# andrewcharlesjones/spatial-alignment

Measured on AMD Instinct MI355X. Metric: training steps/sec (ELBO fwd+bwd), 2-view N=10k M=200, 1/2/4/8 GPU, higher is better.
Workload: dtype f32 (fp64 warp layer, covariance whitening and M x M factorisations)

## Files before the change

include/gpsa_hip.h:

```cpp
#ifndef GPSA_HIP_H
#define GPSA_HIP_H

#ifdef __cplusplus
extern "C" {
#endif

enum {
  GPSA_F32 = 0,
  GPSA_F64 = 1,
  GPSA_F32_X64 = 2,
  GPSA_F32_OUT64 = 3,
  GPSA_F32_ACC64 = 4
};
enum { GPSA_K_RBF = 0, GPSA_K_MATERN12 = 1, GPSA_K_MATERN32 = 2 };
enum { GPSA_EINVAL = -1, GPSA_EWORKSPACE = -2, GPSA_EUNSUPPORTED = -3 };

int gpsa_version(void);
const char* gpsa_build_arch(void);
const char* gpsa_source_hash(void);

int gpsa_kmat(int dtype, int in_dtype, int kind, const void* Z, int M, const void* X, long long C,
              int D, const void* ls_u, const void* var_u, double jitter, void* K, void* stream);

long long gpsa_kmat_bwd_workspace(int dtype, int M, long long C, int D);
int gpsa_kmat_bwd(int dtype, int in_dtype, int kind, const void* Z, int M, const void* X, long long C,
                  int D, const void* ls_u, const void* var_u, const void* Kbar, int same, void* dZ,
                  void* dX, void* dparams, void* workspace, long long workspace_bytes, void* stream);

long long gpsa_gemm_workspace(int dtype, int m, int n, int batch, int splitk);
int gpsa_gemm(int dtype, int transA, int transB, int m, int n, long long k, double alpha,
              const void* A, long long lda, long long strideA, const void* B, long long ldb,
              long long strideB, double beta, void* C, long long ldc, long long strideC, int batch,
              int splitk, void* workspace, long long workspace_bytes, void* stream);

int gpsa_thin_update_f32(const float* A, int M, int L, const float* B, long long C, float* out, void* stream);

int gpsa_omega_fwd(const float* A, int M, int batch, double jitter, double* Omega, void* stream);
int gpsa_omega_bwd(const double* G, const float* A, int M, int batch, int symmetric, float* dA,
                   void* stream);
int gpsa_omega_fwd2(const float* A0, int n0, double* Omega0, const float* A1, int n1, double* Omega1, int M,
                    double jitter, void* stream);
int gpsa_omega_bwd2(const double* G0, const float* A0, float* dA0, int n0, const double* G1, const float* A1,
                    float* dA1, int n1, int M, int symmetric, void* stream);

int gpsa_chol_f64(void* A, int M, int batch, void* logdet, int* info, void* stream);
int gpsa_tri_inv_f64(const void* L, void* Linv, int M, int batch, void* stream);
int gpsa_chol_inv_f64(const void* A, void* Linv, int M, int batch, void* logdet, int* info,
                      void* stream);
int gpsa_chol_inv_sel_f64(const void* A, void* Linv, int M, int batch, int n_always, int keep_lo, int keep_hi,
                          void* logdet, int* info, void* stream);
long long gpsa_chol_inv_blocked_workspace(int M, int batch);
int gpsa_chol_inv_blocked_f64(const void* A, void* Linv, int M, int batch, void* logdet, int* info,
                              void* workspace, long long workspace_bytes, void* stream);

int gpsa_experiment_split_bf16_product(const float* Omega, const float* alpha, int M, long long C, int L, int nprod,
                                       float* W, void* stream);
int gpsa_experiment_split_bf16_rate(int nprod, int outputs, float* out, void* stream);

long long gpsa_quadform_workspace(int dtype, int M, long long C, int L);
int gpsa_quadform_fwd(int dtype, int omega_dtype, const void* alpha, const void* Omega, int M,
                      long long C, int L, void* v, void* workspace, long long workspace_bytes,
                      void* stream);
int gpsa_quadform_bwd_alpha(int dtype, int omega_dtype, const void* alpha, const void* Omega,
                            const void* g, int M, long long C, int L, void* dalpha, void* workspace,
                            long long workspace_bytes, void* stream);
int gpsa_quadform_fwd_keep(int dtype, const void* alpha, const void* Omega, int M, long long C, int L,
                           void* v, void* W, const void* dcT, void* meanT, void* stream);
int gpsa_quadform_bwd_alpha_kept(int dtype, const void* W, const void* g, int M, long long C, int L,
                                 const void* dcT, const void* dmeanT, void* dalpha, void* stream);
long long gpsa_quadform_keep_f32_workspace(int M, int L);
long long gpsa_quadform_keep_f32_bytes(int M, long long C, int L);
int gpsa_quadform_fwd_keep_f32(int omega_dtype, const float* alpha, const void* Omega, int M, long long C, int L,
                               float* v, float* W, void* workspace, long long workspace_bytes, void* stream);
int gpsa_quadform_bwd_alpha_kept_f32(const float* W, const float* g, int M, long long C, int L, const float* dcT,
                                     const float* dmeanT, float* dalpha, void* stream);
int gpsa_quadform_elbo_parts(void);
long long gpsa_quadform_elbo_f32_workspace(int M, long long C, int L);
int gpsa_quadform_elbo_f32(int omega_dtype, const float* alpha, const void* Omega, int M, long long C, int L,
                           const float* meanT, const double* q, const float* var_u, const float* eps, const float* Y,
                           long long N, int S, const float* noise_u, float* g, float* dmeanT, float* abar, double* part,
                           float* FT, void* workspace, long long workspace_bytes, void* stream);
int gpsa_quadform_elbo_takes_delta(int M);
int gpsa_quadform_elbo_delta_f32(int omega_dtype, const float* alpha, const void* Omega, int M, long long C, int L,
                                 const float* delta, const double* q, const float* var_u, const float* eps,
                                 const float* Y, long long N, int S, const float* noise_u, float* g, float* dmeanT,
                                 float* abar, double* part, float* FT, void* workspace, long long workspace_bytes,
                                 void* stream);
long long gpsa_quadform_elbo_x3_f32_workspace(int M, long long C, int L);
int gpsa_quadform_elbo_x3_f32(int omega_dtype, const float* alpha, const void* Omega, int M, long long C, int L,
                              const float* meanT, const double* q, const float* var_u, const float* eps, const float* Y,
                              long long N, int S, const float* noise_u, float* g, float* dmeanT, float* abar, double* part,
                              float* FT, void* workspace, long long workspace_bytes, void* stream);
int gpsa_quadform_elbo_delta_x3_f32(int omega_dtype, const float* alpha, const void* Omega, int M, long long C, int L,
                                    const float* delta, const double* q, const float* var_u, const float* eps,
                                    const float* Y, long long N, int S, const float* noise_u, float* g, float* dmeanT,
                                    float* abar, double* part, float* FT, void* workspace, long long workspace_bytes,
                                    void* stream);
int gpsa_quadform_elbo_skip_f32(int omega_dtype, const float* alpha, const void* Omega, int M, long long C, int L,
                                const float* meanT, const double* q, const float* var_u, const float* eps, const float* Y,
                                long long N, int S, const float* noise_u, float* g, float* dmeanT, float* abar,
                                double* part, float* FT, void* workspace, long long workspace_bytes, void* stream);
int gpsa_quadform_elbo_delta_skip_f32(int omega_dtype, const float* alpha, const void* Omega, int M, long long C, int L,
                                      const float* delta, const double* q, const float* var_u, const float* eps,
                                      const float* Y, long long N, int S, const float* noise_u, float* g, float* dmeanT,
                                      float* abar, double* part, float* FT, void* workspace, long long workspace_bytes,
                                      void* stream);
int gpsa_quadform_bwd_omega(int dtype, int out_dtype, const void* alpha, const void* g, int M, long long C,
                            int L, void* dOmega, void* workspace, long long workspace_bytes, void* stream);
int gpsa_quadform_bwd_omega_takes_delta(int M, long long C);
int gpsa_quadform_bwd_omega_delta_f32(int out_dtype, const float* alpha, const float* g, const float* dmeanT, int M,
                                      long long C, int L, void* dOmega, float* ddelta, double dbeta, void* workspace,
                                      long long workspace_bytes, void* stream);
long long gpsa_quadform_bwd_omega_x3_workspace(int M, long long C, int L);
int gpsa_quadform_bwd_omega_x3(int dtype, int out_dtype, const void* alpha, const void* g, int M, long long C, int L,
                               void* dOmega, void* workspace, long long workspace_bytes, void* stream);
int gpsa_quadform_bwd_omega_delta_x3(int out_dtype, const float* alpha, const float* g, const float* dmeanT, int M,
                                     long long C, int L, void* dOmega, float* ddelta, double dbeta, void* workspace,
                                     long long workspace_bytes, void* stream);

long long gpsa_whiten_workspace(int M);
int gpsa_whiten_f64(const double* Kinv, int in_dtype, const void* Kuf, int M, long long C,
                    int alpha_dtype, void* alpha, double* q, void* workspace, long long workspace_bytes,
                    void* stream);

int gpsa_panel_mm(int dtype, int p_dtype, int transP, const void* P, const void* X, int M, long long C,
                  void* Y, void* colsq, void* workspace, long long workspace_bytes, void* stream);

int gpsa_col_axpy(int dtype, const void* Y, const void* X, const void* d, double s, int M,
                  long long C, void* out, void* stream);

int gpsa_data_sample_fwd(const float* meanT, const float* v, const double* q, const float* var_u,
                         const float* eps, long long C, int L, float* F, float* Sigma, void* stream);
int gpsa_data_sample_bwd(const float* dF, const float* eps, const float* Sigma, const float* var_u,
                         long long C, int L, float* g, float* dmeanT, float* qbar, int dvar_dtype, void* dvar_u,
                         void* workspace, long long workspace_bytes, void* stream);
int gpsa_warp_sample_fwd(const double* meanT, const double* v, const double* q, const float* var_u,
                         const float* X, const float* slopes, const float* intercept,
                         const float* eps, long long n, int D, int S, float* Gmean, float* Gs,
                         double* Gs64, int* bad, void* stream);
int gpsa_warp_sample_bwd(const float* dGmean, const float* dGs, const double* dGs64, const float* eps,
                         const float* var_u, const float* X, long long n, int D, int S, double* dmeanT, double* g,
                         double* qbar, float* dvar_u, float* dslopes, float* dintercept,
                         void* workspace, long long workspace_bytes, void* stream);

int gpsa_mean_resid_fwd(const float* Z, const float* slopes, const float* intercept,
                        const float* delta, int M, int D, double scale, float* mu_z, double* resid,
                        void* stream);
int gpsa_mean_resid_bwd(const double* dresid, const float* Z, const float* slopes, int M, int D,
                        double scale, float* ddelta, float* dZ, float* dslopes, float* dintercept,
                        void* stream);

int gpsa_loglik_fwd(const float* F, const float* Y, const float* noise_u, int S, long long N, int P,
                    double* out, void* workspace, long long workspace_bytes, void* stream);
int gpsa_loglik_bwd(const float* F, const float* Y, const float* noise_u, const double* gout, int S,
                    long long N, int P, float* dF, float* dnoise_u, void* workspace,
                    long long workspace_bytes, void* stream);

int gpsa_bdot(int dtype, const void* A, long long strideA, const void* B, long long strideB,
              long long n, int batch, void* out, void* workspace, long long workspace_bytes,
              void* stream);
int gpsa_add_diag(int dtype, void* A, int M, int batch, double s, void* stream);

int gpsa_mvn_kl_fwd(const double* Kinv, const double* logdetK, const double* Omega,
                    long long omega_stride, const double* logdetO, long long logdet_stride,
                    const double* Dm, const double* KD, int M, int L, double* kl, void* stream);
int gpsa_mvn_kl_bwd(const double* Kuu, const double* Kinv, const double* Omega, long long omega_stride,
                    const double* Oinv, long long oinv_stride, const double* Dm, const double* KD,
                    const double* g, int M, int L, double* dOmega, double* dDm, double* Sp,
                    void* stream);

int gpsa_mvn_kl_grouped_fwd(const double* mats, const double* inv, const double* logdet,
                            const int* om_idx, const int* pr_idx, const double* D, int M, int T,
                            double* kl, double* KD, void* stream);
int gpsa_mvn_kl_grouped_bwd(const double* mats, const double* inv, const int* om_idx,
                            const int* pr_list, const int* grp_off, const int* order, const double* D,
                            const double* KD, const double* g, int M, int T, int P, double* dOmega,
                            double* dD, double* S, void* stream);

int gpsa_elbo_fwd(const double* ll, int n_ll, const double* kl, int n_kl, double kl_scale, float* loss,
                  void* stream);
int gpsa_elbo_bwd(const float* gloss, int n_ll, int n_kl, double kl_scale, double* dll, double* dkl,
                  void* stream);

long long gpsa_kmeans_workspace(long long N, int D, int K);
int gpsa_kmeans_assign(const float* X, long long N, int D, const float* centres, int K, int* assign,
                       float* d2, void* stream);
int gpsa_kmeans_update(const float* X, const int* assign, long long N, int D, int K, float* centres,
                       int* counts, void* workspace, long long workspace_bytes, void* stream);


int gpsa_kmat_batched(int kind, const float* Z, long long strideZ, int M, const float* X, long long strideX,
                      long long C, int D, const float* ls_u, const float* var_u, int stride_par,
                      const long long* n_live, int batch, double jitter, double* K, long long strideK,
                      void* stream);
long long gpsa_kmat_bwd_batched_workspace(int M, long long C, int D, int batch);
int gpsa_kmat_bwd_batched(int kind, const float* Z, long long strideZ, int M, const float* X, long long strideX,
                          long long C, int D, const float* ls_u, const float* var_u, int stride_par,
                          const long long* n_live, int batch, const double* Kbar, long long strideK, int same,
                          double* dZ, long long stride_dZ, double* dparams, void* workspace,
                          long long workspace_bytes, void* stream);
int gpsa_kmat_bwd_x64(int kind, const float* Z, int M, const double* X, long long C, int D, const float* ls_u,
                      const float* var_u, const float* Kbar, double* dZ, double* dX, double* dparams,
                      void* workspace, long long workspace_bytes, void* stream);
int gpsa_kmat_bwd_x64_f64(int kind, const float* Z, int M, const double* X, long long C, int D, const float* ls_u,
                          const float* var_u, const double* Kbar, double* dZ, double* dX, double* dparams,
                          void* workspace, long long workspace_bytes, void* stream);
int gpsa_kmat_bwd_x64_f64_axpy(int kind, const float* Z, int M, const double* X, long long C, int D, const float* ls_u,
                               const float* var_u, const double* Kbar, const double* X2, const float* d, double s,
                               double* dZ, double* dX, double* dparams, void* workspace, long long workspace_bytes,
                               void* stream);
long long gpsa_exact_dkuu_workspace(int M, long long C);
int gpsa_exact_dkuu_f64(const double* G, const double* A, const float* d, int M, long long C, double* dK,
                        void* workspace, long long workspace_bytes, void* stream);
long long gpsa_longk_f64_workspace(int M, long long K, int nprob);
int gpsa_longk_f64(int nprob, const double* const* G, const double* const* B, const void* const* d, int d_dtype,
                   int M, long long K, long long ld, int sym, const double* alpha, const double* beta,
                   double* const* out, void* workspace, long long workspace_bytes, void* stream);
int gpsa_kmat_bwd_x64_axpy(int kind, const float* Z, int M, const double* X, long long C, int D, const float* ls_u,
                           const float* var_u, const float* Kbar, const float* X2, const float* d, double s,
                           double* dZ, double* dX, double* dparams, void* workspace, long long workspace_bytes,
                           void* stream);
int gpsa_whiten_f64_dual(const double* Kinv, const double* Kuf, int M, long long C, double* alpha64, float* alpha32,
                         double* q, void* workspace, long long workspace_bytes, void* stream);

int gpsa_whiten_gen_f64_dual(const double* Kinv, int kind, const float* Z, const double* X64, int D, const float* ls_u,
                             const float* var_u, int M, long long C, double* alpha64, float* alpha32, double* q,
                             void* workspace, long long workspace_bytes, void* stream);
int gpsa_whiten_axpy_f32(const double* Kinv, const float* X, int M, long long C, const float* X2, const float* d,
                         double s, float* out, void* workspace, long long workspace_bytes, void* stream);
int gpsa_whiten_batched_f64(const double* Kinv, long long strideKinv, const double* Kuf, int M, long long C,
                            long long strideX, double* alpha, double* q, int batch, void* workspace,
                            long long workspace_bytes, void* stream);
int gpsa_quadform_fwd_keep_batched_f64(const double* alpha, const double* Omega, int M, long long C, int L,
                                       double* v, double* W, const double* dcT, double* meanT, int batch,
                                       void* stream);
int gpsa_quadform_bwd_alpha_kept_batched_f64(const double* W, const double* g, int M, long long C, int L,
                                             const double* dcT, const double* dmeanT, double* dalpha,
                                             int batch, void* stream);
int gpsa_col_axpy_batched_f64(const double* Y, const double* X, const double* d, double s, int M, long long C,
                              double* out, int batch, void* stream);
long long gpsa_gram_batched_workspace(int M, long long C, int L, int batch);
int gpsa_gram_batched_f64(const double* alpha, const double* g, int M, long long C, int L, double* dOmega,
                          int batch, void* workspace, long long workspace_bytes, void* stream);
int gpsa_mvn_kl_grouped_bwd_acc(const double* mats, const double* inv, const int* om_idx,
                                const int* pr_list, const int* grp_off, const int* order, const double* D,
                                const double* KD, const double* g, int M, int T, int P, double* dOmega,
                                double* dD, double* S, int accumulate, void* stream);
int gpsa_mvn_kl_grouped_fwd_slices(int M);
int gpsa_mvn_kl_grouped_fwd_sliced(const double* mats, const double* inv, const double* logdet, const int* om_idx,
                                   const int* pr_idx, const double* D, int M, int T, double* kl, double* KD,
                                   double* kl_copy, double* part, int* cnt, void* stream);

#define GPSA_MAX_MODS 4

typedef struct gpsa_step_desc {
  int n_views, n_dims, n_mods, n_samples;
  int m_x, m_g;
  int kind_warp, kind_data;
  int n_latent[GPSA_MAX_MODS];
  int n_out[GPSA_MAX_MODS];
  int has_lmc[GPSA_MAX_MODS];
  long long n_rows[GPSA_MAX_MODS];
  int s_test;
  long long n_test[GPSA_MAX_MODS];
  int want_kl;
  const int* view_fixed;
  const long long* view_rows;
  long long keep_budget_bytes;
  int exact_inducing_grad;
  int kl_own_lo, kl_own_hi;
  int contraction;
} gpsa_step_desc;

typedef struct gpsa_step_params {
  const float* Xtilde;
  const float* delta_G;
  const float* Omega_sqt_G;
  const float* warp_ls;
  const float* warp_var;
  const float* slopes;
  const float* intercepts;
  const float* Gtilde;
  const float* data_ls;
  const float* data_var;
  const float* Omega_sqt_F[GPSA_MAX_MODS];
  const float* delta_F[GPSA_MAX_MODS];
  const float* W[GPSA_MAX_MODS];
} gpsa_step_params;

typedef struct gpsa_step_param_grads {
  float *Xtilde, *delta_G, *Omega_sqt_G, *warp_ls, *warp_var, *Gtilde, *data_ls, *data_var;
  float* Omega_sqt_F[GPSA_MAX_MODS];
  float* delta_F[GPSA_MAX_MODS];
  float* W[GPSA_MAX_MODS];
} gpsa_step_param_grads;

typedef struct gpsa_step_io {
  const float* X[GPSA_MAX_MODS];
  const float* eps_G;
  const float* eps_F[GPSA_MAX_MODS];
  const float* G_test[GPSA_MAX_MODS];
  const float* eps_F_test[GPSA_MAX_MODS];
  float* G_means[GPSA_MAX_MODS];
  float* G_samples[GPSA_MAX_MODS];
  float* F_latent[GPSA_MAX_MODS];
  float* F_obs[GPSA_MAX_MODS];
  float* F_latent_test[GPSA_MAX_MODS];
  float* F_obs_test[GPSA_MAX_MODS];
  float* mu_z;
  double* kl;
  int* flag;
  int keep_products;
  int reuse_mm;
  int fuse_elbo;
  const float* Y[GPSA_MAX_MODS];
  const float* noise_u[GPSA_MAX_MODS];
  double* ll_part[GPSA_MAX_MODS];
  float* F_fused_T[GPSA_MAX_MODS];
  double* bwd_acc;
  int bwd_acc_mode;
  void* f_event;
  const float* loss_src;
  float* loss_dst;
  int skip_missing;
} gpsa_step_io;

typedef struct gpsa_step_out_grads {
  const float* dG_means[GPSA_MAX_MODS];
  const float* dG_samples[GPSA_MAX_MODS];
  const float* dF_latent[GPSA_MAX_MODS];
  const float* dF_obs[GPSA_MAX_MODS];
  const float* dF_latent_test[GPSA_MAX_MODS];
  const float* dF_obs_test[GPSA_MAX_MODS];
  const double* dkl;
  const float* gloss;
} gpsa_step_out_grads;

void* gpsa_step_create(const gpsa_step_desc* desc);
int gpsa_step_describe(const gpsa_step_desc* desc, long long* out);
void gpsa_step_destroy(void* plan);
long long gpsa_step_saved_bytes(const void* plan);
long long gpsa_step_saved_bytes_nokeep(const void* plan);
int gpsa_step_fused(const void* plan, int m);
int gpsa_step_contraction(const void* plan, int m);
long long gpsa_step_scratch_bytes(const void* plan);
long long gpsa_step_bwd_acc_bytes(const void* plan);
int gpsa_step_n_kl(const void* plan);
int gpsa_step_n_factorised(const void* plan);
long long gpsa_step_eps_g_numel(const void* plan);
int gpsa_step_graph(void* plan, int enable, long long* out);
long long gpsa_step_early_backwards(const void* plan);
int gpsa_step_batch_layout(const void* plan, long long* out);
int gpsa_step_forward(void* plan, const gpsa_step_params* params, const gpsa_step_io* io, void* saved,
                      void* scratch, int stages, void* stream);
unsigned long long gpsa_stream_capture_id(void* stream);
int gpsa_step_timing(void* plan, int slots);
int gpsa_step_timing_read(void* plan, float* ms, int max_steps);
int gpsa_step_backward(void* plan, const gpsa_step_params* params, const gpsa_step_io* io,
                       const gpsa_step_out_grads* og, void* saved, void* scratch,
                       const gpsa_step_param_grads* grads, void* stream);

int gpsa_elbo_loss_fwd(int n_ll, const float* const* F, const float* const* Y, const float* const* noise_u,
                       const int* S, const long long* N, const int* P, const double* kl, int n_kl,
                       double kl_scale, float* loss, double* ll_out, void* workspace,
                       long long workspace_bytes, void* stream);
int gpsa_elbo_loss_bwd(int n_ll, const float* const* F, const float* const* Y, const float* const* noise_u,
                       const int* S, const long long* N, const int* P, const float* gloss, int n_kl,
                       double kl_scale, float* const* dF, float* const* dnoise, float* dnoise_all, int n_noise,
                       double* dkl, void* workspace, long long workspace_bytes, void* stream);

int gpsa_elbo_loss_fused_fwd(int n_ll, const float* const* F, const float* const* Y, const float* const* noise_u,
                             const int* S, const long long* N, const int* P, const double* const* zpart, int nparts,
                             const double* kl, int n_kl, double kl_scale, float* loss, double* ll_out, void* workspace,
                             long long workspace_bytes, void* stream);
int gpsa_elbo_loss_fused_bwd(int n_ll, const float* const* F, const float* const* Y, const float* const* noise_u,
                             const int* S, const long long* N, const int* P, const double* const* zpart, int nparts,
                             const float* gloss, int n_kl, double kl_scale, float* const* dF, float* const* dnoise,
                             float* dnoise_all, int n_noise, double* dkl, void* workspace, long long workspace_bytes,
                             void* stream);
long long gpsa_lmc_loglik_workspace(long long C, int L, int P, int nparts);
int gpsa_lmc_loglik_fused_f32(const float* F, const float* W, const float* Y, const float* noise_u, int S, long long N,
                              int L, int P, double* zpart, int nparts, float* dF, float* dW, void* workspace,
                              long long workspace_bytes, void* stream);
int gpsa_elbo_fused_post(float* g_ext, float* dmeanT, float* abar, int M, long long C, int L, const float* gloss,
                         const float* var_u, int dvar_dtype, void* dvar_u, void* workspace, long long workspace_bytes,
                         void* stream);

int gpsa_adam_step(int n, float* const* params, const float* const* grads, float* const* exp_avg,
                   float* const* exp_avg_sq, const long long* numel, double lr, double beta1, double beta2,
                   double eps, float* step, void* stream);

int gpsa_row_sample_gather(int n_mods, const int* n_views, const long long* n_rows, const long long* batch,
                           unsigned long long seed, long long* counter, const float* const* X, const int* D,
                           const float* const* Y, const int* P, long long* const* rows, float* const* Xb,
                           float* const* Yb, void* stream);
int gpsa_elbo_loss_weighted_fwd(int n_ll, const float* const* F, const float* const* Y, const float* const* noise_u,
                                const int* S, const long long* N, const int* P, const int* n_views,
                                const long long* const* view_off, const double* const* w, const double* kl, int n_kl,
                                double kl_scale, float* loss, double* ll_out, void* workspace,
                                long long workspace_bytes, void* stream);
int gpsa_elbo_loss_weighted_bwd(int n_ll, const float* const* F, const float* const* Y, const float* const* noise_u,
                                const int* S, const long long* N, const int* P, const int* n_views,
                                const long long* const* view_off, const double* const* w, const float* gloss, int n_kl,
                                double kl_scale, float* const* dF, float* const* dnoise, float* dnoise_all,
                                int n_noise, double* dkl, void* workspace, long long workspace_bytes, void* stream);

long long gpsa_count_observed_workspace(void);
int gpsa_count_observed(int n_ll, const float* const* Y, const long long* N, const int* P, const int* n_views,
                        const long long* const* view_off, double* const* nobs, void* workspace,
                        long long workspace_bytes, void* stream);
int gpsa_elbo_loss_skip_fwd(int n_ll, const float* const* F, const float* const* Y, const float* const* noise_u,
                            const int* S, const long long* N, const int* P, const double* const* zpart, int nparts,
                            const int* n_views, const long long* const* view_off, const double* const* w,
                            const double* const* nobs, const double* kl, int n_kl, double kl_scale, float* loss,
                            double* ll_out, void* workspace, long long workspace_bytes, void* stream);
int gpsa_elbo_loss_skip_bwd(int n_ll, const float* const* F, const float* const* Y, const float* const* noise_u,
                            const int* S, const long long* N, const int* P, const double* const* zpart, int nparts,
                            const int* n_views, const long long* const* view_off, const double* const* w,
                            const double* const* nobs, const float* gloss, int n_kl, double kl_scale, float* const* dF,
                            float* const* dnoise, float* dnoise_all, int n_noise, double* dkl, void* workspace,
                            long long workspace_bytes, void* stream);
int gpsa_lmc_loglik_fused_skip_f32(const float* F, const float* W, const float* Y, const float* noise_u, int S, long long N,
                                   int L, int P, double* zpart, int nparts, float* dF, float* dW, void* workspace,
                                   long long workspace_bytes, void* stream);

#define GPSA_LIK_GAUSSIAN 0
#define GPSA_LIK_POISSON 1
long long gpsa_lgamma_sum_workspace(void);
int gpsa_lgamma_sum(int n_ll, const float* const* Y, const long long* N, const int* P, const int* n_views,
                    const long long* const* view_off, int skip, double* const* out, void* workspace,
                    long long workspace_bytes, void* stream);
int gpsa_elbo_loss_pois_fwd(int n_ll, const float* const* F, const float* const* Y, const float* const* noise_u,
                            const int* S, const long long* N, const int* P, const double* const* zpart, int nparts,
                            const int* n_views, const long long* const* view_off, const double* const* w,
                            const double* const* nobs, const int* kind, const double* const* lgam,
                            const float* const* log_offset, int skip, const double* kl, int n_kl, double kl_scale,
                            float* loss, double* ll_out, void* workspace, long long workspace_bytes, void* stream);
int gpsa_elbo_loss_pois_bwd(int n_ll, const float* const* F, const float* const* Y, const float* const* noise_u,
                            const int* S, const long long* N, const int* P, const double* const* zpart, int nparts,
                            const int* n_views, const long long* const* view_off, const double* const* w,
                            const double* const* nobs, const int* kind, const double* const* lgam,
                            const float* const* log_offset, int skip, const float* gloss, int n_kl, double kl_scale,
                            float* const* dF, float* const* dnoise, float* dnoise_all, int n_noise, double* dkl,
                            void* workspace, long long workspace_bytes, void* stream);
int gpsa_quadform_elbo_pois_f32(int omega_dtype, const float* alpha, const void* Omega, int M, long long C, int L,
                                const float* meanT, const double* q, const float* var_u, const float* eps, const float* Y,
                                long long N, int S, const float* noise_u, float* g, float* dmeanT, float* abar,
                                double* part, float* FT, const float* log_offset, int skip, void* workspace,
                                long long workspace_bytes, void* stream);
int gpsa_quadform_elbo_delta_pois_f32(int omega_dtype, const float* alpha, const void* Omega, int M, long long C, int L,
                                      const float* delta, const double* q, const float* var_u, const float* eps,
                                      const float* Y, long long N, int S, const float* noise_u, float* g, float* dmeanT,
                                      float* abar, double* part, float* FT, const float* log_offset, int skip,
                                      void* workspace, long long workspace_bytes, void* stream);
int gpsa_lmc_loglik_fused_pois_f32(const float* F, const float* W, const float* Y, const float* log_offset, int skip, int S,
                                   long long N, int L, int P, double* zpart, int nparts, float* dF, float* dW,
                                   void* workspace, long long workspace_bytes, void* stream);
int gpsa_step_likelihood(void* plan, int m, int kind, const float* log_offset);

#define GPSA_LIK_NEGBIN 2
long long gpsa_nb_const_workspace(long long N, int P, int n_views);
int gpsa_nb_const(int n_ll, const float* const* Y, const long long* N, const int* P, const float* const* log_disp,
                  const int* n_views, const long long* const* view_off, const double* const* w, int skip,
                  double* const* csum, double* const* dconst, void* workspace, long long workspace_bytes, void* stream);
int gpsa_quadform_elbo_nb_f32(int omega_dtype, const float* alpha, const void* Omega, int M, long long C, int L,
                              const float* meanT, const double* q, const float* var_u, const float* eps, const float* Y,
                              long long N, int S, const float* noise_u, float* g, float* dmeanT, float* abar, double* part,
                              float* FT, const float* log_offset, const float* log_disp, float* u_elems, double* usum,
                              int skip, void* workspace, long long workspace_bytes, void* stream);
int gpsa_quadform_elbo_delta_nb_f32(int omega_dtype, const float* alpha, const void* Omega, int M, long long C, int L,
                                    const float* delta, const double* q, const float* var_u, const float* eps,
                                    const float* Y, long long N, int S, const float* noise_u, float* g, float* dmeanT,
                                    float* abar, double* part, float* FT, const float* log_offset, const float* log_disp,
                                    float* u_elems, double* usum, int skip, void* workspace, long long workspace_bytes,
                                    void* stream);
int gpsa_step_dispersion(void* plan, int m, const float* log_disp, float* u_elems, double* usum, const float* log_offset);
long long gpsa_lmc_loglik_nb_workspace(long long C, int L, int P, int nparts);
int gpsa_lmc_loglik_fused_nb_f32(const float* F, const float* W, const float* Y, const float* log_offset,
                                 const float* log_disp, int skip, int S, long long N, int L, int P, double* zpart,
                                 int nparts, float* dF, float* dW, double* usum, void* workspace,
                                 long long workspace_bytes, void* stream);
long long gpsa_elbo_loss_nb_workspace(int n_ll, const int* S, const long long* N, const int* P, const int* n_views,
                                      const int* kind);
int gpsa_elbo_loss_nb_fwd(int n_ll, const float* const* F, const float* const* Y, const float* const* noise_u,
                          const int* S, const long long* N, const int* P, const double* const* zpart, int nparts,
                          const int* n_views, const long long* const* view_off, const double* const* w,
                          const double* const* nobs, const int* kind, const double* const* lgam,
                          const float* const* log_offset, const float* const* log_disp, const double* const* csum,
                          int skip, const double* kl, int n_kl, double kl_scale, float* loss, double* ll_out,
                          void* workspace, long long workspace_bytes, void* stream);
int gpsa_elbo_loss_nb_bwd(int n_ll, const float* const* F, const float* const* Y, const float* const* noise_u,
                          const int* S, const long long* N, const int* P, const double* const* zpart, int nparts,
                          const int* n_views, const long long* const* view_off, const double* const* w,
                          const double* const* nobs, const int* kind, const double* const* lgam,
                          const float* const* log_offset, const float* const* log_disp, const double* const* dconst,
                          const double* const* usum, int skip, const float* gloss, int n_kl, double kl_scale,
                          float* const* dF, float* const* dnoise, float* dnoise_all, int n_noise, double* dkl,
                          float* const* ddisp, void* workspace, long long workspace_bytes, void* stream);

int gpsa_predict_moments_f32(const float* meanT, const float* v, const double* q, const float* var_u, long long c,
                             int S, int L, int P, const float* W, const float* noise_u, int include_noise,
                             const float* Y, float* F_mean, float* F_var, float* Fl_mean, float* Fl_var, double* lpd,
                             void* stream);

int gpsa_predict_counts_f32(const float* meanT, const float* v, const double* q, const float* var_u, long long c, int S,
                            int L, int P, const float* W, const float* log_offset, const float* Y, float* Y_mean,
                            float* Y_var, double* lpd, void* stream);

int gpsa_warp_field_f64(int kind, const double* Z, const double* beta, const double* A, const double* b,
                        const double* ls_u, const double* var_u, const double* X, long long n, int M, int D, double* G,
                        double* J, double* det, void* stream);
int gpsa_warp_invert_f64(int kind, const double* Z, const double* beta, const double* A, const double* b,
                         const double* ls_u, const double* var_u, const double* target, const double* x0, int iters,
                         long long n, int M, int D, double* X, double* residual, void* stream);

long long gpsa_knn_workspace(long long nq, long long nr, int k, int parts);
int gpsa_knn_f64(const double* Q, long long nq, const double* R, long long nr, int D, int k, int exclude_self, int parts,
                 int* idx, double* d2, void* workspace, long long workspace_bytes, void* stream);
int gpsa_knn_average_f32(const int* idx, const double* d2, long long nq, int k, const float* Y, long long nr, int P,
                         int weights, float* out, void* stream);
// ... 107 lines not shown
```

spatial_alignment_amd/_lib.py:

```python
import ctypes as C
import os

_HERE = os.path.dirname(os.path.abspath(__file__))
LIB_PATH = os.path.join(_HERE, "libgpsa_hip.so")

_vp, _i, _ll, _d = C.c_void_p, C.c_int, C.c_longlong, C.c_double

SIGNATURES = {
    "gpsa_version": (_i, []),
    "gpsa_build_arch": (C.c_char_p, []),
    "gpsa_source_hash": (C.c_char_p, []),
    "gpsa_kmat": (_i, [_i, _i, _i, _vp, _i, _vp, _ll, _i, _vp, _vp, _d, _vp, _vp]),
    "gpsa_kmat_bwd_workspace": (_ll, [_i, _i, _ll, _i]),
    "gpsa_kmat_bwd": (_i, [_i, _i, _i, _vp, _i, _vp, _ll, _i, _vp, _vp, _vp, _i, _vp, _vp, _vp, _vp, _ll, _vp]),
    "gpsa_gemm_workspace": (_ll, [_i, _i, _i, _i, _i]),
    "gpsa_gemm": (_i, [_i, _i, _i, _i, _i, _ll, _d, _vp, _ll, _ll, _vp, _ll, _ll, _d, _vp, _ll, _ll,
                       _i, _i, _vp, _ll, _vp]),
    "gpsa_omega_fwd": (_i, [_vp, _i, _i, _d, _vp, _vp]),
    "gpsa_omega_bwd": (_i, [_vp, _vp, _i, _i, _i, _vp, _vp]),
    "gpsa_omega_fwd2": (_i, [_vp, _i, _vp, _vp, _i, _vp, _i, _d, _vp]),
    "gpsa_omega_bwd2": (_i, [_vp, _vp, _vp, _i, _vp, _vp, _vp, _i, _i, _i, _vp]),
    "gpsa_chol_f64": (_i, [_vp, _i, _i, _vp, _vp, _vp]),
    "gpsa_tri_inv_f64": (_i, [_vp, _vp, _i, _i, _vp]),
    "gpsa_chol_inv_f64": (_i, [_vp, _vp, _i, _i, _vp, _vp, _vp]),
    "gpsa_experiment_split_bf16_product": (_i, [_vp, _vp, _i, _ll, _i, _i, _vp, _vp]),
    "gpsa_experiment_split_bf16_rate": (_i, [_i, _i, _vp, _vp]),
    "gpsa_chol_inv_sel_f64": (_i, [_vp, _vp, _i, _i, _i, _i, _i, _vp, _vp, _vp]),
    "gpsa_chol_inv_blocked_workspace": (_ll, [_i, _i]),
    "gpsa_chol_inv_blocked_f64": (_i, [_vp, _vp, _i, _i, _vp, _vp, _vp, _ll, _vp]),
    "gpsa_quadform_workspace": (_ll, [_i, _i, _ll, _i]),
    "gpsa_quadform_fwd": (_i, [_i, _i, _vp, _vp, _i, _ll, _i, _vp, _vp, _ll, _vp]),
    "gpsa_quadform_bwd_alpha": (_i, [_i, _i, _vp, _vp, _vp, _i, _ll, _i, _vp, _vp, _ll, _vp]),
    "gpsa_quadform_fwd_keep": (_i, [_i, _vp, _vp, _i, _ll, _i, _vp, _vp, _vp, _vp, _vp]),
    "gpsa_quadform_bwd_alpha_kept": (_i, [_i, _vp, _vp, _i, _ll, _i, _vp, _vp, _vp, _vp]),
    "gpsa_quadform_bwd_omega": (_i, [_i, _i, _vp, _vp, _i, _ll, _i, _vp, _vp, _ll, _vp]),
    "gpsa_quadform_bwd_omega_takes_delta": (_i, [_i, _ll]),
    "gpsa_quadform_bwd_omega_delta_f32": (_i, [_i, _vp, _vp, _vp, _i, _ll, _i, _vp, _vp, _d, _vp, _ll, _vp]),
    "gpsa_quadform_bwd_omega_x3_workspace": (_ll, [_i, _ll, _i]),
    "gpsa_quadform_bwd_omega_x3": (_i, [_i, _i, _vp, _vp, _i, _ll, _i, _vp, _vp, _ll, _vp]),
    "gpsa_quadform_bwd_omega_delta_x3": (_i, [_i, _vp, _vp, _vp, _i, _ll, _i, _vp, _vp, _d, _vp, _ll, _vp]),
    "gpsa_whiten_workspace": (_ll, [_i]),
    "gpsa_whiten_f64": (_i, [_vp, _i, _vp, _i, _ll, _i, _vp, _vp, _vp, _ll, _vp]),
    "gpsa_panel_mm": (_i, [_i, _i, _i, _vp, _vp, _i, _ll, _vp, _vp, _vp, _ll, _vp]),
    "gpsa_col_axpy": (_i, [_i, _vp, _vp, _vp, _d, _i, _ll, _vp, _vp]),
    "gpsa_data_sample_fwd": (_i, [_vp, _vp, _vp, _vp, _vp, _ll, _i, _vp, _vp, _vp]),
    "gpsa_data_sample_bwd": (_i, [_vp, _vp, _vp, _vp, _ll, _i, _vp, _vp, _vp, _i, _vp, _vp, _ll, _vp]),
    "gpsa_warp_sample_fwd": (_i, [_vp, _vp, _vp, _vp, _vp, _vp, _vp, _vp, _ll, _i, _i, _vp, _vp, _vp, _vp, _vp]),
    "gpsa_warp_sample_bwd": (_i, [_vp, _vp, _vp, _vp, _vp, _vp, _ll, _i, _i, _vp, _vp, _vp, _vp, _vp, _vp, _vp,
                                  _ll, _vp]),
    "gpsa_mean_resid_fwd": (_i, [_vp, _vp, _vp, _vp, _i, _i, _d, _vp, _vp, _vp]),
    "gpsa_mean_resid_bwd": (_i, [_vp, _vp, _vp, _i, _i, _d, _vp, _vp, _vp, _vp, _vp]),
    "gpsa_loglik_fwd": (_i, [_vp, _vp, _vp, _i, _ll, _i, _vp, _vp, _ll, _vp]),
    "gpsa_loglik_bwd": (_i, [_vp, _vp, _vp, _vp, _i, _ll, _i, _vp, _vp, _vp, _ll, _vp]),
    "gpsa_bdot": (_i, [_i, _vp, _ll, _vp, _ll, _ll, _i, _vp, _vp, _ll, _vp]),
    "gpsa_add_diag": (_i, [_i, _vp, _i, _i, _d, _vp]),
    "gpsa_mvn_kl_fwd": (_i, [_vp, _vp, _vp, _ll, _vp, _ll, _vp, _vp, _i, _i, _vp, _vp]),
    "gpsa_mvn_kl_bwd": (_i, [_vp, _vp, _vp, _ll, _vp, _ll, _vp, _vp, _vp, _i, _i, _vp, _vp, _vp, _vp]),
    "gpsa_mvn_kl_grouped_fwd": (_i, [_vp, _vp, _vp, _vp, _vp, _vp, _i, _i, _vp, _vp, _vp]),
    "gpsa_mvn_kl_grouped_bwd": (_i, [_vp, _vp, _vp, _vp, _vp, _vp, _vp, _vp, _vp, _i, _i, _i, _vp, _vp, _vp,
                                     _vp]),
    "gpsa_elbo_fwd": (_i, [_vp, _i, _vp, _i, _d, _vp, _vp]),
    "gpsa_elbo_bwd": (_i, [_vp, _i, _i, _d, _vp, _vp, _vp]),
    "gpsa_kmeans_workspace": (_ll, [_ll, _i, _i]),
    "gpsa_kmeans_assign": (_i, [_vp, _ll, _i, _vp, _i, _vp, _vp, _vp]),
    "gpsa_kmeans_update": (_i, [_vp, _vp, _ll, _i, _i, _vp, _vp, _vp, _ll, _vp]),
}

MAX_MODS = 4


class StepDesc(C.Structure):
    _fields_ = [
        ("n_views", _i), ("n_dims", _i), ("n_mods", _i), ("n_samples", _i),
        ("m_x", _i), ("m_g", _i), ("kind_warp", _i), ("kind_data", _i),
        ("n_latent", _i * MAX_MODS), ("n_out", _i * MAX_MODS), ("has_lmc", _i * MAX_MODS),
        ("n_rows", _ll * MAX_MODS), ("s_test", _i), ("n_test", _ll * MAX_MODS), ("want_kl", _i),
        ("view_fixed", C.POINTER(_i)), ("view_rows", C.POINTER(_ll)), ("keep_budget_bytes", _ll),
        ("exact_inducing_grad", _i), ("kl_own_lo", _i), ("kl_own_hi", _i), ("contraction", _i),
    ]


class StepParams(C.Structure):
    _fields_ = [
        ("Xtilde", _vp), ("delta_G", _vp), ("Omega_sqt_G", _vp), ("warp_ls", _vp), ("warp_var", _vp),
        ("slopes", _vp), ("intercepts", _vp), ("Gtilde", _vp), ("data_ls", _vp), ("data_var", _vp),
        ("Omega_sqt_F", _vp * MAX_MODS), ("delta_F", _vp * MAX_MODS), ("W", _vp * MAX_MODS),
    ]


class StepParamGrads(C.Structure):
    _fields_ = [
        ("Xtilde", _vp), ("delta_G", _vp), ("Omega_sqt_G", _vp), ("warp_ls", _vp), ("warp_var", _vp),
        ("Gtilde", _vp), ("data_ls", _vp), ("data_var", _vp),
        ("Omega_sqt_F", _vp * MAX_MODS), ("delta_F", _vp * MAX_MODS), ("W", _vp * MAX_MODS),
    ]


class StepIO(C.Structure):
    _fields_ = [
        ("X", _vp * MAX_MODS), ("eps_G", _vp), ("eps_F", _vp * MAX_MODS), ("G_test", _vp * MAX_MODS),
        ("eps_F_test", _vp * MAX_MODS), ("G_means", _vp * MAX_MODS), ("G_samples", _vp * MAX_MODS),
        ("F_latent", _vp * MAX_MODS), ("F_obs", _vp * MAX_MODS), ("F_latent_test", _vp * MAX_MODS),
        ("F_obs_test", _vp * MAX_MODS), ("mu_z", _vp), ("kl", _vp), ("flag", _vp), ("keep_products", _i),
        ("reuse_mm", _i), ("fuse_elbo", _i), ("Y", _vp * MAX_MODS), ("noise_u", _vp * MAX_MODS),
        ("ll_part", _vp * MAX_MODS), ("F_fused_T", _vp * MAX_MODS), ("bwd_acc", _vp), ("bwd_acc_mode", _i),
        ("f_event", _vp), ("loss_src", _vp), ("loss_dst", _vp), ("skip_missing", _i),
    ]


class StepOutGrads(C.Structure):
    _fields_ = [
        ("dG_means", _vp * MAX_MODS), ("dG_samples", _vp * MAX_MODS), ("dF_latent", _vp * MAX_MODS),
        ("dF_obs", _vp * MAX_MODS), ("dF_latent_test", _vp * MAX_MODS), ("dF_obs_test", _vp * MAX_MODS),
        ("dkl", _vp), ("gloss", _vp),
    ]


_pp = C.POINTER(_vp)

SIGNATURES.update({
    "gpsa_kmat_batched": (_i, [_i, _vp, _ll, _i, _vp, _ll, _ll, _i, _vp, _vp, _i, C.POINTER(_ll), _i, _d, _vp, _ll, _vp]),
    "gpsa_kmat_bwd_batched_workspace": (_ll, [_i, _ll, _i, _i]),
    "gpsa_kmat_bwd_batched": (_i, [_i, _vp, _ll, _i, _vp, _ll, _ll, _i, _vp, _vp, _i, C.POINTER(_ll), _i, _vp, _ll, _i,
                                   _vp, _ll, _vp, _vp, _ll, _vp]),
    "gpsa_kmat_bwd_x64": (_i, [_i, _vp, _i, _vp, _ll, _i, _vp, _vp, _vp, _vp, _vp, _vp, _vp, _ll, _vp]),
    "gpsa_kmat_bwd_x64_f64": (_i, [_i, _vp, _i, _vp, _ll, _i, _vp, _vp, _vp, _vp, _vp, _vp, _vp, _ll, _vp]),
    "gpsa_kmat_bwd_x64_f64_axpy": (_i, [_i, _vp, _i, _vp, _ll, _i, _vp, _vp, _vp, _vp, _vp, _d, _vp, _vp, _vp, _vp, _ll,
                                        _vp]),
    "gpsa_exact_dkuu_workspace": (_ll, [_i, _ll]),
    "gpsa_exact_dkuu_f64": (_i, [_vp, _vp, _vp, _i, _ll, _vp, _vp, _ll, _vp]),
    "gpsa_longk_f64_workspace": (_ll, [_i, _ll, _i]),
    "gpsa_longk_f64": (_i, [_i, _vp, _vp, _vp, _i, _i, _ll, _ll, _i, _vp, _vp, _vp, _vp, _ll, _vp]),
    "gpsa_kmat_bwd_x64_axpy": (_i, [_i, _vp, _i, _vp, _ll, _i, _vp, _vp, _vp, _vp, _vp, _d, _vp, _vp, _vp, _vp, _ll,
                                    _vp]),
    "gpsa_thin_update_f32": (_i, [_vp, _i, _i, _vp, _ll, _vp, _vp]),
    "gpsa_whiten_f64_dual": (_i, [_vp, _vp, _i, _ll, _vp, _vp, _vp, _vp, _ll, _vp]),
    "gpsa_whiten_gen_f64_dual": (_i, [_vp, _i, _vp, _vp, _i, _vp, _vp, _i, _ll, _vp, _vp, _vp, _vp, _ll, _vp]),
    "gpsa_whiten_axpy_f32": (_i, [_vp, _vp, _i, _ll, _vp, _vp, _d, _vp, _vp, _ll, _vp]),
    "gpsa_whiten_batched_f64": (_i, [_vp, _ll, _vp, _i, _ll, _ll, _vp, _vp, _i, _vp, _ll, _vp]),
    "gpsa_quadform_fwd_keep_batched_f64": (_i, [_vp, _vp, _i, _ll, _i, _vp, _vp, _vp, _vp, _i, _vp]),
    "gpsa_quadform_bwd_alpha_kept_batched_f64": (_i, [_vp, _vp, _i, _ll, _i, _vp, _vp, _vp, _i, _vp]),
    "gpsa_col_axpy_batched_f64": (_i, [_vp, _vp, _vp, _d, _i, _ll, _vp, _i, _vp]),
    "gpsa_gram_batched_workspace": (_ll, [_i, _ll, _i, _i]),
    "gpsa_gram_batched_f64": (_i, [_vp, _vp, _i, _ll, _i, _vp, _i, _vp, _ll, _vp]),
    "gpsa_mvn_kl_grouped_bwd_acc": (_i, [_vp, _vp, _vp, _vp, _vp, _vp, _vp, _vp, _vp, _i, _i, _i, _vp, _vp, _vp, _i,
                                         _vp]),
    "gpsa_mvn_kl_grouped_fwd_slices": (_i, [_i]),
    "gpsa_mvn_kl_grouped_fwd_sliced": (_i, [_vp, _vp, _vp, _vp, _vp, _vp, _i, _i, _vp, _vp, _vp, _vp, _vp, _vp]),
    "gpsa_step_create": (_vp, [C.POINTER(StepDesc)]),
    "gpsa_step_describe": (_i, [C.POINTER(StepDesc), C.POINTER(_ll)]),
    "gpsa_step_destroy": (None, [_vp]),
    "gpsa_step_saved_bytes": (_ll, [_vp]),
    "gpsa_step_saved_bytes_nokeep": (_ll, [_vp]),
    "gpsa_quadform_keep_f32_workspace": (_ll, [_i, _i]),
    "gpsa_quadform_fwd_keep_f32": (_i, [_i, _vp, _vp, _i, _ll, _i, _vp, _vp, _vp, _ll, _vp]),
    "gpsa_quadform_keep_f32_bytes": (_ll, [_i, _ll, _i]),
    "gpsa_quadform_bwd_alpha_kept_f32": (_i, [_vp, _vp, _i, _ll, _i, _vp, _vp, _vp, _vp]),
    "gpsa_lmc_loglik_workspace": (_ll, [_ll, _i, _i, _i]),
    "gpsa_lmc_loglik_fused_f32": (_i, [_vp, _vp, _vp, _vp, _i, _ll, _i, _i, _vp, _i, _vp, _vp, _vp, _ll, _vp]),
    "gpsa_quadform_elbo_parts": (_i, []),
    "gpsa_quadform_elbo_f32_workspace": (_ll, [_i, _ll, _i]),
    "gpsa_quadform_elbo_f32": (_i, [_i, _vp, _vp, _i, _ll, _i, _vp, _vp, _vp, _vp, _vp, _ll, _i, _vp, _vp, _vp, _vp, _vp,
                                    _vp, _vp, _ll, _vp]),
    "gpsa_quadform_elbo_takes_delta": (_i, [_i]),
    "gpsa_quadform_elbo_x3_f32_workspace": (_ll, [_i, _ll, _i]),
    "gpsa_quadform_elbo_x3_f32": (_i, [_i, _vp, _vp, _i, _ll, _i, _vp, _vp, _vp, _vp, _vp, _ll, _i, _vp, _vp, _vp, _vp,
                                       _vp, _vp, _vp, _ll, _vp]),
    "gpsa_quadform_elbo_delta_x3_f32": (_i, [_i, _vp, _vp, _i, _ll, _i, _vp, _vp, _vp, _vp, _vp, _ll, _i, _vp, _vp, _vp,
                                             _vp, _vp, _vp, _vp, _ll, _vp]),
    "gpsa_quadform_elbo_delta_f32": (_i, [_i, _vp, _vp, _i, _ll, _i, _vp, _vp, _vp, _vp, _vp, _ll, _i, _vp, _vp, _vp, _vp,
                                          _vp, _vp, _vp, _ll, _vp]),
    "gpsa_step_scratch_bytes": (_ll, [_vp]),
    "gpsa_step_bwd_acc_bytes": (_ll, [_vp]),
    "gpsa_step_n_kl": (_i, [_vp]),
    "gpsa_step_n_factorised": (_i, [_vp]),
    "gpsa_step_eps_g_numel": (_ll, [_vp]),
    "gpsa_step_batch_layout": (_i, [_vp, C.POINTER(_ll)]),
    "gpsa_step_graph": (_i, [_vp, _i, C.POINTER(_ll)]),
    "gpsa_step_early_backwards": (_ll, [_vp]),
    "gpsa_stream_capture_id": (C.c_ulonglong, [_vp]),
    "gpsa_step_timing": (_i, [_vp, _i]),
    "gpsa_step_timing_read": (_i, [_vp, _vp, _i]),
    "gpsa_step_forward": (_i, [_vp, C.POINTER(StepParams), C.POINTER(StepIO), _vp, _vp, _i, _vp]),
    "gpsa_step_backward": (_i, [_vp, C.POINTER(StepParams), C.POINTER(StepIO), C.POINTER(StepOutGrads), _vp, _vp,
                                C.POINTER(StepParamGrads), _vp]),
    "gpsa_elbo_loss_fwd": (_i, [_i, _pp, _pp, _pp, C.POINTER(_i), C.POINTER(_ll), C.POINTER(_i), _vp, _i, _d, _vp,
                                _vp, _vp, _ll, _vp]),
    "gpsa_elbo_loss_bwd": (_i, [_i, _pp, _pp, _pp, C.POINTER(_i), C.POINTER(_ll), C.POINTER(_i), _vp, _i, _d, _pp, _pp,
                                _vp, _i, _vp, _vp, _ll, _vp]),
    "gpsa_elbo_loss_fused_fwd": (_i, [_i, _pp, _pp, _pp, C.POINTER(_i), C.POINTER(_ll), C.POINTER(_i), _pp, _i, _vp, _i,
                                      _d, _vp, _vp, _vp, _ll, _vp]),
    "gpsa_elbo_loss_fused_bwd": (_i, [_i, _pp, _pp, _pp, C.POINTER(_i), C.POINTER(_ll), C.POINTER(_i), _pp, _i, _vp, _i,
                                      _d, _pp, _pp, _vp, _i, _vp, _vp, _ll, _vp]),
    "gpsa_elbo_fused_post": (_i, [_vp, _vp, _vp, _i, _ll, _i, _vp, _vp, _i, _vp, _vp, _ll, _vp]),
    "gpsa_step_fused": (_i, [_vp, _i]),
    "gpsa_step_contraction": (_i, [_vp, _i]),
    "gpsa_adam_step": (_i, [_i, _pp, _pp, _pp, _pp, C.POINTER(_ll), _d, _d, _d, _d, _vp, _vp]),
    "gpsa_row_sample_gather": (_i, [_i, C.POINTER(_i), C.POINTER(_ll), C.POINTER(_ll), C.c_ulonglong, _vp, _pp,
                                    C.POINTER(_i), _pp, C.POINTER(_i), _pp, _pp, _pp, _vp]),
    "gpsa_elbo_loss_weighted_fwd": (_i, [_i, _pp, _pp, _pp, C.POINTER(_i), C.POINTER(_ll), C.POINTER(_i),
                                         C.POINTER(_i), _pp, _pp, _vp, _i, _d, _vp, _vp, _vp, _ll, _vp]),
    "gpsa_elbo_loss_weighted_bwd": (_i, [_i, _pp, _pp, _pp, C.POINTER(_i), C.POINTER(_ll), C.POINTER(_i),
                                         C.POINTER(_i), _pp, _pp, _vp, _i, _d, _pp, _pp, _vp, _i, _vp, _vp, _ll, _vp]),
    "gpsa_quadform_elbo_skip_f32": (_i, [_i, _vp, _vp, _i, _ll, _i, _vp, _vp, _vp, _vp, _vp, _ll, _i, _vp, _vp, _vp, _vp,
                                         _vp, _vp, _vp, _ll, _vp]),
    "gpsa_quadform_elbo_delta_skip_f32": (_i, [_i, _vp, _vp, _i, _ll, _i, _vp, _vp, _vp, _vp, _vp, _ll, _i, _vp, _vp, _vp,
                                               _vp, _vp, _vp, _vp, _ll, _vp]),
    "gpsa_count_observed_workspace": (_ll, []),
    "gpsa_count_observed": (_i, [_i, _pp, C.POINTER(_ll), C.POINTER(_i), C.POINTER(_i), _pp, _pp, _vp, _ll, _vp]),
    "gpsa_elbo_loss_skip_fwd": (_i, [_i, _pp, _pp, _pp, C.POINTER(_i), C.POINTER(_ll), C.POINTER(_i), _pp, _i,
                                     C.POINTER(_i), _pp, _pp, _pp, _vp, _i, _d, _vp, _vp, _vp, _ll, _vp]),
    "gpsa_elbo_loss_skip_bwd": (_i, [_i, _pp, _pp, _pp, C.POINTER(_i), C.POINTER(_ll), C.POINTER(_i), _pp, _i,
                                     C.POINTER(_i), _pp, _pp, _pp, _vp, _i, _d, _pp, _pp, _vp, _i, _vp, _vp, _ll, _vp]),
    "gpsa_lmc_loglik_fused_skip_f32": (_i, [_vp, _vp, _vp, _vp, _i, _ll, _i, _i, _vp, _i, _vp, _vp, _vp, _ll, _vp]),
    "gpsa_predict_moments_f32": (_i, [_vp, _vp, _vp, _vp, _ll, _i, _i, _i, _vp, _vp, _i, _vp, _vp, _vp, _vp, _vp, _vp,
                                      _vp]),
    "gpsa_predict_counts_f32": (_i, [_vp, _vp, _vp, _vp, _ll, _i, _i, _i, _vp, _vp, _vp, _vp, _vp, _vp, _vp]),
    "gpsa_warp_field_f64": (_i, [_i, _vp, _vp, _vp, _vp, _vp, _vp, _vp, _ll, _i, _i, _vp, _vp, _vp, _vp]),
    "gpsa_warp_invert_f64": (_i, [_i, _vp, _vp, _vp, _vp, _vp, _vp, _vp, _vp, _i, _ll, _i, _i, _vp, _vp, _vp]),
    "gpsa_knn_workspace": (_ll, [_ll, _ll, _i, _i]),
    "gpsa_knn_f64": (_i, [_vp, _ll, _vp, _ll, _i, _i, _i, _i, _vp, _vp, _vp, _ll, _vp]),
    "gpsa_knn_average_f32": (_i, [_vp, _vp, _ll, _i, _vp, _ll, _i, _i, _vp, _vp]),
    "gpsa_knn_average_f64": (_i, [_vp, _vp, _ll, _i, _vp, _ll, _i, _i, _vp, _vp]),
    "gpsa_count_workspace": (_ll, [_ll, _ll]),
    "gpsa_count_margins_f32": (_i, [_vp, _ll, _ll, _vp, _vp, _vp, _vp, _vp, _vp, _ll, _vp]),
    "gpsa_count_deviance_f32": (_i, [_vp, _ll, _ll, _vp, _vp, _vp, _vp, _ll, _vp]),
    "gpsa_count_transform_f32": (_i, [_i, _vp, _ll, _ll, _vp, _vp, _d, _d, _d, _d, _vp, _vp]),
    "gpsa_standardize_views_f32": (_i, [_vp, _ll, _ll, C.POINTER(_ll), _i, _vp, _vp, _vp, _ll, _vp]),
    "gpsa_count_csr_workspace": (_ll, [_ll, _ll]),
    "gpsa_csr_check": (_i, [_vp, _vp, _vp, _ll, _ll, _ll, _vp, _vp, _ll, _vp]),
    "gpsa_count_margins_csr_f32": (_i, [_vp, _vp, _vp, _vp, _ll, _ll, _ll, _vp, _vp, _vp, _vp, _vp, _vp, _ll, _vp]),
    "gpsa_count_deviance_csr_f32": (_i, [_vp, _vp, _vp, _vp, _ll, _ll, _ll, _vp, _vp, _vp, _vp, _ll, _vp]),
    "gpsa_csr_gather_dense_f32": (_i, [_vp, _vp, _vp, _ll, _ll, _ll, _vp, _ll, _vp, _ll, _vp, _vp]),
    "gpsa_column_moments_workspace": (_ll, [_ll, _ll, _i]),
    "gpsa_column_moments_csr_workspace": (_ll, [_ll, _ll, _i]),
    "gpsa_column_moments_f32": (_i, [_i, _vp, _ll, _ll, _vp, C.POINTER(_ll), _i, _vp, _vp, _vp, _vp, _vp, _ll, _vp]),
    "gpsa_column_moments_csr_f32": (_i, [_i, _vp, _vp, _vp, _vp, _ll, _ll, _ll, _vp, C.POINTER(_ll), _i, _vp, _vp, _vp,
                                         _vp, _vp, _ll, _vp]),
    "gpsa_gpr_cov_f64": (_i, [_i, _vp, _ll, _vp, _ll, _i, _vp, _i, _i, _d, _vp, _vp]),
    "gpsa_gpr_lml_grad_workspace": (_ll, [_ll, _i]),
    "gpsa_gpr_lml_grad_f64": (_i, [_i, _vp, _ll, _i, _vp, _i, _vp, _i, _vp, _vp, _vp, _ll, _vp]),
    "gpsa_gpr_mean_f64": (_i, [_i, _vp, _ll, _vp, _ll, _i, _vp, _i, _vp, _i, _vp, _vp]),
    "gpsa_ot_dist_f64": (_i, [_vp, _ll, _i, _vp, _vp]),
    "gpsa_ot_sqmatvec_f64": (_i, [_vp, _ll, _ll, _vp, _vp, _vp]),
    "gpsa_ot_expr_rows_workspace": (_ll, [_ll]),
    "gpsa_ot_expr_rows_f32": (_i, [_i, _vp, _ll, _ll, _vp, _vp, _vp, _vp, _vp, _ll, _vp]),
    "gpsa_ot_expr_cost_f64": (_i, [_i, _vp, _ll, _ll, _vp, _vp, _vp]),
    "gpsa_ot_cost_workspace": (_ll, [_ll, _ll]),
    "gpsa_ot_cost_f64": (_i, [_vp, _vp, _vp, _vp, _vp, _vp, _vp, _d, _ll, _ll, _vp, _vp, _ll, _vp]),
    "gpsa_ot_sinkhorn_workspace": (_ll, [_ll, _ll]),
    "gpsa_ot_sinkhorn_f64": (_i, [_vp, _ll, _ll, _vp, _vp, _vp, _vp, _vp, _i, _vp, _ll, _vp]),
    "gpsa_ot_plan_workspace": (_ll, [_ll, _ll]),
    "gpsa_ot_plan_f64": (_i, [_vp, _ll, _ll, _vp, _vp, _vp, _vp, _vp, _vp, _vp, _vp, _vp, _vp, _ll, _vp]),
    "gpsa_image_select_workspace": (_ll, [_ll, _ll, _i]),
    "gpsa_image_select_count_u8": (_i, [_vp, _ll, _ll, _i, _i, _i, C.c_float, _i, C.POINTER(_d), _vp, _ll, _vp]),
    "gpsa_image_select_count_f32": (_i, [_vp, _ll, _ll, _i, _i, _i, C.c_float, _i, C.POINTER(_d), _vp, _ll, _vp]),
    "gpsa_image_select_write_u8": (_i, [_vp, _ll, _ll, _i, _i, _i, C.c_float, _i, C.POINTER(_d), _vp, _ll, _vp, _vp, _ll,
                                        _vp]),
    "gpsa_image_select_write_f32": (_i, [_vp, _ll, _ll, _i, _i, _i, C.c_float, _i, C.POINTER(_d), _vp, _ll, _vp, _vp, _ll,
                                         _vp]),
    "gpsa_image_sample_u8": (_i, [_vp, _ll, _ll, _i, _vp, _ll, _i, C.c_float, _vp, _vp, _vp]),
    "gpsa_image_sample_f32": (_i, [_vp, _ll, _ll, _i, _vp, _ll, _i, C.c_float, _vp, _vp, _vp]),
    "gpsa_graph_workspace": (_ll, [_ll]),
    "gpsa_graph_merge_count": (_i, [_vp, _vp, _vp, _ll, _i, _i, _vp, _vp]),
    "gpsa_graph_merge_write": (_i, [_vp, _vp, _vp, _ll, _i, _i, _i, _vp, _ll, _vp, _vp, _vp]),
    "gpsa_graph_check_f64": (_i, [_vp, _vp, _vp, _ll, _ll, _vp, _vp, _ll, _vp]),
    "gpsa_graph_sums_f64": (_i, [_vp, _vp, _vp, _vp, _vp, _ll, _ll, _vp, _vp, _ll, _vp]),
    "gpsa_autocorr_perm_workspace": (_ll, [_ll, _ll, _ll]),
    "gpsa_autocorr_perm_f64": (_i, [_vp, _ll, _ll, _vp, _vp, _vp, _ll, _vp, _ll, _i, _vp, _vp, _vp, _ll, _vp]),
    "gpsa_lgamma_sum_workspace": (_ll, []),
    "gpsa_lgamma_sum": (_i, [_i, _pp, C.POINTER(_ll), C.POINTER(_i), C.POINTER(_i), _pp, _i, _pp, _vp, _ll, _vp]),
    "gpsa_elbo_loss_pois_fwd": (_i, [_i, _pp, _pp, _pp, C.POINTER(_i), C.POINTER(_ll), C.POINTER(_i), _pp, _i,
                                     C.POINTER(_i), _pp, _pp, _pp, C.POINTER(_i), _pp, _pp, _i, _vp, _i, _d, _vp, _vp,
                                     _vp, _ll, _vp]),
    "gpsa_elbo_loss_pois_bwd": (_i, [_i, _pp, _pp, _pp, C.POINTER(_i), C.POINTER(_ll), C.POINTER(_i), _pp, _i,
                                     C.POINTER(_i), _pp, _pp, _pp, C.POINTER(_i), _pp, _pp, _i, _vp, _i, _d, _pp, _pp,
                                     _vp, _i, _vp, _vp, _ll, _vp]),
    "gpsa_quadform_elbo_pois_f32": (_i, [_i, _vp, _vp, _i, _ll, _i, _vp, _vp, _vp, _vp, _vp, _ll, _i, _vp, _vp, _vp, _vp,
                                         _vp, _vp, _vp, _i, _vp, _ll, _vp]),
    "gpsa_quadform_elbo_delta_pois_f32": (_i, [_i, _vp, _vp, _i, _ll, _i, _vp, _vp, _vp, _vp, _vp, _ll, _i, _vp, _vp, _vp,
                                               _vp, _vp, _vp, _vp, _i, _vp, _ll, _vp]),
    "gpsa_lmc_loglik_fused_pois_f32": (_i, [_vp, _vp, _vp, _vp, _i, _i, _ll, _i, _i, _vp, _i, _vp, _vp, _vp, _ll, _vp]),
    "gpsa_step_likelihood": (_i, [_vp, _i, _i, _vp]),
    "gpsa_nb_const_workspace": (_ll, [_ll, _i, _i]),
    "gpsa_nb_const": (_i, [_i, _pp, C.POINTER(_ll), C.POINTER(_i), _pp, C.POINTER(_i), _pp, _pp, _i, _pp, _pp, _vp, _ll,
                           _vp]),
    "gpsa_quadform_elbo_nb_f32": (_i, [_i, _vp, _vp, _i, _ll, _i, _vp, _vp, _vp, _vp, _vp, _ll, _i, _vp, _vp, _vp, _vp,
                                       _vp, _vp, _vp, _vp, _vp, _vp, _i, _vp, _ll, _vp]),
    "gpsa_quadform_elbo_delta_nb_f32": (_i, [_i, _vp, _vp, _i, _ll, _i, _vp, _vp, _vp, _vp, _vp, _ll, _i, _vp, _vp, _vp,
                                             _vp, _vp, _vp, _vp, _vp, _vp, _vp, _i, _vp, _ll, _vp]),
    "gpsa_step_dispersion": (_i, [_vp, _i, _vp, _vp, _vp, _vp]),
    "gpsa_lmc_loglik_nb_workspace": (_ll, [_ll, _i, _i, _i]),
    "gpsa_lmc_loglik_fused_nb_f32": (_i, [_vp, _vp, _vp, _vp, _vp, _i, _i, _ll, _i, _i, _vp, _i, _vp, _vp, _vp, _vp, _ll,
                                          _vp]),
    "gpsa_elbo_loss_nb_workspace": (_ll, [_i, C.POINTER(_i), C.POINTER(_ll), C.POINTER(_i), C.POINTER(_i),
                                          C.POINTER(_i)]),
    "gpsa_elbo_loss_nb_fwd": (_i, [_i, _pp, _pp, _pp, C.POINTER(_i), C.POINTER(_ll), C.POINTER(_i), _pp, _i,
                                   C.POINTER(_i), _pp, _pp, _pp, C.POINTER(_i), _pp, _pp, _pp, _pp, _i, _vp, _i, _d, _vp,
                                   _vp, _vp, _ll, _vp]),
    "gpsa_elbo_loss_nb_bwd": (_i, [_i, _pp, _pp, _pp, C.POINTER(_i), C.POINTER(_ll), C.POINTER(_i), _pp, _i,
                                   C.POINTER(_i), _pp, _pp, _pp, C.POINTER(_i), _pp, _pp, _pp, _pp, _pp, _i, _vp, _i, _d,
                                   _pp, _pp, _vp, _i, _vp, _pp, _vp, _ll, _vp]),
})

LIK_KINDS = {"gaussian": 0, "poisson": 1}
LIK_NEGBIN = 2
LIK_KIND_OF = dict(LIK_KINDS, negative_binomial=LIK_NEGBIN)

_lib = None


def source_hash():
    import glob
    import hashlib

    csrc = os.path.join(_HERE, "csrc")
    header = os.path.join(os.path.dirname(_HERE), "include", "gpsa_hip.h")
    files = sorted(glob.glob(os.path.join(csrc, "*.hip")) + glob.glob(os.path.join(csrc, "*.hpp")))
    if not files or not os.path.exists(header):
        return None
    h = hashlib.sha256()
    for f in files + [header]:
        h.update(os.path.basename(f).encode() + b"\0")
        h.update(open(f, "rb").read())
        h.update(b"\0")
    return h.hexdigest()


def library_hash(path=None):
    import re

    path = path or LIB_PATH
    if not os.path.exists(path):
        return None
    m = re.search(rb"GPSA_SOURCE_HASH=([0-9a-f]{64}|unstamped)", open(path, "rb").read())
    return m.group(1).decode() if m else None


class GpsaHipError(RuntimeError):
    pass


def load():
    global _lib
    if _lib is not None:
        return _lib
    if not os.path.exists(LIB_PATH):
        raise GpsaHipError(
            f"{LIB_PATH} not found: build it with `python -c 'import __graft_entry__ as g; g.build()'` "
            "(hipcc --offload-arch=gfx950).  There is no CPU fallback."
        )
    lib = C.CDLL(LIB_PATH)
    for name, (res, args) in SIGNATURES.items():
        fn = getattr(lib, name)
        fn.restype = res
        fn.argtypes = args
    want = source_hash()
    got = lib.gpsa_source_hash().decode().split("=", 1)[1]
    if want is not None and got != want and os.environ.get("GPSA_ALLOW_STALE_LIB") != "1":
        raise GpsaHipError(
            f"{LIB_PATH} was built from other sources (stamp {got[:12]}, sources {want[:12]}): rebuild it with "
            "`python -c 'import __graft_entry__ as g; g.build()'`"
        )
    _lib = lib
    return lib


GPSA_EINVAL, GPSA_EWORKSPACE, GPSA_EUNSUPPORTED = -1, -2, -3


def check(rc, what):
    if rc != 0:
        kind = {-1: "invalid argument", -2: "workspace too small", -3: "unsupported size"}.get(
            rc, f"hipError_t {rc}"
        )
        raise GpsaHipError(f"{what} failed: {kind}")
```

spatial_alignment_amd/csrc/longk64.hip:

```cpp
#include <stdlib.h>
#include <string.h>

#include "internal.hpp"

namespace gpsa {

typedef double lk_f64x4 __attribute__((ext_vector_type(4)));
typedef double lk_f64x2 __attribute__((ext_vector_type(2)));
typedef float lk_f32x2 __attribute__((ext_vector_type(2)));
typedef __attribute__((address_space(3))) void* lk_lds_ptr;

constexpr int LK_WAVES = 8;
constexpr int LK_MAXP = 48;

struct LongKArgs {
  const double* G[LK_MAXP];
  const double* B[LK_MAXP];
  const void* d[LK_MAXP];
  double* part;
  int M, nprob, nsplit, sym;
  long long K, ld, gper;
};

__device__ __forceinline__ void lk_set_m0(unsigned lds_base) {
  asm volatile("s_mov_b32 m0, %0\n\ts_nop 0" ::"s"(lds_base) : "memory");
}
template <int IMM>
__device__ __forceinline__ void lk_glds16(const void* gsrc_minus_imm) {
  asm volatile("global_load_lds_dwordx4 %0, off offset:%1" ::"v"(gsrc_minus_imm), "n"(IMM) : "memory");
}
template <int IMM>
__device__ __forceinline__ void lk_glds4(const void* gsrc_minus_imm) {
  asm volatile("global_load_lds_dword %0, off offset:%1" ::"v"(gsrc_minus_imm), "n"(IMM) : "memory");
}

template <int MB, bool HASG, int DT>
__global__ void __launch_bounds__(512) longk64_kernel(LongKArgs a) {
  static_assert(HASG || DT != 0, "a left operand");
  constexpr int MP = MB * 16;
  constexpr int NOPD = HASG ? 2 : 1;
  constexpr int NPIECE = MB * NOPD * 2;
  constexpr int NPW = (NPIECE + LK_WAVES - 1) / LK_WAVES;
  static_assert(NPW <= 8, "two groups of four pieces per wave (an immediate offset reaches 4 KiB)");
  constexpr int DAREA = DT == 2 ? 1024 : 256;
  constexpr int STAGE_B = NPW * LK_WAVES * 1024 + (DT ? LK_WAVES * DAREA : 0);
  constexpr int NT_MAX = (MB * MB + LK_WAVES - 1) / LK_WAVES;
  constexpr int NT_SYM = (MB * (MB + 1) / 2 + LK_WAVES - 1) / LK_WAVES;
  extern __shared__ __attribute__((aligned(16))) char lk_smem[];

  const int tid = threadIdx.x, lane = tid & 63;
  const int w = __builtin_amdgcn_readfirstlane(tid >> 6);
  const int li = lane & 15, kq = lane >> 4;
  const int p = blockIdx.y, sp = blockIdx.x;
  const int M = a.M;
  const long long K = a.K, ld = a.ld;
  const double* __restrict__ Bp = a.B[p];
  const double* __restrict__ Gp = HASG ? a.G[p] : nullptr;
  const long long ng = (K + 15) >> 4;
  const long long g_lo = (long long)sp * a.gper;
  long long g_hi = g_lo + a.gper;
  if (g_hi > ng) g_hi = ng;
  const unsigned lds0 = (unsigned)(unsigned long long)(lk_lds_ptr)(&lk_smem[0]);

  const int T = a.sym ? MB * (MB + 1) / 2 : MB * MB;
  const int t_lo = w * T / LK_WAVES, t_hi = (w + 1) * T / LK_WAVES;
  const int cnt = t_hi - t_lo;
  int i0 = 0, j0 = 0;
  if (a.sym) {
    while ((i0 + 1) * (i0 + 2) / 2 <= t_lo) ++i0;
    j0 = t_lo - i0 * (i0 + 1) / 2;
  } else {
    i0 = t_lo / MB;
    j0 = t_lo - i0 * MB;
  }
  if (cnt == 0) i0 = j0 = 0;

  const double* rp[NPW];
  int koff[NPW];
#pragma unroll
  for (int u = 0; u < NPW; ++u) {
    int q = w + LK_WAVES * u;
    q = q < NPIECE ? q : NPIECE - 1;
    const int h = q & 1, ot = q >> 1;
    const bool isg = HASG && ot >= MB;
    const int t = isg ? ot - MB : ot;
    int row = t * 16 + li;
    row = row < M ? row : M - 1;
    rp[u] = (isg ? Gp : Bp) + (long long)row * ld;
    koff[u] = 8 * h + 2 * kq;
  }

  auto issue = [&](long long g, int s) {
    const long long kb = g << 4;
#pragma unroll
    for (int u = 0; u < NPW; ++u) {
      if ((u & 3) == 0)
        lk_set_m0(__builtin_amdgcn_readfirstlane(lds0 + (unsigned)(s * STAGE_B + (w * NPW + u) * 1024)));
      long long k = kb + koff[u];
      k = k < K - 2 ? k : K - 2;
      const char* src = reinterpret_cast<const char*>(rp[u] + k);
      switch (u & 3) {
        case 0: lk_glds16<0>(src); break;
        case 1: lk_glds16<1024>(src - 1024); break;
        case 2: lk_glds16<2048>(src - 2048); break;
        default: lk_glds16<3072>(src - 3072); break;
      }
    }
    if (DT != 0) {
      lk_set_m0(__builtin_amdgcn_readfirstlane(lds0 + (unsigned)(s * STAGE_B + NPW * LK_WAVES * 1024 + w * DAREA)));
      if (DT == 1) {
        long long k = kb + (lane & 15);
        k = k < K ? k : K - 1;
        lk_glds4<0>(reinterpret_cast<const float*>(a.d[p]) + k);
      } else {
        long long k = kb + 2 * (lane & 7);
        k = k < K - 1 ? k : K - 2;
        lk_glds16<0>(reinterpret_cast<const double*>(a.d[p]) + k);
      }
    }
  };

  lk_f64x4 acc[NT_MAX];
#pragma unroll
  for (int t = 0; t < NT_MAX; ++t) acc[t] = (lk_f64x4){0.0, 0.0, 0.0, 0.0};

  if (g_lo < g_hi) {
    issue(g_lo, 0);
    int s = 0;
    for (long long g = g_lo; g < g_hi; ++g) {
      asm volatile("s_waitcnt vmcnt(0)" ::: "memory");
      __syncthreads();
      if (g + 1 < g_hi) issue(g + 1, s ^ 1);
      const char* slot = lk_smem + s * STAGE_B;
      const char* dslot = slot + NPW * LK_WAVES * 1024 + w * DAREA;
      const long long k_a = (g << 4) + 2 * kq;
      double dv[2][2] = {{1.0, 1.0}, {1.0, 1.0}};
      bool ok[2][2];
#pragma unroll
      for (int h = 0; h < 2; ++h) {
        ok[h][0] = k_a + 8 * h < K;
        ok[h][1] = k_a + 8 * h + 1 < K;
        if (DT == 1) {
          const lk_f32x2 x = *reinterpret_cast<const lk_f32x2*>(dslot + 4 * (8 * h + 2 * kq));
          dv[h][0] = (double)x.x;
          dv[h][1] = (double)x.y;
        } else if (DT == 2) {
          const lk_f64x2 x = *reinterpret_cast<const lk_f64x2*>(dslot + 8 * (8 * h + 2 * kq));
          dv[h][0] = x.x;
          dv[h][1] = x.y;
        }
      }
#define LK_FRAG(O, TL, H)                                                                              \
  (*reinterpret_cast<const lk_f64x2*>(slot + ((((((O) * MB + (TL)) * 2 + (H)) & 7) * NPW +             \
                                                 ((((O) * MB + (TL)) * 2 + (H)) >> 3)) << 10) + lane * 16))
      int i = i0, j = j0, cur = -1;
      double af[2][2] = {{0.0, 0.0}, {0.0, 0.0}};
      lk_f64x2 bn0 = LK_FRAG(0, j, 0), bn1 = LK_FRAG(0, j, 1);
#pragma unroll
      for (int t = 0; t < NT_MAX; ++t) {
        if (t >= NT_SYM && a.sym) break;
        if (i != cur) {
          cur = i;
#pragma unroll
          for (int h = 0; h < 2; ++h) {
            const lk_f64x2 bi = LK_FRAG(0, i, h);
            double x0, x1;
            if (HASG) {
              const lk_f64x2 gi = LK_FRAG(1, i, h);
              x0 = DT ? fma(dv[h][0], bi.x, gi.x) : gi.x;
              x1 = DT ? fma(dv[h][1], bi.y, gi.y) : gi.y;
            } else {
              x0 = dv[h][0] * bi.x;
              x1 = dv[h][1] * bi.y;
            }
            af[h][0] = ok[h][0] ? x0 : 0.0;
            af[h][1] = ok[h][1] ? x1 : 0.0;
          }
        }
        const lk_f64x2 b0 = bn0, b1 = bn1;
        if (t + 1 < cnt) {
          ++j;
          if (a.sym ? j > i : j == MB) {
            ++i;
            j = 0;
          }
        }
        if (t + 1 < NT_MAX) {
          bn0 = LK_FRAG(0, j, 0);
          bn1 = LK_FRAG(0, j, 1);
        }
        acc[t] = __builtin_amdgcn_mfma_f64_16x16x4f64(af[0][0], b0.x, acc[t], 0, 0, 0);
        acc[t] = __builtin_amdgcn_mfma_f64_16x16x4f64(af[0][1], b0.y, acc[t], 0, 0, 0);
        acc[t] = __builtin_amdgcn_mfma_f64_16x16x4f64(af[1][0], b1.x, acc[t], 0, 0, 0);
        acc[t] = __builtin_amdgcn_mfma_f64_16x16x4f64(af[1][1], b1.y, acc[t], 0, 0, 0);
      }
#undef LK_FRAG
      s ^= 1;
    }
  }
  double* __restrict__ out = a.part + ((long long)p * a.nsplit + sp) * MP * MP;
  int i = i0, j = j0;
#pragma unroll
  for (int t = 0; t < NT_MAX; ++t) {
    if (t < cnt) {
#pragma unroll
      for (int r = 0; r < 4; ++r) out[(long long)(i * 16 + kq + 4 * r) * MP + j * 16 + li] = acc[t][r];
      ++j;
      if (a.sym ? j > i : j == MB) {
        ++i;
        j = 0;
      }
    }
  }
}

struct LongKOut {
  double* out[LK_MAXP];
  double alpha[LK_MAXP], beta[LK_MAXP];
};

__global__ void __launch_bounds__(256)
longk64_reduce_kernel(const double* __restrict__ part, int M, int MP, int nsplit, int sym, LongKOut o) {
  __shared__ double red[4][64];
  const int lane = threadIdx.x & 63, grp = threadIdx.x >> 6;
  const int p = blockIdx.y;
  const long long e = blockIdx.x * 64LL + lane;
  const int r = (int)(e / M), c = (int)(e % M);
  const bool ok = e < (long long)M * M && !(sym && c > r);
  const long long mm = (long long)MP * MP;
  const double* q = part + (long long)p * nsplit * mm + (long long)r * MP + c;
  double a0 = 0.0, a1 = 0.0, a2 = 0.0, a3 = 0.0;
  if (ok) {
    int s = grp;
    for (; s + 12 < nsplit; s += 16) {
      a0 += q[s * mm];
      a1 += q[(s + 4) * mm];
      a2 += q[(s + 8) * mm];
      a3 += q[(s + 12) * mm];
    }
    for (; s < nsplit; s += 4) a0 += q[s * mm];
  }
  red[grp][lane] = (a0 + a1) + (a2 + a3);
  __syncthreads();
  if (grp == 0 && ok) {
    const double sum = (red[0][lane] + red[1][lane]) + (red[2][lane] + red[3][lane]);
    const double al = o.alpha[p], be = o.beta[p];
    double* dst = o.out[p] + (long long)r * M + c;
    *dst = (be == 0.0) ? al * sum : al * sum + be * (*dst);
    if (sym && c < r) {
      double* dm = o.out[p] + (long long)c * M + r;
      *dm = (be == 0.0) ? al * sum : al * sum + be * (*dm);
    }
  }
}

static inline int longk_mb_for(int M) {
  const int mb = (M + 15) / 16;
  if (mb <= 2) return 2;
  if (mb <= 4) return 4;
  if (mb <= 7) return 7;
  if (mb <= 13) return 13;
  if (mb <= 16) return 16;
  return 0;
}

static inline int longk_nsplit(long long K, int nprob) {
  const long long ng = (K + 15) / 16;
  long long s = (long long)num_cus() / (nprob > 0 ? nprob : 1);
  if (s > ng / 4) s = ng / 4;
  return (int)(s < 1 ? 1 : s);
}

template <int MB, bool HASG, int DT>
static int longk64_launch_mb(const LongKArgs& a, hipStream_t st) {
  constexpr int NPIECE = MB * (HASG ? 2 : 1) * 2, NPW = (NPIECE + LK_WAVES - 1) / LK_WAVES;
  constexpr int lds = 2 * (NPW * LK_WAVES * 1024 + (DT ? LK_WAVES * (DT == 2 ? 1024 : 256) : 0));
  static per_device_flag attr_flag;
  bool& attr_set = attr_flag.here();
  if (!attr_set) {
    if (hipFuncSetAttribute(reinterpret_cast<const void*>(&longk64_kernel<MB, HASG, DT>),
                            hipFuncAttributeMaxDynamicSharedMemorySize, lds) != hipSuccess)
      return GPSA_EUNSUPPORTED;
    attr_set = true;
  }
  dim3 grid((unsigned)a.nsplit, (unsigned)a.nprob);
  longk64_kernel<MB, HASG, DT><<<grid, 512, lds, st>>>(a);
  GPSA_LAUNCH_CHECK();
  return 0;
}

template <bool HASG, int DT>
static int longk64_launch(int MB, const LongKArgs& a, hipStream_t st) {
  switch (MB) {
    case 2: return longk64_launch_mb<2, HASG, DT>(a, st);
    case 4: return longk64_launch_mb<4, HASG, DT>(a, st);
    case 7: return longk64_launch_mb<7, HASG, DT>(a, st);
    case 13: return longk64_launch_mb<13, HASG, DT>(a, st);
    case 16: return longk64_launch_mb<16, HASG, DT>(a, st);
    default: return GPSA_EUNSUPPORTED;
  }
}

}

extern "C" {

long long gpsa_longk_f64_workspace(int M, long long K, int nprob) {
  using namespace gpsa;
  const int MB = longk_mb_for(M);
  if (MB == 0 || nprob < 1 || nprob > LK_MAXP || K < 512 || (K & 1)) return 0;
  const int ns = longk_nsplit(K, nprob);
  if ((long long)ns * nprob < 48) return 0;
  return (long long)nprob * ns * MB * 16 * MB * 16 * 8;
}

int gpsa_longk_f64(int nprob, const double* const* G, const double* const* B, const void* const* d, int d_dtype,
                   int M, long long K, long long ld, int sym, const double* alpha, const double* beta,
                   double* const* out, void* workspace, long long workspace_bytes, void* stream) {
  using namespace gpsa;
  if (nprob < 1 || nprob > LK_MAXP || !B || !out || !alpha || !beta || M < 1 || K < 2 || ld < K) return GPSA_EINVAL;
  if (d != nullptr && d_dtype != GPSA_F32 && d_dtype != GPSA_F64) return GPSA_EINVAL;
  if (G == nullptr && d == nullptr) return GPSA_EINVAL;
  const long long need = gpsa_longk_f64_workspace(M, K, nprob);
  if (need == 0 || (ld & 1)) return GPSA_EUNSUPPORTED;
  if (workspace_bytes < need) return GPSA_EWORKSPACE;
  const int MB = longk_mb_for(M);
  LongKArgs a;
  LongKOut o;
  memset(&a, 0, sizeof(a));
  memset(&o, 0, sizeof(o));
  for (int p = 0; p < nprob; ++p) {
    a.B[p] = B[p];
    a.G[p] = G ? G[p] : nullptr;
    a.d[p] = d ? d[p] : nullptr;
    if (!B[p] || !out[p] || (G && !G[p]) || (d && !d[p])) return GPSA_EINVAL;
    if ((reinterpret_cast<uintptr_t>(B[p]) & 15) || (G && (reinterpret_cast<uintptr_t>(G[p]) & 15)) ||
        (d && d_dtype == GPSA_F64 && (reinterpret_cast<uintptr_t>(d[p]) & 15)))
      return GPSA_EUNSUPPORTED;
    o.out[p] = out[p];
    o.alpha[p] = alpha[p];
    o.beta[p] = beta[p];
  }
  a.part = reinterpret_cast<double*>(workspace);
  a.M = M;
  a.nprob = nprob;
  a.nsplit = longk_nsplit(K, nprob);
  a.sym = sym ? 1 : 0;
  a.K = K;
  a.ld = ld;
  a.gper = cdiv(cdiv(K, 16), a.nsplit);
  hipStream_t st = as_stream(stream);
  int rc;
  if (G && d && d_dtype == GPSA_F32) rc = longk64_launch<true, 1>(MB, a, st);
  else if (G && d) rc = longk64_launch<true, 2>(MB, a, st);
  else if (G) rc = longk64_launch<true, 0>(MB, a, st);
  else if (d_dtype == GPSA_F32) rc = longk64_launch<false, 1>(MB, a, st);
  else rc = longk64_launch<false, 2>(MB, a, st);
  if (rc) return rc;
  dim3 rg((unsigned)cdiv((long long)M * M, 64), (unsigned)nprob);
  longk64_reduce_kernel<<<rg, 256, 0, st>>>(a.part, M, MB * 16, a.nsplit, a.sym, o);
  GPSA_LAUNCH_CHECK();
  return 0;
}

}
```

spatial_alignment_amd/csrc/step.hip:

```cpp
#include <stdint.h>
#include <stdio.h>
#include <stdlib.h>
#include <string.h>

#include <new>
#include <vector>

#include "internal.hpp"

namespace gpsa {

constexpr int MAXMODS = GPSA_MAX_MODS;
constexpr int KM_MAXB_STEP = 16;

struct Arena {
  char* base = nullptr;
  long long off = 0, high = 0;
  long long limit = -1;
  bool dry = false;
  bool overflow = false;
  template <typename T>
  T* get(long long n) {
    off = (off + 255) & ~255LL;
    T* p = dry ? nullptr : reinterpret_cast<T*>(base + off);
// ... 592 lines not shown
  p->bidx.assign(V, -1);
  p->nview.assign(V, 0);
  p->epsoff.assign(V, 0);
  for (int m = 0; m < nm; ++m) {
    long long tot = 0;
    for (int v = 0; v < V; ++v) {
      if (p->rows[(long long)m * V + v] < 0) { free_plan(p); return nullptr; }
      tot += p->rows[(long long)m * V + v];
    }
    if (tot != dsc->n_rows[m] || dsc->n_latent[m] < 1 || dsc->n_out[m] < 1) { free_plan(p); return nullptr; }
    if (!dsc->has_lmc[m] && dsc->n_latent[m] != dsc->n_out[m]) { free_plan(p); return nullptr; }
  }
  long long maxn = 0;
  for (int v = 0; v < V; ++v) {
    for (int m = 0; m < nm; ++m) p->nview[v] += p->rows[(long long)m * V + v];
    if (!p->fixed[v]) {
      p->bidx[v] = (int)p->free_views.size();
      p->free_views.push_back(v);
      p->epsoff[v] = p->eps_total;
      p->eps_total += (long long)S * p->nview[v] * D;
      if (p->nview[v] > maxn) maxn = p->nview[v];
    }
  }
  p->nf = (int)p->free_views.size();
  p->Cs = (maxn + 63) / 64 * 64;
  for (int b = 0; b < p->nf;) {
    int e = b + 1;
    while (e < p->nf && p->free_views[e] == p->free_views[e - 1] + 1 && e - b < KM_MAXB_STEP) ++e;
    p->runs.push_back(Run{p->free_views[b], b, e - b});
    b = e;
  }
  p->Ltot = 0;
  for (int m = 0; m < nm; ++m) {
    p->Loff[m] = p->Ltot;
    p->Ltot += dsc->n_latent[m];
  }
  for (int m = nm; m < MAXMODS; ++m) p->Loff[m] = p->Ltot;
  p->merged = p->Mx == p->Mg;
  if (p->merged) {
    p->ng = 1;
    p->grp[0].M = p->Mx;
    p->grp[0].n_prior = p->nf + 1;
    p->grp[0].n_omega = V * D + p->Ltot;
    p->grp[0].kl_off = 0;
  } else {
    p->ng = 2;
    p->grp[0].M = p->Mx; p->grp[0].n_prior = p->nf; p->grp[0].n_omega = V * D; p->grp[0].kl_off = 0;
    p->grp[1].M = p->Mg; p->grp[1].n_prior = 1; p->grp[1].n_omega = p->Ltot; p->grp[1].kl_off = V * D;
  }
  for (int g = 0; g < p->ng; ++g) {
    Group& G = p->grp[g];
    G.own_lo = 0;
    G.own_hi = G.n_omega;
    if (dsc->kl_own_hi > 0) {
      const int lo = dsc->kl_own_lo - G.kl_off, hi = dsc->kl_own_hi - G.kl_off;
      G.own_lo = lo < 0 ? 0 : (lo > G.n_omega ? G.n_omega : lo);
      G.own_hi = hi < G.own_lo ? G.own_lo : (hi > G.n_omega ? G.n_omega : hi);
    }
  }
  for (int m = 0; m < nm; ++m)
    if (dsc->n_rows[m] > 0 && S > 0) {
      Pass q; q.m = m; q.test = false; q.C = (long long)S * dsc->n_rows[m];
      p->passes.push_back(q);
    }
  if (dsc->s_test > 0)
    for (int m = 0; m < nm; ++m)
      if (dsc->n_test[m] > 0) {
        Pass q; q.m = m; q.test = true; q.C = (long long)dsc->s_test * dsc->n_test[m];
        p->passes.push_back(q);
      }
  long long o = 0;
  auto take = [&](long long bytes) { long long r = o; o = align256(o + bytes); return r; };
  for (int g = 0; g < p->ng; ++g) {
    Group& G = p->grp[g];
    const long long mm = (long long)G.M * G.M;
    G.o_mats = take(G.nb() * mm * 8);
    G.o_inv = take(G.nb() * mm * 8);
    G.o_logdet = take(G.nb() * 8LL);
    G.o_info = take(G.nb() * 4LL);
    G.o_D = take((long long)G.n_omega * G.M * 8);
    G.o_KD = take((long long)G.n_omega * G.M * 8);
  }
  p->o_klcache = take(((long long)V * D + p->Ltot) * 8);
  p->o_resid = take((long long)V * p->Mx * D * 8);
  p->o_Xv = take((long long)p->nf * p->Cs * D * 4);
  p->o_alpha_w = take((long long)p->nf * p->Mx * p->Cs * 8);
  p->o_Wk = take((long long)p->nf * D * p->Mx * p->Cs * 8);
  for (int m = 0; m < nm; ++m) p->o_G64[m] = take((long long)S * dsc->n_rows[m] * D * 8);
  p->nbad = 0;
  for (int m = 0; m < nm; ++m) p->nbad += (dsc->n_rows[m] + 255) / 256;
  p->o_bad = take((p->nbad + 1) * 4);
  for (auto& q : p->passes) {
    q.o_alpha = take((long long)p->Mg * q.C * 4);
    q.o_sigma = take((long long)dsc->n_latent[q.m] * q.C * 4);
    if (dsc->exact_inducing_grad) q.o_alpha64 = take((long long)p->Mg * q.C * 8);
    const int Lq = dsc->n_latent[q.m];
    if (!q.test && !dsc->has_lmc[q.m] && gpsa_quadform_elbo_f32_workspace(p->Mg, q.C, Lq) > 0) {
      q.o_fuse = take((2LL * Lq + 1 + p->Mg) * q.C * 4);
      q.x3 = dsc->contraction == 1 && gpsa_quadform_elbo_x3_f32_workspace(p->Mg, q.C, Lq) > 0;
    }
    q.gx3 = !q.test && dsc->contraction == 1 && gpsa_quadform_bwd_omega_x3_workspace(p->Mg, q.C, Lq) > 0;
  }
  p->o_apk_w = take(gpsa_whiten_workspace(p->Mx) * (long long)(p->nf > 0 ? p->nf : 1));
  p->o_apk_d = take(gpsa_whiten_workspace(p->Mg));
  p->saved_bytes_nokeep = o + 256;
  {
    static const double keep_gb = [] { const char* e = getenv("GPSA_KEEP_GB"); return e ? atof(e) : 48.0; }();
    double budget = keep_gb * 1073741824.0;
    if (dsc->keep_budget_bytes > 0) {
      budget = (double)dsc->keep_budget_bytes;
    } else if (dsc->keep_budget_bytes < 0) {
      budget = -1.0;
    } else if (!host_only) {
      size_t fr = 0, total = 0;
      if (hipMemGetInfo(&fr, &total) == hipSuccess && 0.6 * (double)fr < budget) budget = 0.6 * (double)fr;
    }
    long long tot = 0;
    bool ok = true;
    for (auto& q : p->passes) {
      const long long b = gpsa_quadform_keep_f32_bytes(p->Mg, q.C, dsc->n_latent[q.m]);
      if (b == 0) ok = false;
      tot += b;
    }
    if (ok && (double)tot <= budget)
      for (auto& q : p->passes) q.o_keep = take(gpsa_quadform_keep_f32_bytes(p->Mg, q.C, dsc->n_latent[q.m]));
  }
  p->saved_bytes = o + 256;
  const long long n_ll = (long long)nm * (V + 1) + (long long)nm * V + V + V;
  long long n_int = V  + p->nf ;
  for (int g = 0; g < p->ng; ++g) {
    const Group& G = p->grp[g];
    n_int += 2 * G.n_omega + G.n_prior + (G.n_prior + 2) + G.n_omega;
  }
  const long long bytes = n_ll * 8 + n_int * 4 + 64;
  std::vector<char> host((size_t)bytes, 0);
  long long* hl = reinterpret_cast<long long*>(host.data());
  int* hi = reinterpret_cast<int*>(host.data() + n_ll * 8);
  if (!host_only && hipMalloc(reinterpret_cast<void**>(&p->dev), (size_t)bytes) != hipSuccess) { p->dev = nullptr; free_plan(p); return nullptr; }
  long long* dl = reinterpret_cast<long long*>(p->dev);
  int* di = reinterpret_cast<int*>(p->dev + n_ll * 8);
  long long lo = 0, io = 0;
  p->tab.vstart = dl + lo;
  for (int m = 0; m < nm; ++m) {
    long long acc = 0;
    for (int v = 0; v <= V; ++v) {
      hl[lo++] = acc;
      if (v < V) acc += p->rows[(long long)m * V + v];
    }
  }
  p->tab.colbase = dl + lo;
  for (int m = 0; m < nm; ++m)
    for (int v = 0; v < V; ++v) {
      long long acc = 0;
      for (int mm = 0; mm < m; ++mm) acc += p->rows[(long long)mm * V + v];
      hl[lo++] = acc;
    }
  p->tab.nview = dl + lo;
  for (int v = 0; v < V; ++v) hl[lo++] = p->nview[v];
  p->tab.epsoff = dl + lo;
  for (int v = 0; v < V; ++v) hl[lo++] = p->epsoff[v];
  p->tab.bidx = di + io;
  for (int v = 0; v < V; ++v) hi[io++] = p->bidx[v];
  p->d_free = di + io;
  for (int b = 0; b < p->nf; ++b) hi[io++] = p->free_views[b];
  for (int g = 0; g < p->ng; ++g) {
    Group& G = p->grp[g];
    std::vector<int> prior(G.n_omega, -1);
    for (int t = 0; t < G.n_omega; ++t) {
      if (g == 0 && t < V * D) prior[t] = p->bidx[t % V];
      else prior[t] = p->merged ? p->nf : 0;
      if (t < G.own_lo || t >= G.own_hi) prior[t] = -1;
    }
    G.om_idx = di + io;
    for (int t = 0; t < G.n_omega; ++t) hi[io++] = G.n_prior + t;
    G.pr_idx = di + io;
    for (int t = 0; t < G.n_omega; ++t) hi[io++] = prior[t];
    G.pr_list = di + io;
    for (int q = 0; q < G.n_prior; ++q) hi[io++] = q;
    std::vector<int> order, off(1, 0);
    for (int q = 0; q <= G.n_prior; ++q) {
      const int want = q < G.n_prior ? q : -1;
      for (int t = 0; t < G.n_omega; ++t)
        if (prior[t] == want) order.push_back(t);
      off.push_back((int)order.size());
    }
    G.grp_off = di + io;
    for (int q = 0; q < G.n_prior + 2; ++q) hi[io++] = off[q];
    G.order = di + io;
    for (int t = 0; t < G.n_omega; ++t) hi[io++] = order[t];
  }
  if (!host_only && hipMemcpy(p->dev, host.data(), (size_t)bytes, hipMemcpyHostToDevice) != hipSuccess) { free_plan(p); return nullptr; }
  p->tab.V = V; p->tab.D = D; p->tab.S = S; p->tab.nm = nm; p->tab.nf = p->nf; p->tab.Cs = p->Cs;
  return p;
}

static inline int splitk_for(long long k, int m, int n) {
  const long long tiles = cdiv(m, 64) * cdiv(n, 64);
  long long s = cdiv(512, tiles > 0 ? tiles : 1);
  if (s > 256) s = 256;
  if (s > k / 64) s = k / 64;
  if (s < 1) s = 1;
  return (int)s;
}
static inline int splitk_small(long long k, int m, int n, int batch) {
  if (batch == 1 && k >= 128 && k <= 1024 && cdiv(m, 64) * cdiv(n, 64) <= 32) {
    int s = (int)(k / 48);
    return s > 4 ? 4 : (s < 1 ? 1 : s);
  }
  return 1;
}

static inline int splitk_few(long long k, int m, int n, int batch) {
  if (batch <= 4 && k >= 128 && k <= 1024 && cdiv(m, 64) * cdiv(n, 64) * batch <= 64) {
    int s = (int)(k / 48);
    return s > 4 ? 4 : (s < 1 ? 1 : s);
  }
  return splitk_small(k, m, n, batch);
}

struct Ctx {
  Plan& P;
  const gpsa_step_params& prm;
  const gpsa_step_io& io;
  char* saved;
  Arena& sc;
  hipStream_t st;
  bool dry;
  bool apk_d = false;
  bool quiet = false;
  void* stv() const { return (void*)st; }
  template <typename T> T* sv(long long off) const { return reinterpret_cast<T*>(saved + off); }
  double* mats(const Group& G, int pos) const { return sv<double>(G.o_mats) + (long long)pos * G.M * G.M; }
  double* inv(const Group& G, int pos) const { return sv<double>(G.o_inv) + (long long)pos * G.M * G.M; }
};

static int gemm64(Ctx& c, int ta, int tb, int m, int n, long long k, double alpha, const double* A, long long lda,
                  long long sA, const double* B, long long ldb, long long sB, double beta, double* C,
                  long long ldc, long long sC, int batch, int splitk) {
  const bool dry = c.dry;
  const long long mk = c.sc.mark();
  void* ws = nullptr;
  long long wsb = 0;
  if (splitk > 1) {
    wsb = (long long)batch * splitk * m * n * 8;
    ws = c.sc.get<char>(wsb);
  }
  GPSA_RUN(gemm_launch<double>(ta, tb, m, n, k, alpha, A, lda, sA, B, ldb, sB, beta, C, ldc, sC, batch, splitk,
                               ws, wsb, c.st));
  c.sc.release(mk);
  return 0;
}
static int gemm32(Ctx& c, int ta, int tb, int m, int n, long long k, double alpha, const float* A, long long lda,
                  long long sA, const float* B, long long ldb, long long sB, double beta, float* C,
                  long long ldc, long long sC, int batch, int splitk) {
  const bool dry = c.dry;
  const long long mk = c.sc.mark();
  void* ws = nullptr;
  long long wsb = 0;
  if (splitk > 1) {
    wsb = (long long)batch * splitk * m * n * 4;
    ws = c.sc.get<char>(wsb);
  }
  GPSA_RUN(gemm_launch<float>(ta, tb, m, n, k, alpha, A, lda, sA, B, ldb, sB, beta, C, ldc, sC, batch, splitk,
                              ws, wsb, c.st));
  c.sc.release(mk);
  return 0;
}
static int thin_update(Ctx& c, const float* A, int M, int L, const float* B, long long C, float* out) {
  if (!c.dry) {
    if (c.sc.overflow) return GPSA_EWORKSPACE;
    const int rc = gpsa_thin_update_f32(A, M, L, B, C, out, c.stv());
    if (rc != GPSA_EUNSUPPORTED) return rc;
  }
  return gemm32(c, 0, 0, M, (int)C, L, 1.0, A, L, 0, B, C, 0, 1.0, out, C, 0, 1, 1);
}
template <typename TIA, typename TIB, typename TO>
static int gemmx(Ctx& c, int ta, int tb, int m, int n, long long k, double alpha, const TIA* A, long long lda,
                 long long sA, const TIB* B, long long ldb, long long sB, double beta, TO* C, long long ldc,
                 long long sC, int batch, int splitk) {
  const bool dry = c.dry;
  const long long mk = c.sc.mark();
  void* ws = nullptr;
  long long wsb = 0;
  if (splitk > 1) {
    wsb = (long long)batch * splitk * m * n * 8;
    ws = c.sc.get<char>(wsb);
  }
  GPSA_RUN((gemm64_launch<TIA, TIB, TO>(ta, tb, m, n, k, alpha, A, lda, sA, B, ldb, sB, beta, C, ldc, sC, batch,
                                        splitk, ws, wsb, c.st)));
  c.sc.release(mk);
  return 0;
}

static int longk(Ctx& c, int nprob, const double* const* G, const double* const* Bm, const void* const* d, int d_dtype,
                 int M, long long K, long long ld, int sym, const double* alpha, const double* beta, double* const* out) {
  const long long wsb = gpsa_longk_f64_workspace(M, K, nprob);
  if (wsb == 0 || (ld & 1)) return GPSA_EUNSUPPORTED;
  const long long mk = c.sc.mark();
  void* ws = c.sc.get<char>(wsb);
  int rc = 0;
  if (!c.dry) rc = gpsa_longk_f64(nprob, G, Bm, d, d_dtype, M, K, ld, sym, alpha, beta, out, ws, wsb, c.stv());
  c.sc.release(mk);
  return rc;
}

static int mm_stage_fwd(Ctx& c) {
  Plan& P = c.P;
  const bool dry = c.dry;
  const int V = P.V, D = P.D, Mx = P.Mx, Mg = P.Mg;
  Group& GW = P.gw();
  Group& GD = P.gd();
  const bool kl = P.d.want_kl != 0;
  double* klpart[2] = {nullptr, nullptr};
  int* klcnt[2] = {nullptr, nullptr};
  if (kl && !c.io.reuse_mm)
    for (int g = 0; g < P.ng; ++g)
      if (P.grp[g].n_omega > 0) {
        klpart[g] = c.sc.get<double>((long long)P.grp[g].n_omega * mvn_kl_grouped_fwd_slices(P.grp[g].M));
        klcnt[g] = c.sc.get<int>(P.grp[g].n_omega);
      }
  {
    PrepArgs a;
    memset(&a, 0, sizeof(a));
    a.Xtilde = c.prm.Xtilde; a.delta_G = c.prm.delta_G; a.slopes = c.prm.slopes; a.intercepts = c.prm.intercepts;
    for (int m = 0; m < P.nm; ++m) { a.delta_F[m] = c.prm.delta_F[m]; a.L[m] = P.d.n_latent[m]; a.Loff[m] = P.Loff[m]; }
    a.V = V; a.D = D; a.Mx = Mx; a.Mg = Mg; a.nm = P.nm;
    a.bidx = P.tab.bidx;
    a.mu_z = c.io.mu_z;
    a.resid = c.sv<double>(P.o_resid);
    a.Dw = kl ? c.sv<double>(GW.o_D) : nullptr;
    a.Dd = kl ? c.sv<double>(GD.o_D) + (P.merged ? (long long)V * D * Mx : 0) : nullptr;
    for (int g = 0; g < P.ng; ++g)
      if (kl && !P.grp[g].own_all() && !c.io.reuse_mm) {
        a.zinfo[g] = c.sv<int>(P.grp[g].o_info);
        a.nzinfo[g] = P.grp[g].nb();
      }
    for (int g = 0; g < P.ng; ++g)
      if (klcnt[g] != nullptr) {
        a.zinfo[2 + g] = klcnt[g];
        a.nzinfo[2 + g] = P.grp[g].n_omega;
      }
    const long long nd = kl ? cdiv((long long)P.Ltot * Mg, 256) : 0;
    if (!dry) {
      step_prep_kernel<<<(unsigned)(V + nd), 256, 0, c.st>>>(a);
      GPSA_LAUNCH_CHECK();
    }
  }
  if (c.io.reuse_mm) {
    if (kl && !dry)
      GPSA_CK(copy_async(c.io.kl, c.sv<double>(P.o_klcache), (size_t)((long long)V * D + P.Ltot) * 8, c.st));
    return 0;
  }
  for (const Run& r : P.runs)
    GPSA_RUN(gpsa_kmat_batched(P.d.kind_warp, c.prm.Xtilde + (long long)r.v0 * Mx * D, (long long)Mx * D, Mx,
                               c.prm.Xtilde + (long long)r.v0 * Mx * D, (long long)Mx * D, Mx, D,
                               c.prm.warp_ls + r.v0, c.prm.warp_var + r.v0, 1, nullptr, r.cnt, 1e-5,
                               c.mats(GW, P.pos_Kw(r.b0)), (long long)Mx * Mx, c.stv()));
  GPSA_RUN(gpsa_kmat_batched(P.d.kind_data, c.prm.Gtilde, 0, Mg, c.prm.Gtilde, 0, Mg, D, c.prm.data_ls,
                             c.prm.data_var, 0, nullptr, 1, 1e-5, c.mats(GD, P.pos_KF()), 0, c.stv()));
  const int m_first = (Mx == Mg && P.nm > 0) ? 1 : 0;
  if (m_first)
    GPSA_RUN(gpsa_omega_fwd2(c.prm.Omega_sqt_G, V * D, c.mats(GW, P.pos_OmG(0)), c.prm.Omega_sqt_F[0], P.d.n_latent[0],
                             c.mats(GD, P.pos_OmF(0, 0)), Mx, 1e-5, c.stv()));
  else
    GPSA_RUN(gpsa_omega_fwd(c.prm.Omega_sqt_G, Mx, V * D, 1e-5, c.mats(GW, P.pos_OmG(0)), c.stv()));
  for (int m = m_first; m < P.nm; ++m)
    GPSA_RUN(gpsa_omega_fwd(c.prm.Omega_sqt_F[m], Mg, P.d.n_latent[m], 1e-5, c.mats(GD, P.pos_OmF(m, 0)), c.stv()));
  for (int g = 0; g < P.ng; ++g) {
    Group& G = P.grp[g];
    const long long mm = (long long)G.M * G.M;
    double* logdet = c.sv<double>(G.o_logdet);
    int* info = c.sv<int>(G.o_info);
    const int np = G.n_prior, n_own = G.own_hi - G.own_lo;
    const bool sel = kl && !G.own_all();
    const int nb_main = kl ? G.nb() : np;
    auto inverse_product = [&](const double* Lin, double* out, int cnt) -> int {
      if (cnt <= 0) return 0;
      if (splitk_small(G.M, G.M, G.M, cnt) == 1)
        GPSA_RUN(gemm_launch_tri<double>(1, 0, G.M, G.M, G.M, 1.0, Lin, G.M, mm, Lin, G.M, mm, 0.0, out, G.M, mm, cnt, 1,
                                         nullptr, 0, c.st, GEMM_TRI_LTL));
      else
        GPSA_CK(gemm64(c, 1, 0, G.M, G.M, G.M, 1.0, Lin, G.M, mm, Lin, G.M, mm, 0.0, out, G.M, mm, cnt,
                       splitk_small(G.M, G.M, G.M, cnt)));
      return 0;
    };
    if (nb_main > 0) {
      const long long mk = c.sc.mark();
      double* Linv = c.sc.get<double>(nb_main * mm);
      if (G.M > 256) {
        const long long wsb = gpsa_chol_inv_blocked_workspace(G.M, nb_main);
        void* ws = c.sc.get<char>(wsb);
        if (!sel) {
          GPSA_RUN(gpsa_chol_inv_blocked_f64(c.mats(G, 0), Linv, G.M, nb_main, logdet, info, ws, wsb, c.stv()));
        } else {
          if (np > 0)
            GPSA_RUN(gpsa_chol_inv_blocked_f64(c.mats(G, 0), Linv, G.M, np, logdet, info, ws, wsb, c.stv()));
          if (n_own > 0)
            GPSA_RUN(gpsa_chol_inv_blocked_f64(c.mats(G, np + G.own_lo), Linv + (long long)(np + G.own_lo) * mm, G.M,
                                               n_own, logdet + np + G.own_lo, info + np + G.own_lo, ws, wsb, c.stv()));
        }
      } else if (!sel) {
        GPSA_RUN(gpsa_chol_inv_f64(c.mats(G, 0), Linv, G.M, nb_main, logdet, info, c.stv()));
      } else {
        GPSA_RUN(gpsa_chol_inv_sel_f64(c.mats(G, 0), Linv, G.M, nb_main, np, np + G.own_lo, np + G.own_hi, logdet, info,
                                       c.stv()));
      }
      if (!sel) {
        GPSA_CK(inverse_product(Linv, c.inv(G, 0), nb_main));
      } else if (G.own_lo == 0) {
        GPSA_CK(inverse_product(Linv, c.inv(G, 0), np + n_own));
      } else {
        GPSA_CK(inverse_product(Linv, c.inv(G, 0), np));
        GPSA_CK(inverse_product(Linv + (long long)(np + G.own_lo) * mm, c.inv(G, np + G.own_lo), n_own));
      }
      c.sc.release(mk);
    }
  }
  if (kl)
    for (int g = 0; g < P.ng; ++g) {
      Group& G = P.grp[g];
      if (G.n_omega > 0)
        GPSA_RUN(mvn_kl_grouped_fwd_copy(c.mats(G, 0), c.inv(G, 0), c.sv<double>(G.o_logdet), G.om_idx, G.pr_idx,
                                         c.sv<double>(G.o_D), G.M, G.n_omega, c.io.kl + G.kl_off,
                                         c.sv<double>(G.o_KD), c.sv<double>(P.o_klcache) + G.kl_off, klpart[g], klcnt[g],
                                         c.st));
    }
  return 0;
}

static ModPtrs mod_ptrs(Ctx& c, const gpsa_step_out_grads* og, const double* const* dG64) {
  ModPtrs p;
  memset(&p, 0, sizeof(p));
  for (int m = 0; m < c.P.nm; ++m) {
    p.X[m] = c.io.X[m];
    p.Gm[m] = c.io.G_means[m];
    p.Gs[m] = c.io.G_samples[m];
    p.G64[m] = c.sv<double>(c.P.o_G64[m]);
    p.N[m] = c.P.d.n_rows[m];
    if (og != nullptr) {
      p.dGm[m] = og->dG_means[m];
      p.dGs[m] = og->dG_samples[m];
    }
    if (dG64 != nullptr) p.dG64[m] = dG64[m];
  }
  return p;
}

static int project_views(Ctx& c, const double* Kinv, const double* Kuf, int M, long long Cs, double* alpha,
                         double* q, int cnt, int b0, bool packed) {
  const bool dry = c.dry;
  const long long wsb1 = gpsa_whiten_workspace(M);
  if (wsb1 > 0) {
    void* ws = c.sv<char>(c.P.o_apk_w) + wsb1 * b0;
    GPSA_RUN(gpsa_whiten_batched_f64(packed ? nullptr : Kinv, (long long)M * M, Kuf, M, Cs, (long long)M * Cs, alpha, q,
                                     cnt, ws, wsb1 * cnt, c.stv()));
    return 0;
  }
  GPSA_CK(gemm64(c, 0, 0, M, (int)Cs, M, 1.0, Kinv, M, (long long)M * M, Kuf, Cs, (long long)M * Cs, 0.0, alpha,
                 Cs, (long long)M * Cs, cnt, 1));
  if (q != nullptr && !dry) {
    dim3 grid((unsigned)cdiv(Cs, 256), (unsigned)cnt);
    coldot2_kernel<<<grid, 256, 0, c.st>>>(Kuf, alpha, M, Cs, q);
    GPSA_LAUNCH_CHECK();
  }
  return 0;
}

static int warp_stage_fwd(Ctx& c) {
  Plan& P = c.P;
  const bool dry = c.dry;
  const int V = P.V, D = P.D, Mx = P.Mx, nf = P.nf;
  const long long Cs = P.Cs;
  Group& GW = P.gw();
  (void)V;
  const long long mk = c.sc.mark();
  double* meanT = nullptr;
  double* vq = nullptr;
  double* q = nullptr;
  if (nf > 0 && Cs > 0) {
    float* Xv = c.sv<float>(P.o_Xv);
    double* alpha = c.sv<double>(P.o_alpha_w);
    double* Wk = c.sv<double>(P.o_Wk);
    meanT = c.sc.get<double>((long long)nf * D * Cs);
    vq = c.sc.get<double>((long long)nf * D * Cs);
    q = c.sc.get<double>((long long)nf * Cs);
    double* Kuf = c.sc.get<double>((long long)nf * Mx * Cs);
    if (!dry) {
      dim3 grid((unsigned)cdiv(Cs, 256), (unsigned)nf);
      warp_gather_kernel<<<grid, 256, 0, c.st>>>(P.tab, P.d_free, mod_ptrs(c, nullptr, nullptr), Xv);
      GPSA_LAUNCH_CHECK();
    }
    for (const Run& r : P.runs) {
      long long nlive[KM_MAXB_STEP];
      for (int i = 0; i < r.cnt; ++i) nlive[i] = P.nview[r.v0 + i];
      GPSA_RUN(gpsa_kmat_batched(P.d.kind_warp, c.prm.Xtilde + (long long)r.v0 * Mx * D, (long long)Mx * D, Mx,
                                 Xv + (long long)r.b0 * Cs * D, Cs * D, Cs, D, c.prm.warp_ls + r.v0,
                                 c.prm.warp_var + r.v0, 1, nlive, r.cnt, 0.0, Kuf + (long long)r.b0 * Mx * Cs,
                                 (long long)Mx * Cs, c.stv()));
      GPSA_CK(project_views(c, c.inv(GW, P.pos_Kw(r.b0)), Kuf + (long long)r.b0 * Mx * Cs, Mx, Cs,
                            alpha + (long long)r.b0 * Mx * Cs, q + (long long)r.b0 * Cs, r.cnt, r.b0, false));
      GPSA_RUN(gpsa_quadform_fwd_keep_batched_f64(
          alpha + (long long)r.b0 * Mx * Cs, c.mats(GW, P.pos_OmG(r.v0 * D)), Mx, Cs, D,
          vq + (long long)r.b0 * D * Cs, Wk + (long long)r.b0 * D * Mx * Cs,
          c.sv<double>(P.o_resid) + (long long)r.v0 * Mx * D, meanT + (long long)r.b0 * D * Cs, r.cnt, c.stv()));
    }
  }
  int* bad = c.sv<int>(P.o_bad);
  long long boff = 0;
  for (int m = 0; m < P.nm; ++m) {
    const long long N = P.d.n_rows[m];
    if (N == 0) continue;
    const long long nb = cdiv(N, 256);
    if (!dry) {
      warp_sample_views_fwd_kernel<<<(unsigned)nb, 256, 0, c.st>>>(
          P.tab, m, c.io.X[m], meanT, vq, q, c.prm.warp_var, c.prm.slopes, c.prm.intercepts, c.io.eps_G, N,
          c.io.G_means[m], c.io.G_samples[m], c.sv<double>(P.o_G64[m]), bad + boff);
      GPSA_LAUNCH_CHECK();
    }
    boff += nb;
  }
  c.sc.release(mk);
  if (c.io.flag != nullptr && !dry) {
    Group& G0 = P.grp[0];
    const int n0 = P.d.want_kl ? G0.nb() : G0.n_prior;
    flag_reduce_kernel<<<1, 256, 0, c.st>>>(c.sv<int>(G0.o_info), n0, bad, P.nbad, c.io.flag);
    GPSA_LAUNCH_CHECK();
    if (P.ng == 2) {
      Group& G1 = P.grp[1];
      const int n1 = P.d.want_kl ? G1.nb() : G1.n_prior;
      flag_reduce_kernel<<<1, 256, 0, c.st>>>(c.sv<int>(G1.o_info), n1, c.io.flag, 1, c.io.flag);
      GPSA_LAUNCH_CHECK();
    }
  }
  return 0;
}

static int data_pass_fwd(Ctx& c, const Pass& ps) {
  Plan& P = c.P;
  const bool dry = c.dry;
  const int m = ps.m, Mg = P.Mg, D = P.D, L = P.d.n_latent[m], Pm = P.d.n_out[m];
  const long long C = ps.C;
  Group& GD = P.gd();
  const double* Kinv = c.inv(GD, P.pos_KF());
  const double* Om = c.mats(GD, P.pos_OmF(m, 0));
  float* alpha = c.sv<float>(ps.o_alpha);
  float* Sigma = c.sv<float>(ps.o_sigma);
  const float* eps = ps.test ? c.io.eps_F_test[m] : c.io.eps_F[m];
  float* F = ps.test ? c.io.F_latent_test[m] : c.io.F_latent[m];
  float* Fo = ps.test ? c.io.F_obs_test[m] : c.io.F_obs[m];
  const long long mk = c.sc.mark();
  double* q = c.sc.get<double>(C);
  {
    const long long mk2 = c.sc.mark();
    double* Kuf = c.sc.get<double>((long long)Mg * C);
    const long long wsb = gpsa_whiten_workspace(Mg);
    const bool exact = ps.o_alpha64 >= 0;
    bool fused = false;
    if (!ps.test && exact && wsb > 0 && !dry) {
      if (c.sc.overflow) return GPSA_EWORKSPACE;
      const int rc = gpsa_whiten_gen_f64_dual(c.apk_d ? nullptr : Kinv, P.d.kind_data, c.prm.Gtilde,
                                              c.sv<double>(P.o_G64[m]), D, c.prm.data_ls, c.prm.data_var, Mg, C,
                                              c.sv<double>(ps.o_alpha64), alpha, q, c.sv<char>(P.o_apk_d), wsb, c.stv());
      if (rc == 0) fused = true, c.apk_d = true;
      else if (rc != GPSA_EUNSUPPORTED) return rc;
    }
    if (!fused) {
      if (ps.test)
        GPSA_RUN(gpsa_kmat(GPSA_F64, GPSA_F32, P.d.kind_data, c.prm.Gtilde, Mg, c.io.G_test[m], C, D, c.prm.data_ls,
                           c.prm.data_var, 0.0, Kuf, c.stv()));
      else
        GPSA_RUN(gpsa_kmat(GPSA_F64, GPSA_F32_X64, P.d.kind_data, c.prm.Gtilde, Mg, c.sv<double>(P.o_G64[m]), C, D,
                           c.prm.data_ls, c.prm.data_var, 0.0, Kuf, c.stv()));
      if (wsb > 0 && !exact) {
        void* ws = c.sv<char>(P.o_apk_d);
        GPSA_RUN(gpsa_whiten_f64(c.apk_d ? nullptr : Kinv, GPSA_F64, Kuf, Mg, C, GPSA_F32, alpha, q, ws, wsb,
                                 c.stv()));
        c.apk_d = true;
      } else if (wsb > 0) {
        void* ws = c.sv<char>(P.o_apk_d);
        double* a64 = c.sv<double>(ps.o_alpha64);
        GPSA_RUN(gpsa_whiten_f64_dual(c.apk_d ? nullptr : Kinv, Kuf, Mg, C, a64, alpha, q, ws, wsb, c.stv()));
        c.apk_d = true;
      } else {
        double* a64 = exact ? c.sv<double>(ps.o_alpha64) : c.sc.get<double>((long long)Mg * C);
        GPSA_CK(gemm64(c, 0, 0, Mg, (int)C, Mg, 1.0, Kinv, Mg, 0, Kuf, C, 0, 0.0, a64, C, 0, 1, 1));
        if (!dry) {
          coldot2_kernel<<<dim3((unsigned)cdiv(C, 256), 1), 256, 0, c.st>>>(Kuf, a64, Mg, C, q);
          GPSA_LAUNCH_CHECK();
          convert_kernel_step<double, float><<<(unsigned)cdiv((long long)Mg * C, 256), 256, 0, c.st>>>(
              a64, (long long)Mg * C, alpha);
          GPSA_LAUNCH_CHECK();
        }
      }
    }
    c.sc.release(mk2);
  }
  float* meanT = c.sc.get<float>((long long)L * C);
  float* v = c.sc.get<float>((long long)L * C);
  const bool mean_in_product = ps.fused(c.io) && gpsa_quadform_elbo_takes_delta(Mg) != 0;
  if (!mean_in_product)
    GPSA_CK(gemm32(c, 1, 0, L, (int)C, Mg, 1.0, c.prm.delta_F[m], L, 0, alpha, C, 0, 0.0, meanT, C, 0, 1, 1));
  if (ps.fused(c.io)) {
    if (c.io.noise_u[m] == nullptr || c.io.ll_part[m] == nullptr) return GPSA_EINVAL;
    float* g_ext = c.sv<float>(ps.o_fuse);
    float* dmeanT = g_ext + (long long)(L + 1) * C;
    float* abar = dmeanT + (long long)L * C;
// ... 108 lines not shown
static int data_pass_bwd(Ctx& c, const Pass& ps, int pass_idx, const float* dFl_in, const float* dFo_in,
                         BwdBufs& B, const gpsa_step_param_grads& out, bool first_for_mod, const float* gloss) {
  Plan& P = c.P;
  const bool dry = c.dry;
  const int m = ps.m, Mg = P.Mg, D = P.D, L = P.d.n_latent[m], Pm = P.d.n_out[m];
  const long long C = ps.C, mm = (long long)Mg * Mg;
  Group& GD = P.gd();
  const double* Kinv = c.inv(GD, P.pos_KF());
  const double* Om = c.mats(GD, P.pos_OmF(m, 0));
  double* dOm = B.dstack[P.merged ? 0 : 1] + (long long)P.pos_OmF(m, 0) * mm;
  double* dKuu = B.dstack[P.merged ? 0 : 1] + (long long)P.pos_KF() * mm;
  const float* alpha = c.sv<float>(ps.o_alpha);
  const float* Sigma = c.sv<float>(ps.o_sigma);
  const float* eps = ps.test ? c.io.eps_F_test[m] : c.io.eps_F[m];
  const float* F = ps.test ? c.io.F_latent_test[m] : c.io.F_latent[m];
  const long long mk = c.sc.mark();
  const float* dFl = dFl_in;
  if (P.d.has_lmc[m] && dFo_in != nullptr) {
    float* buf = c.sc.get<float>(C * L);
    if (dFl_in != nullptr) GPSA_RUN(copy_async(buf, dFl_in, (size_t)(C * L * 4), c.st));
    GPSA_CK(gemm32(c, 0, 1, (int)C, L, Pm, 1.0, dFo_in, Pm, 0, c.prm.W[m], Pm, 0, dFl_in != nullptr ? 1.0 : 0.0, buf, L,
                   0, 1, 1));
    if (out.W[m] != nullptr)
      GPSA_CK(gemm32(c, 1, 0, L, Pm, C, 1.0, F, L, 0, dFo_in, Pm, 0, first_for_mod ? 0.0 : 1.0, out.W[m], Pm, 0, 1,
                     splitk_for(C, L, Pm)));
    dFl = buf;
  } else if (!P.d.has_lmc[m] && dFo_in != nullptr && dFl_in != nullptr && dFo_in != dFl_in) {
    return GPSA_EINVAL;
  } else if (dFl == nullptr) {
    dFl = dFo_in;
  }
  const bool fusedp = ps.fused(c.io);
  float* g_ext = fusedp ? c.sv<float>(ps.o_fuse) : c.sc.get<float>((long long)(L + 1) * C);
  float* dmeanT = fusedp ? g_ext + (long long)(L + 1) * C : c.sc.get<float>((long long)L * C);
  float* qbar = g_ext + (long long)L * C;
  if (!fusedp) {
    const long long wsb = 8 * (C / 32 + 2);
    void* ws = c.sc.get<char>(wsb);
    GPSA_RUN(gpsa_data_sample_bwd(dFl, eps, Sigma, c.prm.data_var, C, L, g_ext, dmeanT, qbar, GPSA_F64,
                                  B.dvar_ds + pass_idx, ws, wsb, c.stv()));
  }
  float* abar = fusedp ? dmeanT + (long long)L * C : c.sc.get<float>((long long)Mg * C);
  if (fusedp) {
    if (gloss == nullptr) return GPSA_EINVAL;
    const long long wsb = 8 * (C / 256 + 2);
    void* ws = c.sc.get<char>(wsb);
    const bool timed = !dry && !c.quiet && &ps == &P.passes[0];
    if (timed) P.tick(1, 0, false, c.st);
    if (pass_idx < BWD_TICKS - 32)
      GPSA_RUN(elbo_fused_post_ticket(g_ext, dmeanT, abar, Mg, C, L, gloss, c.prm.data_var, B.dvar_ds + pass_idx,
                                      (double*)ws, B.tick + 32 + pass_idx, c.st));
    else
      GPSA_RUN(gpsa_elbo_fused_post(g_ext, dmeanT, abar, Mg, C, L, gloss, c.prm.data_var, GPSA_F64,
                                    B.dvar_ds + pass_idx, ws, wsb, c.stv()));
    GPSA_CK(thin_update(c, c.prm.delta_F[m], Mg, L, dmeanT, C, abar));
    if (timed) P.tick(1, 1, false, c.st);
  } else {
    const long long wsb = gpsa_quadform_workspace(GPSA_F32, Mg, C, L);
    const long long mk2 = c.sc.mark();
    void* ws = c.sc.get<char>(wsb);
    const bool timed = !dry && !c.quiet && &ps == &P.passes[0];
    if (timed) P.tick(1, 0, false, c.st);
    const bool kept = c.io.keep_products && ps.o_keep >= 0;
    if (kept)
      GPSA_RUN(gpsa_quadform_bwd_alpha_kept_f32(c.sv<float>(ps.o_keep), g_ext, Mg, C, L, c.prm.delta_F[m], dmeanT, abar,
                                                c.stv()));
    else
      GPSA_RUN(gpsa_quadform_bwd_alpha(GPSA_F32, GPSA_F64, alpha, Om, g_ext, Mg, C, L, abar, ws, wsb, c.stv()));
    if (timed) P.tick(1, 1, false, c.st);
    c.sc.release(mk2);
    if (!kept) GPSA_CK(thin_update(c, c.prm.delta_F[m], Mg, L, dmeanT, C, abar));
  }
  const bool ddelta_in_gram = gpsa_quadform_bwd_omega_takes_delta(Mg, C) != 0;
  if (!ddelta_in_gram)
    GPSA_CK(gemm32(c, 0, 1, Mg, L, C, 1.0, alpha, C, 0, dmeanT, C, 0, first_for_mod ? 0.0 : 1.0, B.ddc_F[m], L, 0, 1,
                   splitk_for(C, Mg, L)));
  B.have_ddc[m] = true;
  const bool exact = ps.o_alpha64 >= 0;
  double* gamma64 = nullptr;
  if (exact) {
    const double* a64 = c.sv<double>(ps.o_alpha64);
    gamma64 = c.sc.get<double>((long long)Mg * C);
    const long long wsb = gpsa_whiten_workspace(Mg);
    if (wsb > 0) {
      GPSA_RUN(gpsa_whiten_f64(nullptr, GPSA_F32, abar, Mg, C, GPSA_F64, gamma64, nullptr, c.sv<char>(P.o_apk_d), wsb,
                               c.stv()));
    } else {
      const long long mk2 = c.sc.mark();
      double* abar64 = c.sc.get<double>((long long)Mg * C);
      if (!dry) {
        convert_kernel_step<float, double><<<(unsigned)cdiv((long long)Mg * C, 256), 256, 0, c.st>>>(
            abar, (long long)Mg * C, abar64);
        GPSA_LAUNCH_CHECK();
      }
      GPSA_CK(gemm64(c, 0, 0, Mg, (int)C, Mg, 1.0, Kinv, Mg, 0, abar64, C, 0, 0.0, gamma64, C, 0, 1, 1));
      c.sc.release(mk2);
    }
    {
      const double* Gs[1] = {gamma64};
      const double* Bs[1] = {a64};
      const void* ds[1] = {qbar};
      const double al[1] = {-1.0}, be[1] = {1.0};
      double* os[1] = {dKuu};
      int rc = longk(c, 1, Gs, Bs, ds, GPSA_F32, Mg, C, C, 0, al, be, os);
      if (rc == GPSA_EUNSUPPORTED || (dry && rc == 0)) {
        const long long wsb2 = gpsa_exact_dkuu_workspace(Mg, C);
        const long long mk2 = c.sc.mark();
        void* ws2 = c.sc.get<char>(wsb2);
        GPSA_RUN(gpsa_exact_dkuu_f64(gamma64, a64, qbar, Mg, C, dKuu, ws2, wsb2, c.stv()));
        c.sc.release(mk2);
      } else if (rc != 0) {
        return rc;
      }
    }
    if (ps.test) {
      const long long mk2 = c.sc.mark();
      double* qbar64 = c.sc.get<double>(C);
      double* W64 = c.sc.get<double>((long long)Mg * C);
      if (!dry) {
        convert_kernel_step<float, double><<<(unsigned)cdiv(C, 256), 256, 0, c.st>>>(qbar, C, qbar64);
        GPSA_LAUNCH_CHECK();
        dim3 grid((unsigned)cdiv(C, 256), (unsigned)((Mg < 64) ? Mg : 64));
        exact_axpy2_kernel<<<grid, 256, 0, c.st>>>(gamma64, a64, qbar64, Mg, C, W64, gamma64);
        GPSA_LAUNCH_CHECK();
      }
      c.sc.release(mk2);
    }
  }
  const bool cov_early = exact && !ps.test;
  if (cov_early) {
    const long long mk2 = c.sc.mark();
    const long long wsb = gpsa_kmat_bwd_workspace(GPSA_F64, Mg, C, D);
    void* ws = c.sc.get<char>(wsb);
    GPSA_RUN(gpsa_kmat_bwd_x64_f64_axpy(P.d.kind_data, c.prm.Gtilde, Mg, c.sv<double>(P.o_G64[m]), C, D, c.prm.data_ls,
                                        c.prm.data_var, gamma64, c.sv<double>(ps.o_alpha64), qbar, 2.0,
                                        B.dZ_df + (long long)pass_idx * Mg * D, B.dG64[m],
                                        B.dpar_df + (long long)pass_idx * 2, ws, wsb, c.stv()));
    B.have_dG[m] = true;
    c.sc.release(mk2);
  }
  float* gamma = exact ? nullptr : c.sc.get<float>((long long)Mg * C);
  const bool identity = !exact && C >= 4LL * L * Mg;
  bool axpy_in_cov = false;
  if (!exact) {
    const long long wsb = gpsa_whiten_workspace(Mg);
    if (wsb > 0) {
      const long long mk2 = c.sc.mark();
      void* ws = c.sv<char>(P.o_apk_d);
      GPSA_RUN(gpsa_whiten_f64(nullptr, GPSA_F32, abar, Mg, C, GPSA_F32, gamma, nullptr, ws, wsb, c.stv()));
      c.sc.release(mk2);
    } else {
      GPSA_CK((gemmx<double, float, float>(c, 0, 0, Mg, (int)C, Mg, 1.0, Kinv, Mg, 0, abar, C, 0, 0.0, gamma, C, 0, 1, 1)));
    }
  }
  {
    const long long mk2 = c.sc.mark();
    long long wsb = gpsa_quadform_workspace(GPSA_F32, Mg, C, L);
    if (ps.gx3 && gpsa_quadform_bwd_omega_x3_workspace(Mg, C, L) > wsb) wsb = gpsa_quadform_bwd_omega_x3_workspace(Mg, C, L);
    void* ws = c.sc.get<char>(wsb);
    double* dst = first_for_mod ? dOm : c.sc.get<double>((long long)L * mm);
    const bool timed = !dry && !c.quiet && &ps == &P.passes[0];
    if (timed) P.tick(2, 0, false, c.st);
    int rc = 0;
    if (dry) {
      const long long mk3 = c.sc.mark();
      if (ddelta_in_gram)
        GPSA_CK(gemm32(c, 0, 1, Mg, L, C, 1.0, alpha, C, 0, dmeanT, C, 0, 0.0, B.ddc_F[m], L, 0, 1, splitk_for(C, Mg, L)));
      c.sc.get<float>((long long)L * mm);
      c.sc.release(mk3);
    }
    if (!dry && ddelta_in_gram) {
      rc = ps.gx3 ? gpsa_quadform_bwd_omega_delta_x3(GPSA_F64, alpha, g_ext, dmeanT, Mg, C, L, dst, B.ddc_F[m],
                                                     first_for_mod ? 0.0 : 1.0, ws, wsb, c.stv())
                  : gpsa_quadform_bwd_omega_delta_f32(GPSA_F64, alpha, g_ext, dmeanT, Mg, C, L, dst, B.ddc_F[m],
                                                      first_for_mod ? 0.0 : 1.0, ws, wsb, c.stv());
      if (rc == GPSA_EUNSUPPORTED) {
        GPSA_CK(gemm32(c, 0, 1, Mg, L, C, 1.0, alpha, C, 0, dmeanT, C, 0, first_for_mod ? 0.0 : 1.0, B.ddc_F[m], L, 0, 1,
                       splitk_for(C, Mg, L)));
        rc = ps.gx3 ? gpsa_quadform_bwd_omega_x3(GPSA_F32, GPSA_F64, alpha, g_ext, Mg, C, L, dst, ws, wsb, c.stv())
                    : gpsa_quadform_bwd_omega(GPSA_F32, GPSA_F64, alpha, g_ext, Mg, C, L, dst, ws, wsb, c.stv());
      }
    } else if (!dry) {
      rc = ps.gx3 ? gpsa_quadform_bwd_omega_x3(GPSA_F32, GPSA_F64, alpha, g_ext, Mg, C, L, dst, ws, wsb, c.stv())
                  : gpsa_quadform_bwd_omega(GPSA_F32, GPSA_F64, alpha, g_ext, Mg, C, L, dst, ws, wsb, c.stv());
    }
    if (rc == GPSA_EUNSUPPORTED) {
      float* tmp = c.sc.get<float>((long long)L * mm);
      GPSA_RUN(gpsa_quadform_bwd_omega(GPSA_F32, GPSA_F32, alpha, g_ext, Mg, C, L, tmp, ws, wsb, c.stv()));
      if (!dry) {
        convert_kernel_step<float, double><<<(unsigned)cdiv((long long)L * mm, 256), 256, 0, c.st>>>(
            tmp, (long long)L * mm, dst);
        GPSA_LAUNCH_CHECK();
      }
    } else if (rc != 0) {
      return rc;
    }
    if (timed) { P.tick(2, 1, false, c.st); ++P.tbwd; }
    if (dry) (void)c.sc.get<float>((long long)L * mm);
    if (!first_for_mod && !dry) {
      add_inplace_kernel<<<(unsigned)cdiv((long long)L * mm, 256), 256, 0, c.st>>>(dOm, dst, (long long)L * mm);
      GPSA_LAUNCH_CHECK();
    }
    if (identity) {
      double* Pm_ = c.sc.get<double>(mm);
      float* ddc_p = B.ddc_F[m];
      if (!first_for_mod) {
        ddc_p = c.sc.get<float>((long long)Mg * L);
        GPSA_CK(gemm32(c, 0, 1, Mg, L, C, 1.0, alpha, C, 0, dmeanT, C, 0, 0.0, ddc_p, L, 0, 1, splitk_for(C, Mg, L)));
      }
      GPSA_CK(gemm64(c, 1, 0, Mg, Mg, (long long)L * Mg, 2.0, Om, Mg, 0, dst, Mg, 0, 0.0, Pm_, Mg, 0, 1,
                     splitk_for((long long)L * Mg, Mg, Mg)));
      GPSA_CK((gemmx<float, float, double>(c, 0, 1, Mg, Mg, L, 1.0, c.prm.delta_F[m], L, 0, ddc_p, L, 0, 1.0, Pm_, Mg, 0,
                                           1, 1)));
      double* sumOm = c.sc.get<double>(mm);
      if (!dry) {
        reduce_rows_kernel<double, double><<<(unsigned)cdiv(mm, 64), 256, 0, c.st>>>(dst, L, mm, mm, sumOm, 1.0);
        GPSA_LAUNCH_CHECK();
      }
      GPSA_CK(gemm64(c, 0, 0, Mg, Mg, Mg, -1.0, Kinv, Mg, 0, Pm_, Mg, 0, 1.0, sumOm, Mg, 0, 1, splitk_small(Mg, Mg, Mg, 1)));
      if (!dry) {
        add_inplace_kernel<<<(unsigned)cdiv(mm, 256), 256, 0, c.st>>>(dKuu, sumOm, mm);
        GPSA_LAUNCH_CHECK();
      }
      if (ps.test)
        GPSA_RUN(gpsa_col_axpy(GPSA_F32, gamma, alpha, qbar, 2.0, Mg, C, gamma, c.stv()));
      else
        axpy_in_cov = true;
    } else if (!exact) {
      GPSA_RUN(gpsa_col_axpy(GPSA_F32, gamma, alpha, qbar, 1.0, Mg, C, gamma, c.stv()));
      GPSA_CK((gemmx<float, float, double>(c, 0, 1, Mg, Mg, C, -1.0, gamma, C, 0, alpha, C, 0, 1.0, dKuu, Mg, 0, 1,
                                           splitk_for(C, Mg, Mg))));
      GPSA_RUN(gpsa_col_axpy(GPSA_F32, gamma, alpha, qbar, 1.0, Mg, C, gamma, c.stv()));
    }
    c.sc.release(mk2);
  }
  if (!cov_early) {
    const long long wsb = gpsa_kmat_bwd_workspace(GPSA_F64, Mg, C, D);
    void* ws = c.sc.get<char>(wsb);
    double* dZ = B.dZ_df + (long long)pass_idx * Mg * D;
    double* dpar = B.dpar_df + (long long)pass_idx * 2;
    if (exact && ps.test) {
      GPSA_RUN(gpsa_kmat_bwd(GPSA_F64, GPSA_F32_OUT64, P.d.kind_data, c.prm.Gtilde, Mg, c.io.G_test[m], C, D,
                             c.prm.data_ls, c.prm.data_var, gamma64, 0, dZ, nullptr, dpar, ws, wsb, c.stv()));
    } else if (exact) {
      GPSA_RUN(gpsa_kmat_bwd_x64_f64_axpy(P.d.kind_data, c.prm.Gtilde, Mg, c.sv<double>(P.o_G64[m]), C, D, c.prm.data_ls,
                                          c.prm.data_var, gamma64, c.sv<double>(ps.o_alpha64), qbar, 2.0, dZ, B.dG64[m],
                                          dpar, ws, wsb, c.stv()));
      B.have_dG[m] = true;
    } else if (ps.test) {
      GPSA_RUN(gpsa_kmat_bwd(GPSA_F64, GPSA_F32_ACC64, P.d.kind_data, c.prm.Gtilde, Mg, c.io.G_test[m], C, D,
                             c.prm.data_ls, c.prm.data_var, gamma, 0, dZ, nullptr, dpar, ws, wsb, c.stv()));
    } else {
      GPSA_RUN(gpsa_kmat_bwd_x64_axpy(P.d.kind_data, c.prm.Gtilde, Mg, c.sv<double>(P.o_G64[m]), C, D, c.prm.data_ls,
                                      c.prm.data_var, gamma, axpy_in_cov ? alpha : nullptr, axpy_in_cov ? qbar : nullptr,
                                      2.0, dZ, B.dG64[m], dpar, ws, wsb, c.stv()));
      B.have_dG[m] = true;
    }
  }
  c.sc.release(mk);
  return 0;
}

static int warp_stage_bwd(Ctx& c, const gpsa_step_out_grads& og, BwdBufs& B, bool acc) {
  Plan& P = c.P;
  const bool dry = c.dry;
  const int D = P.D, Mx = P.Mx, nf = P.nf;
  const long long Cs = P.Cs, mm = (long long)Mx * Mx;
  Group& GW = P.gw();
  if (nf == 0 || Cs == 0) return 0;
  const long long mk = c.sc.mark();
  const float* Xv = c.sv<float>(P.o_Xv);
  const double* alpha = c.sv<double>(P.o_alpha_w);
  const double* Wk = c.sv<double>(P.o_Wk);
  double* dmeanT = c.sc.get<double>((long long)nf * D * Cs);
  double* g = c.sc.get<double>((long long)nf * D * Cs);
  double* qbar = c.sc.get<double>((long long)nf * Cs);
  const long long nblk = cdiv(Cs, 256);
  double* part = c.sc.get<double>((long long)nf * nblk);
  if (!dry) {
    const double* dG64[MAXMODS];
    for (int m = 0; m < MAXMODS; ++m) dG64[m] = (m < P.nm && B.have_dG[m]) ? B.dG64[m] : nullptr;
    dim3 grid((unsigned)nblk, (unsigned)nf);
    const bool closes = nf <= 32;
    warp_sample_views_bwd_kernel<<<grid, 256, 0, c.st>>>(P.tab, P.d_free, mod_ptrs(c, &og, dG64), c.io.eps_G, dmeanT,
                                                         g, qbar, part, closes ? B.tick : nullptr, c.prm.warp_var,
                                                         B.dvar_ws);
    GPSA_LAUNCH_CHECK();
    if (!closes) {
      warp_sample_views_bwd_finish_kernel<<<nf, 64, 0, c.st>>>(part, nblk, P.d_free, c.prm.warp_var, B.dvar_ws);
      GPSA_LAUNCH_CHECK();
    }
  }
  double* abar = c.sc.get<double>((long long)nf * Mx * Cs);
  double* gamma = c.sc.get<double>((long long)nf * Mx * Cs);
  for (const Run& r : P.runs) {
    const long long oMC = (long long)r.b0 * Mx * Cs, oDC = (long long)r.b0 * D * Cs;
    const double* resid = c.sv<double>(P.o_resid) + (long long)r.v0 * Mx * D;
    GPSA_RUN(gpsa_quadform_bwd_alpha_kept_batched_f64(Wk + (long long)r.b0 * D * Mx * Cs, g + oDC, Mx, Cs, D, resid,
                                                      dmeanT + oDC, abar + oMC, r.cnt, c.stv()));
    GPSA_CK(gemm64(c, 0, 1, Mx, D, Cs, 1.0, alpha + oMC, Cs, (long long)Mx * Cs, dmeanT + oDC, Cs, (long long)D * Cs,
                   0.0, B.dresid + (long long)r.v0 * Mx * D, D, (long long)Mx * D, r.cnt, splitk_for(Cs, Mx, D)));
    GPSA_CK(project_views(c, c.inv(GW, P.pos_Kw(r.b0)), abar + oMC, Mx, Cs, gamma + oMC, nullptr, r.cnt, r.b0, true));
    bool done = false;
    if (r.cnt * D <= 48 && gpsa_longk_f64_workspace(Mx, Cs, r.cnt * D) > 0 && gpsa_longk_f64_workspace(Mx, Cs, r.cnt) > 0) {
      const double *Gs[48], *Bs[48];
      const void* ds[48];
      double al[48], be[48];
      double* os[48];
      int n = 0;
      for (int i = 0; i < r.cnt; ++i)
        for (int jj = 0; jj < D; ++jj, ++n) {
          Gs[n] = nullptr;
          Bs[n] = alpha + oMC + (long long)i * Mx * Cs;
          ds[n] = g + oDC + ((long long)i * D + jj) * Cs;
          al[n] = 1.0;
          be[n] = acc ? 1.0 : 0.0;
          os[n] = B.dstack[0] + ((long long)P.pos_OmG((r.v0 + i) * D + jj)) * mm;
        }
      int rc = longk(c, n, nullptr, Bs, ds, GPSA_F64, Mx, Cs, Cs, 1, al, be, os);
      if (rc == 0) {
        for (int i = 0; i < r.cnt; ++i) {
          Gs[i] = gamma + oMC + (long long)i * Mx * Cs;
          Bs[i] = alpha + oMC + (long long)i * Mx * Cs;
          ds[i] = qbar + (long long)(r.b0 + i) * Cs;
          al[i] = -1.0;
          be[i] = acc ? 1.0 : 0.0;
          os[i] = B.dstack[0] + (long long)P.pos_Kw(r.b0 + i) * mm;
        }
        rc = longk(c, r.cnt, Gs, Bs, ds, GPSA_F64, Mx, Cs, Cs, 0, al, be, os);
        if (rc != 0) return rc == GPSA_EUNSUPPORTED ? GPSA_EINVAL : rc;
        GPSA_RUN(gpsa_col_axpy_batched_f64(gamma + oMC, alpha + oMC, qbar + (long long)r.b0 * Cs, 2.0, Mx, Cs,
                                           gamma + oMC, r.cnt, c.stv()));
        done = true;
      } else if (rc != GPSA_EUNSUPPORTED) {
        return rc;
      }
    }
    if (!done || dry) {
      if (acc && !dry) return GPSA_EINVAL;
      {
        const long long mk2 = c.sc.mark();
        const long long wsb = gpsa_gram_batched_workspace(Mx, Cs, D, r.cnt);
        void* ws = c.sc.get<char>(wsb);
        GPSA_RUN(gpsa_gram_batched_f64(alpha + oMC, g + oDC, Mx, Cs, D, B.dstack[0] + (long long)P.pos_OmG(r.v0 * D) * mm,
                                       r.cnt, ws, wsb, c.stv()));
        c.sc.release(mk2);
      }
      GPSA_RUN(gpsa_col_axpy_batched_f64(gamma + oMC, alpha + oMC, qbar + (long long)r.b0 * Cs, 1.0, Mx, Cs, gamma + oMC,
                                         r.cnt, c.stv()));
      GPSA_CK(gemm64(c, 0, 1, Mx, Mx, Cs, -1.0, gamma + oMC, Cs, (long long)Mx * Cs, alpha + oMC, Cs, (long long)Mx * Cs,
                     0.0, B.dstack[0] + (long long)P.pos_Kw(r.b0) * mm, Mx, mm, r.cnt, splitk_for(Cs, Mx, Mx)));
      GPSA_RUN(gpsa_col_axpy_batched_f64(gamma + oMC, alpha + oMC, qbar + (long long)r.b0 * Cs, 1.0, Mx, Cs, gamma + oMC,
                                         r.cnt, c.stv()));
    }
    {
      const long long mk2 = c.sc.mark();
      long long nlive[KM_MAXB_STEP];
      for (int i = 0; i < r.cnt; ++i) nlive[i] = P.nview[r.v0 + i];
      const long long wsb = gpsa_kmat_bwd_batched_workspace(Mx, Cs, D, r.cnt);
      void* ws = c.sc.get<char>(wsb);
      GPSA_RUN(gpsa_kmat_bwd_batched(P.d.kind_warp, c.prm.Xtilde + (long long)r.v0 * Mx * D, (long long)Mx * D, Mx,
                                     Xv + (long long)r.b0 * Cs * D, Cs * D, Cs, D, c.prm.warp_ls + r.v0,
                                     c.prm.warp_var + r.v0, 1, nlive, r.cnt, gamma + oMC, (long long)Mx * Cs, 0,
                                     B.dZ_wf + (long long)r.b0 * Mx * D, (long long)Mx * D,
                                     B.dpar_wf + (long long)r.b0 * 2, ws, wsb, c.stv()));
      c.sc.release(mk2);
    }
  }
  c.sc.release(mk);
  return 0;
}

static bool warp_runs_longk(const Plan& P) {
  for (const Run& r : P.runs)
    if (!(r.cnt * P.D <= 48 && gpsa_longk_f64_workspace(P.Mx, P.Cs, r.cnt * P.D) > 0 &&
          gpsa_longk_f64_workspace(P.Mx, P.Cs, r.cnt) > 0))
      return false;
  return true;
}

static int step_backward(Plan& P, const gpsa_step_params& prm, const gpsa_step_io& io,
                         const gpsa_step_out_grads& og, char* saved, Arena& sc, const gpsa_step_param_grads& out,
                         hipStream_t st) {
  Ctx c{P, prm, io, saved, sc, st, sc.dry};
  const bool dry = c.dry;
  const int V = P.V, D = P.D, Mx = P.Mx, Mg = P.Mg, nf = P.nf, npass = (int)P.passes.size();
  BwdBufs B;
  memset(&B, 0, sizeof(B));
  const bool kl = P.d.want_kl != 0 && og.dkl != nullptr;
  for (int g = 0; g < P.ng; ++g) {
    Group& G = P.grp[g];
    B.dD[g] = sc.get<double>((long long)G.n_omega * G.M);
  }
  const long long z0 = (sc.off + 255) & ~255LL;
  for (int g = 0; g < P.ng; ++g) {
    Group& G = P.grp[g];
    B.dstack[g] = sc.get<double>((long long)G.nb() * G.M * G.M);
  }
  const long long nwz = (long long)(nf > 0 ? nf : 1) * Mx * D;
  B.dZ_wf = sc.get<double>(nwz);
  B.dpar_wf = sc.get<double>(2LL * (nf > 0 ? nf : 1));
  B.dvar_ws = sc.get<double>(nf > 0 ? nf : 1);
  B.dresid = sc.get<double>((long long)V * Mx * D);
  B.dZ_df = sc.get<double>((long long)(npass > 0 ? npass : 1) * Mg * D);
  B.dpar_df = sc.get<double>(2LL * (npass > 0 ? npass : 1));
  B.dvar_ds = sc.get<double>(npass > 0 ? npass : 1);
  B.tick = sc.get<int>(BWD_TICKS);
  const long long zf = sc.off;
  sc.get<char>(256);
  const long long z1 = (sc.off + 255) & ~255LL;
  if (!dry) GPSA_CK(zero_fill_async(sc.base + z0, (size_t)(z1 - z0), st));
  if (dry) {
    long long ab = z1 - z0;
    for (int m = 0; m < P.nm; ++m) ab += ((long long)Mg * P.d.n_latent[m] * 4 + 255) & ~255LL;
    for (int m = 0; m < P.nm; ++m)
      if (P.d.has_lmc[m]) ab += ((long long)P.d.n_latent[m] * P.d.n_out[m] * 4 + 255) & ~255LL;
    P.bwd_acc_bytes = ab + 256;
  }
  B.dZ_wu = sc.get<double>(nwz);
  B.dpar_wu = sc.get<double>(2LL * (nf > 0 ? nf : 1));
  B.dZ_du = sc.get<double>((long long)Mg * D); B.dpar_du = sc.get<double>(2);
  for (int m = 0; m < P.nm; ++m) {
    B.ddc_F[m] = sc.get<float>((long long)Mg * P.d.n_latent[m]);
    B.dG64[m] = sc.get<double>((long long)P.S * P.d.n_rows[m] * D);
  }
  bool seen[MAXMODS] = {false, false, false, false};
  for (int pi = 0; pi < npass; ++pi) {
    const Pass& ps = P.passes[pi];
    const float* dFl = ps.test ? og.dF_latent_test[ps.m] : og.dF_latent[ps.m];
    const float* dFo = ps.test ? og.dF_obs_test[ps.m] : og.dF_obs[ps.m];
    if (dFl == nullptr && dFo == nullptr && !ps.fused(io)) continue;
    GPSA_CK(data_pass_bwd(c, ps, pi, dFl, dFo, B, out, !seen[ps.m], og.gloss));
    seen[ps.m] = true;
  }
  const bool early = io.f_event != nullptr && !dry && (io.bwd_acc == nullptr || io.bwd_acc_mode == 0) &&
                     warp_runs_longk(P);
  if (!early) GPSA_CK(warp_stage_bwd(c, og, B, false));
  if (io.bwd_acc_mode != 0 && io.bwd_acc != nullptr && !dry) {
    char* accb = reinterpret_cast<char*>(io.bwd_acc);
    const long long nD = (zf - z0) / 8;
    double* rD = reinterpret_cast<double*>(sc.base + z0);
    double* aD = reinterpret_cast<double*>(accb);
    long long aoff = z1 - z0;
    if (io.bwd_acc_mode == 1) {
      GPSA_CK(copy_async(aD, rD, (size_t)(nD * 8), st));
    } else {
      double* dst = io.bwd_acc_mode == 2 ? aD : rD;
      const double* src = io.bwd_acc_mode == 2 ? rD : aD;
      add_inplace_kernel<<<(unsigned)cdiv(nD, 256), 256, 0, st>>>(dst, src, nD);
      GPSA_LAUNCH_CHECK();
    }
    for (int m = 0; m < P.nm; ++m) {
      const long long n = (long long)Mg * P.d.n_latent[m];
      float* a = reinterpret_cast<float*>(accb + aoff);
      aoff += (n * 4 + 255) & ~255LL;
      if (!B.have_ddc[m]) {
        if (io.bwd_acc_mode == 1) GPSA_CK(zero_fill_async(a, (size_t)(n * 4), st));
        continue;
      }
      if (io.bwd_acc_mode == 1) {
        GPSA_CK(copy_async(a, B.ddc_F[m], (size_t)(n * 4), st));
      } else {
        add_inplace_f32_kernel<<<(unsigned)cdiv(n, 256), 256, 0, st>>>(io.bwd_acc_mode == 2 ? a : B.ddc_F[m],
                                                                        io.bwd_acc_mode == 2 ? B.ddc_F[m] : a, n);
        GPSA_LAUNCH_CHECK();
      }
    }
    for (int m = 0; m < P.nm; ++m) {
      if (!P.d.has_lmc[m]) continue;
      const long long n = (long long)P.d.n_latent[m] * P.d.n_out[m];
      float* a = reinterpret_cast<float*>(accb + aoff);
      aoff += (n * 4 + 255) & ~255LL;
      if (out.W[m] == nullptr) continue;
      if (io.bwd_acc_mode == 1) {
        GPSA_CK(copy_async(a, out.W[m], (size_t)(n * 4), st));
      } else {
        add_inplace_f32_kernel<<<(unsigned)cdiv(n, 256), 256, 0, st>>>(io.bwd_acc_mode == 2 ? a : out.W[m],
                                                                        io.bwd_acc_mode == 2 ? out.W[m] : a, n);
        GPSA_LAUNCH_CHECK();
      }
    }
    if (io.bwd_acc_mode != 3) return 0;
  }
  auto kl_backward = [&]() -> int {
    for (int g = 0; g < P.ng && kl; ++g) {
      Group& G = P.grp[g];
      if (G.n_omega == 0 || G.n_prior == 0) continue;
      const long long mm = (long long)G.M * G.M;
      const long long mk = sc.mark();
      double* S = sc.get<double>((long long)G.n_prior * mm);
      double* T1 = sc.get<double>((long long)G.n_prior * mm);
      GPSA_RUN(gpsa_mvn_kl_grouped_bwd_acc(c.mats(G, 0), c.inv(G, 0), G.om_idx, G.pr_list, G.grp_off, G.order,
                                           c.sv<double>(G.o_D), c.sv<double>(G.o_KD), og.dkl + G.kl_off, G.M, G.n_omega,
                                           G.n_prior, B.dstack[g] + (long long)G.n_prior * mm, B.dD[g], S, 1, c.stv()));
      GPSA_CK(gemm64(c, 0, 0, G.M, G.M, G.M, 1.0, c.inv(G, 0), G.M, mm, S, G.M, mm, 0.0, T1, G.M, mm, G.n_prior,
                     splitk_few(G.M, G.M, G.M, G.n_prior)));
      GPSA_CK(gemm64(c, 0, 0, G.M, G.M, G.M, 0.5, T1, G.M, mm, c.inv(G, 0), G.M, mm, 1.0, B.dstack[g], G.M, mm, G.n_prior,
                     splitk_few(G.M, G.M, G.M, G.n_prior)));
      sc.release(mk);
    }
    return 0;
  };
  auto priors_backward = [&]() -> int {
    {
      for (const Run& r : P.runs) {
        const long long mk = sc.mark();
        const long long wsb = gpsa_kmat_bwd_batched_workspace(Mx, Mx, D, r.cnt);
        void* ws = sc.get<char>(wsb);
        GPSA_RUN(gpsa_kmat_bwd_batched(P.d.kind_warp, prm.Xtilde + (long long)r.v0 * Mx * D, (long long)Mx * D, Mx,
                                       prm.Xtilde + (long long)r.v0 * Mx * D, (long long)Mx * D, Mx, D, prm.warp_ls + r.v0,
                                       prm.warp_var + r.v0, 1, nullptr, r.cnt,
                                       B.dstack[0] + (long long)P.pos_Kw(r.b0) * Mx * Mx, (long long)Mx * Mx, 1,
                                       B.dZ_wu + (long long)r.b0 * Mx * D, (long long)Mx * D, B.dpar_wu + (long long)r.b0 * 2,
                                       ws, wsb, c.stv()));
        sc.release(mk);
      }
      {
        const long long mk = sc.mark();
        const long long wsb = gpsa_kmat_bwd_batched_workspace(Mg, Mg, D, 1);
        void* ws = sc.get<char>(wsb);
        GPSA_RUN(gpsa_kmat_bwd_batched(P.d.kind_data, prm.Gtilde, 0, Mg, prm.Gtilde, 0, Mg, D, prm.data_ls, prm.data_var, 0,
                                       nullptr, 1, B.dstack[P.merged ? 0 : 1] + (long long)P.pos_KF() * Mg * Mg, 0, 1,
                                       B.dZ_du, 0, B.dpar_du, ws, wsb, c.stv()));
        sc.release(mk);
      }
    }
    return 0;
  };
  auto omega_backward = [&](int which) -> int {
    int m_first = 0;
    if ((which & 1) && out.Omega_sqt_G != nullptr) {
      if ((which & 2) && Mx == Mg && P.nm > 0 && out.Omega_sqt_F[0] != nullptr) {
        m_first = 1;
        GPSA_RUN(gpsa_omega_bwd2(B.dstack[0] + (long long)P.pos_OmG(0) * Mx * Mx, prm.Omega_sqt_G, out.Omega_sqt_G, V * D,
                                 B.dstack[P.merged ? 0 : 1] + (long long)P.pos_OmF(0, 0) * Mg * Mg, prm.Omega_sqt_F[0],
                                 out.Omega_sqt_F[0], P.d.n_latent[0], Mx, 1, c.stv()));
      } else {
        GPSA_RUN(gpsa_omega_bwd(B.dstack[0] + (long long)P.pos_OmG(0) * Mx * Mx, prm.Omega_sqt_G, Mx, V * D, 1,
                                out.Omega_sqt_G, c.stv()));
      }
    }
    if (which & 2)
      for (int m = m_first; m < P.nm; ++m)
        if (out.Omega_sqt_F[m] != nullptr)
          GPSA_RUN(gpsa_omega_bwd(B.dstack[P.merged ? 0 : 1] + (long long)P.pos_OmF(m, 0) * Mg * Mg, prm.Omega_sqt_F[m], Mg,
                                  P.d.n_latent[m], 1, out.Omega_sqt_F[m], c.stv()));
    return 0;
  };
  auto finalize = [&](int part) -> int {
    FinalArgs a;
    memset(&a, 0, sizeof(a));
    a.part = part;
    a.V = V; a.D = D; a.Mx = Mx; a.Mg = Mg; a.nm = P.nm; a.nf = nf; a.npass = npass;
    a.bidx = P.tab.bidx;
    a.slopes = prm.slopes;
    a.dZ_wf = B.dZ_wf; a.dZ_wu = B.dZ_wu; a.dpar_wf = B.dpar_wf; a.dpar_wu = B.dpar_wu; a.dvar_ws = B.dvar_ws;
    a.dresid = B.dresid;
    a.dD_w = kl ? B.dD[0] : nullptr;
    a.dZ_df = B.dZ_df; a.dpar_df = B.dpar_df; a.dvar_ds = B.dvar_ds; a.dZ_du = B.dZ_du; a.dpar_du = B.dpar_du;
    a.dD_d = kl ? (P.merged ? B.dD[0] + (long long)V * D * Mx : B.dD[1]) : nullptr;
    const long long nsmall = (long long)V * Mx * D + 2LL * V + (long long)Mg * D + 2;
    long long nF = 0;
    for (int m = 0; m < P.nm; ++m) {
      a.ddc_F[m] = B.have_ddc[m] ? B.ddc_F[m] : nullptr;
      a.L[m] = P.d.n_latent[m];
      a.Loff[m] = P.Loff[m];
      nF += (long long)Mg * P.d.n_latent[m];
    }
    a.out = out;
    if (part != 1 && io.loss_src != nullptr && io.loss_dst != nullptr) {
      a.loss_src = io.loss_src;
      a.loss_dst = io.loss_dst;
    }
    const long long tot = part == 1 ? nF : (part == 2 ? nsmall : nsmall + nF);
    if (!dry && tot > 0) {
      step_finalize_kernel<<<(unsigned)cdiv(tot, 256), 256, 0, st>>>(a);
      GPSA_LAUNCH_CHECK();
    }
    return 0;
  };
  if (early) {
    ++P.n_early;
    GPSA_CK(kl_backward());
    GPSA_CK(omega_backward(2));
    GPSA_CK(finalize(1));
    GPSA_CK((int)hipEventRecord(reinterpret_cast<hipEvent_t>(io.f_event), st));
    GPSA_CK(warp_stage_bwd(c, og, B, true));
    GPSA_CK(priors_backward());
    GPSA_CK(omega_backward(1));
    GPSA_CK(finalize(2));
  } else {
    GPSA_CK(kl_backward());
    GPSA_CK(priors_backward());
    GPSA_CK(omega_backward(3));
    GPSA_CK(finalize(0));
    if (io.f_event != nullptr && !dry) GPSA_CK((int)hipEventRecord(reinterpret_cast<hipEvent_t>(io.f_event), st));
  }
  return 0;
}

}

namespace gpsa {

static bool graph_usable(Plan& P, hipStream_t st) {
  if (P.g_enabled < 0) {
    const char* e = getenv("GPSA_STEP_GRAPH");
    P.g_enabled = (e && e[0] == '1') ? 1 : 0;
  }
  if (!P.g_enabled || P.tslots != 0 || P.g_idle_captures > 8) return false;
  for (int m = 0; m < P.nm; ++m)
    if (P.lik[m] != GPSA_LIK_GAUSSIAN) return false;
  hipStreamCaptureStatus cs = hipStreamCaptureStatusNone;
  if (hipStreamIsCapturing(st, &cs) != hipSuccess || cs != hipStreamCaptureStatusNone) return false;
  return true;
}

template <typename F>
static int graph_call(Plan& P, const Plan::GraphKey& key, hipStream_t st, F&& enqueue) {
  ++P.gtick;
  for (size_t i = 0; i < P.retired.size();) {
    if (hipEventQuery(P.retired[i].ev) == hipSuccess) {
      (void)hipGraphExecDestroy(P.retired[i].exec);
      (void)hipEventDestroy(P.retired[i].ev);
      P.retired.erase(P.retired.begin() + (long)i);
    } else {
      (void)hipGetLastError();
      ++i;
    }
  }
  for (auto& ge : P.graphs)
    if (memcmp(ge.key.b, key.b, Plan::GraphKey::BYTES) == 0) {
      if (ge.used == 0) P.g_idle_captures = 0;
      ge.used = P.gtick;
      ge.last = st;
      ++P.g_hits;
      return (int)hipGraphLaunch(ge.exec, st);
    }
  bool met = false;
  for (auto& k : P.seen)
    if (memcmp(k.b, key.b, Plan::GraphKey::BYTES) == 0) { met = true; break; }
  if (!met) {
    static const bool dbg = [] { const char* e = getenv("GPSA_STEP_GRAPH_DEBUG"); return e && e[0] == '1'; }();
    if (dbg) {
      for (size_t q = P.seen.size(); q-- > 0;) {
        const Plan::GraphKey& o = P.seen[q];
        if (o.bwd() != key.bwd() || o.stages() != key.stages()) continue;
        fprintf(stderr, "[step graph] %s stages %d differs from its last sighting at bytes:", key.bwd() ? "bwd" : "fwd",
                key.stages());
        for (size_t i = 0; i < Plan::GraphKey::BYTES; i += 8)
          if (memcmp(o.b + i, key.b + i, 8) != 0) fprintf(stderr, " %zu", i);
        fprintf(stderr, "  [io at %zu, og at %zu, pg at %zu, arenas at %zu]\n", Plan::GraphKey::O_IO, Plan::GraphKey::O_OG,
                Plan::GraphKey::O_PG, Plan::GraphKey::O_PTR);
        break;
      }
    }
    if (P.seen.size() >= 96) P.seen.erase(P.seen.begin());
    P.seen.push_back(key);
    ++P.g_eager;
    return enqueue(st);
  }
  if (P.gstream == nullptr && hipStreamCreateWithFlags(&P.gstream, hipStreamNonBlocking) != hipSuccess) {
    P.gstream = nullptr;
    (void)hipGetLastError();
    P.g_enabled = 0;
    ++P.g_eager;
    return enqueue(st);
  }
  if (hipStreamBeginCapture(P.gstream, hipStreamCaptureModeThreadLocal) != hipSuccess) {
    (void)hipGetLastError();
    P.g_enabled = 0;
    ++P.g_eager;
    return enqueue(st);
  }
  const int rc = enqueue(P.gstream);
  hipGraph_t g = nullptr;
  const hipError_t ec = hipStreamEndCapture(P.gstream, &g);
  if (rc != 0 || ec != hipSuccess || g == nullptr) {
    if (g != nullptr) (void)hipGraphDestroy(g);
    (void)hipGetLastError();
// ... 306 lines not shown
```

Before: 150.9.

## Merge symmetric and general long-K f64 products into one mixed launch with row strips

The warp-layer backward used to launch two long-K reduction kernels: a symmetric one for the D Omega-gradient products and a general one for the Kw products. They are now combined into a single mixed launch. Each problem carries its own symmetry and has-G flags, and a planner splits tall outputs into row strips and chooses K-splits so the workgroups fill the CUs. This removes one kernel launch and its separate reduce, and balances work across more workgroups. In exchange it adds more complex indexing, a runtime GM dispatch branch, and a different partial-buffer layout.

Measured after the change: 150.9 (median of 3 runs). No clear change (-0.0%).

```diff
diff --git a/include/gpsa_hip.h b/include/gpsa_hip.h
--- a/include/gpsa_hip.h
+++ b/include/gpsa_hip.h
@@ -216,6 +216,16 @@
 int gpsa_longk_f64(int nprob, const double* const* G, const double* const* B, const void* const* d, int d_dtype,
                    int M, long long K, long long ld, int sym, const double* alpha, const double* beta,
                    double* const* out, void* workspace, long long workspace_bytes, void* stream);
+int gpsa_longk_f64_plan(int nprob, const int* sym, int M, long long K, int cus, int* rs, int* ns,
+                        long long* workspace_bytes);
+long long gpsa_longk_f64_plan_workspace(int nprob, const int* sym, int M, long long K, const int* rs, const int* ns);
+int gpsa_longk_f64_strip(int M, int sym, int rs, int s, int* row0, int* row1);
+int gpsa_longk_f64_slice(long long K, int ns, int t, long long* g0, long long* g1);
+long long gpsa_longk_f64_mixed_workspace(int nprob, const int* sym, int M, long long K);
+int gpsa_longk_f64_mixed(int nprob, const int* sym, const double* const* G, const double* const* B,
+                         const void* const* d, int d_dtype, int M, long long K, long long ld, const double* alpha,
+                         const double* beta, double* const* out, const int* plan_rs, const int* plan_ns,
+                         void* workspace, long long workspace_bytes, void* stream);
 int gpsa_kmat_bwd_x64_axpy(int kind, const float* Z, int M, const double* X, long long C, int D, const float* ls_u,
                            const float* var_u, const float* Kbar, const float* X2, const float* d, double s,
                            double* dZ, double* dX, double* dparams, void* workspace, long long workspace_bytes,
diff --git a/spatial_alignment_amd/_lib.py b/spatial_alignment_amd/_lib.py
--- a/spatial_alignment_amd/_lib.py
+++ b/spatial_alignment_amd/_lib.py
@@ -131,6 +131,12 @@
     "gpsa_exact_dkuu_f64": (_i, [_vp, _vp, _vp, _i, _ll, _vp, _vp, _ll, _vp]),
     "gpsa_longk_f64_workspace": (_ll, [_i, _ll, _i]),
     "gpsa_longk_f64": (_i, [_i, _vp, _vp, _vp, _i, _i, _ll, _ll, _i, _vp, _vp, _vp, _vp, _ll, _vp]),
+    "gpsa_longk_f64_plan": (_i, [_i, _vp, _i, _ll, _i, _vp, _vp, _vp]),
+    "gpsa_longk_f64_plan_workspace": (_ll, [_i, _vp, _i, _ll, _vp, _vp]),
+    "gpsa_longk_f64_strip": (_i, [_i, _i, _i, _i, _vp, _vp]),
+    "gpsa_longk_f64_slice": (_i, [_ll, _i, _i, _vp, _vp]),
+    "gpsa_longk_f64_mixed_workspace": (_ll, [_i, _vp, _i, _ll]),
+    "gpsa_longk_f64_mixed": (_i, [_i, _vp, _vp, _vp, _vp, _i, _i, _ll, _ll, _vp, _vp, _vp, _vp, _vp, _vp, _ll, _vp]),
     "gpsa_kmat_bwd_x64_axpy": (_i, [_i, _vp, _i, _vp, _ll, _i, _vp, _vp, _vp, _vp, _vp, _d, _vp, _vp, _vp, _vp, _ll,
                                     _vp]),
     "gpsa_thin_update_f32": (_i, [_vp, _i, _i, _vp, _ll, _vp, _vp]),
diff --git a/spatial_alignment_amd/csrc/longk64.hip b/spatial_alignment_amd/csrc/longk64.hip
--- a/spatial_alignment_amd/csrc/longk64.hip
+++ b/spatial_alignment_amd/csrc/longk64.hip
@@ -12,14 +12,58 @@
 
 constexpr int LK_WAVES = 8;
 constexpr int LK_MAXP = 48;
+constexpr int LK_MAXWG = 384;
+constexpr unsigned LK_NOWG = 0xffffffffu;
+constexpr int LK_LONG = 21;
+
+__host__ __device__ constexpr int lk_tri(int i) { return i * (i + 1) / 2; }
+
+__host__ __device__ constexpr int lk_cut(int MB, int rs, int s, bool sym) {
+  if (s <= 0) return 0;
+  if (s >= rs) return MB;
+  int prev = 0;
+  for (int q = 1; q <= s; ++q) {
+    int c = (q * MB + rs / 2) / rs;
+    if (sym) {
+      const int want = q * lk_tri(MB);
+      int best = -1;
+      for (int i = 0; i <= MB; ++i) {
+        const int e = lk_tri(i) * rs > want ? lk_tri(i) * rs - want : want - lk_tri(i) * rs;
+        if (best < 0 || e < best) {
+          best = e;
+          c = i;
+        }
+      }
+    }
+    const int lo = prev + 1, hi = MB - (rs - q);
+    c = c < lo ? lo : (c > hi ? hi : c);
+    prev = c;
+  }
+  return prev;
+}
+__host__ __device__ constexpr int lk_strip_tiles(int MB, int rs, int s, bool sym) {
+  const int a = lk_cut(MB, rs, s, sym), b = lk_cut(MB, rs, s + 1, sym);
+  return sym ? lk_tri(b) - lk_tri(a) : (b - a) * MB;
+}
+__host__ __device__ constexpr int lk_nt(int MB, int rs, bool sym) {
+  int m = 0;
+  for (int s = 0; s < rs; ++s) {
+    const int t = lk_strip_tiles(MB, rs, s, sym);
+    m = t > m ? t : m;
+  }
+  return (m + LK_WAVES - 1) / LK_WAVES;
+}
 
 struct LongKArgs {
   const double* G[LK_MAXP];
   const double* B[LK_MAXP];
   const void* d[LK_MAXP];
+  long long pbase[LK_MAXP];
+  unsigned meta[LK_MAXP];
+  unsigned wg[LK_MAXWG];
   double* part;
-  int M, nprob, nsplit, sym;
-  long long K, ld, gper;
+  int M;
+  long long K, ld;
 };
 
 __device__ __forceinline__ void lk_set_m0(unsigned lds_base) {
@@ -34,56 +78,63 @@
   asm volatile("global_load_lds_dword %0, off offset:%1" ::"v"(gsrc_minus_imm), "n"(IMM) : "memory");
 }
 
-template <int MB, bool HASG, int DT>
-__global__ void __launch_bounds__(512) longk64_kernel(LongKArgs a) {
+template <int MB, int SC, bool STRIPS, bool HASG, int DT>
+__device__ __forceinline__ void longk64_body(const LongKArgs& a, const int p, const int i0s_, const int i1s_,
+                                             const int sp, const bool sym, char* lk_smem) {
   static_assert(HASG || DT != 0, "a left operand");
-  constexpr int MP = MB * 16;
   constexpr int NOPD = HASG ? 2 : 1;
   constexpr int NPIECE = MB * NOPD * 2;
   constexpr int NPW = (NPIECE + LK_WAVES - 1) / LK_WAVES;
   static_assert(NPW <= 8, "two groups of four pieces per wave (an immediate offset reaches 4 KiB)");
   constexpr int DAREA = DT == 2 ? 1024 : 256;
   constexpr int STAGE_B = NPW * LK_WAVES * 1024 + (DT ? LK_WAVES * DAREA : 0);
-  constexpr int NT_MAX = (MB * MB + LK_WAVES - 1) / LK_WAVES;
-  constexpr int NT_SYM = (MB * (MB + 1) / 2 + LK_WAVES - 1) / LK_WAVES;
-  extern __shared__ __attribute__((aligned(16))) char lk_smem[];
+  constexpr int NT_MAX = lk_nt(MB, SC, false);
+  constexpr int NT_SYM = lk_nt(MB, SC, true);
 
   const int tid = threadIdx.x, lane = tid & 63;
   const int w = __builtin_amdgcn_readfirstlane(tid >> 6);
   const int li = lane & 15, kq = lane >> 4;
-  const int p = blockIdx.y, sp = blockIdx.x;
   const int M = a.M;
   const long long K = a.K, ld = a.ld;
   const double* __restrict__ Bp = a.B[p];
   const double* __restrict__ Gp = HASG ? a.G[p] : nullptr;
+  const int i0s = STRIPS ? i0s_ : 0, i1s = STRIPS ? i1s_ : MB;
+  const int nb = (STRIPS && sym) ? i1s : MB;
+  const int nbp = 2 * nb, npc = nbp + (HASG ? 2 * (i1s - i0s) : 0);
   const long long ng = (K + 15) >> 4;
-  const long long g_lo = (long long)sp * a.gper;
-  long long g_hi = g_lo + a.gper;
-  if (g_hi > ng) g_hi = ng;
+  const int ns = a.meta[p] & 0xffff;
+  const long long g_lo = sp * ng / ns, g_hi = (sp + 1) * ng / ns;
   const unsigned lds0 = (unsigned)(unsigned long long)(lk_lds_ptr)(&lk_smem[0]);
 
-  const int T = a.sym ? MB * (MB + 1) / 2 : MB * MB;
+  const int T = sym ? lk_tri(i1s) - lk_tri(i0s) : (i1s - i0s) * MB;
   const int t_lo = w * T / LK_WAVES, t_hi = (w + 1) * T / LK_WAVES;
   const int cnt = t_hi - t_lo;
-  int i0 = 0, j0 = 0;
-  if (a.sym) {
-    while ((i0 + 1) * (i0 + 2) / 2 <= t_lo) ++i0;
-    j0 = t_lo - i0 * (i0 + 1) / 2;
+  const int nt_run = (T + LK_WAVES - 1) / LK_WAVES;
+  int i0 = i0s, j0 = 0;
+  if (sym) {
+    const int tg = lk_tri(i0s) + t_lo;
+    while (lk_tri(i0 + 1) <= tg) ++i0;
+    j0 = tg - lk_tri(i0);
   } else {
-    i0 = t_lo / MB;
-    j0 = t_lo - i0 * MB;
-  }
-  if (cnt == 0) i0 = j0 = 0;
+    i0 = i0s + t_lo / MB;
+    j0 = t_lo - (i0 - i0s) * MB;
+  }
+  if (cnt == 0) {
+    i0 = i0s;
+    j0 = 0;
+  }
 
   const double* rp[NPW];
   int koff[NPW];
+  bool live[NPW];
 #pragma unroll
   for (int u = 0; u < NPW; ++u) {
     int q = w + LK_WAVES * u;
-    q = q < NPIECE ? q : NPIECE - 1;
-    const int h = q & 1, ot = q >> 1;
-    const bool isg = HASG && ot >= MB;
-    const int t = isg ? ot - MB : ot;
+    live[u] = !STRIPS || q < npc;
+    q = q < npc ? q : npc - 1;
+    const int h = q & 1;
+    const bool isg = HASG && q >= nbp;
+    const int t = isg ? i0s + ((q - nbp) >> 1) : q >> 1;
     int row = t * 16 + li;
     row = row < M ? row : M - 1;
     rp[u] = (isg ? Gp : Bp) + (long long)row * ld;
@@ -99,11 +150,13 @@
       long long k = kb + koff[u];
       k = k < K - 2 ? k : K - 2;
       const char* src = reinterpret_cast<const char*>(rp[u] + k);
-      switch (u & 3) {
-        case 0: lk_glds16<0>(src); break;
-        case 1: lk_glds16<1024>(src - 1024); break;
-        case 2: lk_glds16<2048>(src - 2048); break;
-        default: lk_glds16<3072>(src - 3072); break;
+      if (live[u]) {
+        switch (u & 3) {
+          case 0: lk_glds16<0>(src); break;
+          case 1: lk_glds16<1024>(src - 1024); break;
+          case 2: lk_glds16<2048>(src - 2048); break;
+          default: lk_glds16<3072>(src - 3072); break;
+        }
       }
     }
     if (DT != 0) {
@@ -150,23 +203,23 @@
           dv[h][1] = x.y;
         }
       }
-#define LK_FRAG(O, TL, H)                                                                              \
-  (*reinterpret_cast<const lk_f64x2*>(slot + ((((((O) * MB + (TL)) * 2 + (H)) & 7) * NPW +             \
-                                                 ((((O) * MB + (TL)) * 2 + (H)) >> 3)) << 10) + lane * 16))
+#define LK_PIECE(Q) (*reinterpret_cast<const lk_f64x2*>(slot + (((((Q) & 7) * NPW + ((Q) >> 3))) << 10) + lane * 16))
+#define LK_FRAG_B(TL, H) LK_PIECE((TL) * 2 + (H))
+#define LK_FRAG_G(TL, H) LK_PIECE(nbp + ((TL) - i0s) * 2 + (H))
       int i = i0, j = j0, cur = -1;
       double af[2][2] = {{0.0, 0.0}, {0.0, 0.0}};
-      lk_f64x2 bn0 = LK_FRAG(0, j, 0), bn1 = LK_FRAG(0, j, 1);
+      lk_f64x2 bn0 = LK_FRAG_B(j, 0), bn1 = LK_FRAG_B(j, 1);
 #pragma unroll
       for (int t = 0; t < NT_MAX; ++t) {
-        if (t >= NT_SYM && a.sym) break;
+        if (t >= NT_SYM && t >= nt_run) break;
         if (i != cur) {
           cur = i;
 #pragma unroll
           for (int h = 0; h < 2; ++h) {
-            const lk_f64x2 bi = LK_FRAG(0, i, h);
+            const lk_f64x2 bi = LK_FRAG_B(i, h);
             double x0, x1;
             if (HASG) {
-              const lk_f64x2 gi = LK_FRAG(1, i, h);
+              const lk_f64x2 gi = LK_FRAG_G(i, h);
               x0 = DT ? fma(dv[h][0], bi.x, gi.x) : gi.x;
               x1 = DT ? fma(dv[h][1], bi.y, gi.y) : gi.y;
             } else {
@@ -180,55 +233,83 @@
         const lk_f64x2 b0 = bn0, b1 = bn1;
         if (t + 1 < cnt) {
           ++j;
-          if (a.sym ? j > i : j == MB) {
+          if (sym ? j > i : j == MB) {
             ++i;
             j = 0;
           }
         }
         if (t + 1 < NT_MAX) {
-          bn0 = LK_FRAG(0, j, 0);
-          bn1 = LK_FRAG(0, j, 1);
+          bn0 = LK_FRAG_B(j, 0);
+          bn1 = LK_FRAG_B(j, 1);
         }
         acc[t] = __builtin_amdgcn_mfma_f64_16x16x4f64(af[0][0], b0.x, acc[t], 0, 0, 0);
         acc[t] = __builtin_amdgcn_mfma_f64_16x16x4f64(af[0][1], b0.y, acc[t], 0, 0, 0);
         acc[t] = __builtin_amdgcn_mfma_f64_16x16x4f64(af[1][0], b1.x, acc[t], 0, 0, 0);
         acc[t] = __builtin_amdgcn_mfma_f64_16x16x4f64(af[1][1], b1.y, acc[t], 0, 0, 0);
       }
-#undef LK_FRAG
+#undef LK_FRAG_G
+#undef LK_FRAG_B
+#undef LK_PIECE
       s ^= 1;
     }
   }
-  double* __restrict__ out = a.part + ((long long)p * a.nsplit + sp) * MP * MP;
-  int i = i0, j = j0;
+  const long long before = sym ? lk_tri(i0s) : i0s * MB;
+  double* __restrict__ out = a.part + a.pbase[p] + ((long long)ns * before + (long long)sp * T) * 256;
 #pragma unroll
   for (int t = 0; t < NT_MAX; ++t) {
     if (t < cnt) {
 #pragma unroll
-      for (int r = 0; r < 4; ++r) out[(long long)(i * 16 + kq + 4 * r) * MP + j * 16 + li] = acc[t][r];
-      ++j;
-      if (a.sym ? j > i : j == MB) {
-        ++i;
-        j = 0;
-      }
-    }
+      for (int r = 0; r < 4; ++r) out[(long long)(t_lo + t) * 256 + (kq + 4 * r) * 16 + li] = acc[t][r];
+    }
+  }
+}
+
+template <int MB, int SC, bool STRIPS, int GM, int DT>
+__global__ void __launch_bounds__(512) longk64_kernel(LongKArgs a) {
+  extern __shared__ __attribute__((aligned(16))) char lk_smem[];
+  const unsigned e = a.wg[blockIdx.x];
+  if (e == LK_NOWG) return;
+  const int p = e & 63, i0 = (e >> 6) & 31, i1 = (e >> 11) & 31, sp = e >> 16;
+  const unsigned meta = a.meta[p];
+  const bool sym = (meta >> 16 & 1) != 0;
+  if constexpr (GM == 1) {
+    longk64_body<MB, SC, STRIPS, true, DT>(a, p, i0, i1, sp, sym, lk_smem);
+  } else if constexpr (GM == 0) {
+    longk64_body<MB, SC, STRIPS, false, DT>(a, p, i0, i1, sp, sym, lk_smem);
+  } else {
+    if (meta >> 16 & 2)
+      longk64_body<MB, SC, STRIPS, true, DT>(a, p, i0, i1, sp, sym, lk_smem);
+    else
+      longk64_body<MB, SC, STRIPS, false, DT>(a, p, i0, i1, sp, sym, lk_smem);
   }
 }
 
 struct LongKOut {
   double* out[LK_MAXP];
   double alpha[LK_MAXP], beta[LK_MAXP];
+  long long pbase[LK_MAXP];
+  unsigned meta[LK_MAXP];
 };
 
-__global__ void __launch_bounds__(256)
-longk64_reduce_kernel(const double* __restrict__ part, int M, int MP, int nsplit, int sym, LongKOut o) {
+__global__ void __launch_bounds__(256) longk64_reduce_kernel(const double* __restrict__ part, int M, int MB, LongKOut o) {
   __shared__ double red[4][64];
   const int lane = threadIdx.x & 63, grp = threadIdx.x >> 6;
   const int p = blockIdx.y;
+  const unsigned meta = o.meta[p];
+  const bool sym = (meta >> 16 & 1) != 0;
+  const int nsplit = meta & 0xffff, rs = meta >> 24;
   const long long e = blockIdx.x * 64LL + lane;
   const int r = (int)(e / M), c = (int)(e % M);
   const bool ok = e < (long long)M * M && !(sym && c > r);
-  const long long mm = (long long)MP * MP;
-  const double* q = part + (long long)p * nsplit * mm + (long long)r * MP + c;
+  const int i = ok ? r >> 4 : 0, j = ok ? c >> 4 : 0;
+  int st = 0;
+  while (st + 1 < rs && lk_cut(MB, rs, st + 1, sym) <= i) ++st;
+  const int i0 = lk_cut(MB, rs, st, sym), i1 = lk_cut(MB, rs, st + 1, sym);
+  const long long T = sym ? lk_tri(i1) - lk_tri(i0) : (i1 - i0) * MB;
+  const long long before = sym ? lk_tri(i0) : i0 * MB;
+  const long long tile = sym ? lk_tri(i) - lk_tri(i0) + j : (long long)(i - i0) * MB + j;
+  const long long mm = T * 256;
+  const double* q = part + o.pbase[p] + nsplit * before * 256 + tile * 256 + (r & 15) * 16 + (c & 15);
   double a0 = 0.0, a1 = 0.0, a2 = 0.0, a3 = 0.0;
   if (ok) {
     int s = grp;
@@ -271,96 +352,287 @@
   return (int)(s < 1 ? 1 : s);
 }
 
-template <int MB, bool HASG, int DT>
-static int longk64_launch_mb(const LongKArgs& a, hipStream_t st) {
-  constexpr int NPIECE = MB * (HASG ? 2 : 1) * 2, NPW = (NPIECE + LK_WAVES - 1) / LK_WAVES;
+static inline int lk_tiles(int MB, bool sym) { return sym ? lk_tri(MB) : MB * MB; }
+
+static int lk_plan(int nprob, const int* sym, int MB, long long K, int cus, int* rs, int* ns) {
+  int tmin = MB * MB;
+  for (int p = 0; p < nprob; ++p) tmin = lk_tiles(MB, sym[p] != 0) < tmin ? lk_tiles(MB, sym[p] != 0) : tmin;
+  long long units = 0;
+  for (int p = 0; p < nprob; ++p) {
+    int r = 1;
+    while (r < 4 && 2 * r <= MB) {
+      int m = 0;
+      for (int s = 0; s < r; ++s) {
+        const int t = lk_strip_tiles(MB, r, s, sym[p] != 0);
+        m = t > m ? t : m;
+      }
+      if (m <= tmin) break;
+      r *= 2;
+    }
+    rs[p] = r;
+    units += r;
+  }
+  if (cus > LK_MAXWG) cus = LK_MAXWG;
+  if (units > cus) return GPSA_EUNSUPPORTED;
+  const long long ng = (K + 15) / 16;
+  long long n = cus / units;
+  if (n > ng / 4) n = ng / 4;
+  if (n < 1) n = 1;
+  const long long nlong = ng / LK_LONG;
+  if (nlong < n && nlong * 8 >= n * 7) n = nlong;
+  for (int p = 0; p < nprob; ++p) ns[p] = (int)n;
+  return 0;
+}
+
+static long long lk_plan_bytes(int nprob, const int* sym, int MB, long long K, const int* rs, const int* ns,
+                               long long* wgs) {
+  const long long ng = (K + 15) / 16;
+  long long bytes = 0, w = 0;
+  for (int p = 0; p < nprob; ++p) {
+    if ((rs[p] != 1 && rs[p] != 2 && rs[p] != 4) || rs[p] > MB || ns[p] < 1 || ns[p] > ng || ns[p] > 65535) return 0;
+    bytes += (long long)ns[p] * lk_tiles(MB, sym[p] != 0) * 256 * 8;
+    w += (long long)rs[p] * ns[p];
+  }
+  if (wgs) *wgs = w;
+  return bytes;
+}
+
+static inline bool lk_shape_ok(int MB, long long K, int nprob) {
+  return MB != 0 && nprob >= 1 && nprob <= LK_MAXP && K >= 512 && !(K & 1);
+}
+
+template <int MB, int SC, bool STRIPS, int GM, int DT>
+static int longk64_launch_one(const LongKArgs& a, int nblk, hipStream_t st) {
+  constexpr int NPIECE = MB * (GM ? 2 : 1) * 2, NPW = (NPIECE + LK_WAVES - 1) / LK_WAVES;
   constexpr int lds = 2 * (NPW * LK_WAVES * 1024 + (DT ? LK_WAVES * (DT == 2 ? 1024 : 256) : 0));
   static per_device_flag attr_flag;
   bool& attr_set = attr_flag.here();
   if (!attr_set) {
-    if (hipFuncSetAttribute(reinterpret_cast<const void*>(&longk64_kernel<MB, HASG, DT>),
+    if (hipFuncSetAttribute(reinterpret_cast<const void*>(&longk64_kernel<MB, SC, STRIPS, GM, DT>),
                             hipFuncAttributeMaxDynamicSharedMemorySize, lds) != hipSuccess)
       return GPSA_EUNSUPPORTED;
     attr_set = true;
   }
-  dim3 grid((unsigned)a.nsplit, (unsigned)a.nprob);
-  longk64_kernel<MB, HASG, DT><<<grid, 512, lds, st>>>(a);
+  longk64_kernel<MB, SC, STRIPS, GM, DT><<<dim3((unsigned)nblk), 512, lds, st>>>(a);
   GPSA_LAUNCH_CHECK();
   return 0;
 }
 
-template <bool HASG, int DT>
-static int longk64_launch(int MB, const LongKArgs& a, hipStream_t st) {
+template <int MB, int SC, bool STRIPS>
+static int longk64_launch_sc(int gm, int dt, const LongKArgs& a, int nblk, hipStream_t st) {
+  if (dt == 0) return longk64_launch_one<MB, SC, STRIPS, 1, 0>(a, nblk, st);
+  if constexpr (!STRIPS) {
+    if (gm == 1)
+      return dt == 1 ? longk64_launch_one<MB, SC, false, 1, 1>(a, nblk, st)
+                     : longk64_launch_one<MB, SC, false, 1, 2>(a, nblk, st);
+    if (gm == 0)
+      return dt == 1 ? longk64_launch_one<MB, SC, false, 0, 1>(a, nblk, st)
+                     : longk64_launch_one<MB, SC, false, 0, 2>(a, nblk, st);
+  }
+  return dt == 1 ? longk64_launch_one<MB, SC, STRIPS, 2, 1>(a, nblk, st)
+                 : longk64_launch_one<MB, SC, STRIPS, 2, 2>(a, nblk, st);
+}
+
+template <int MB>
+static int longk64_launch_mb(int sc, bool strips, int gm, int dt, const LongKArgs& a, int nblk, hipStream_t st) {
+  if (!strips) return longk64_launch_sc<MB, 1, false>(gm, dt, a, nblk, st);
+  if (sc == 4 && MB >= 4) return longk64_launch_sc<MB, (MB >= 4 ? 4 : 2), true>(gm, dt, a, nblk, st);
+  if (sc >= 2) return longk64_launch_sc<MB, 2, true>(gm, dt, a, nblk, st);
+  return longk64_launch_sc<MB, 1, true>(gm, dt, a, nblk, st);
+}
+
+static int longk64_launch(int MB, int sc, bool strips, int gm, int dt, const LongKArgs& a, int nblk, hipStream_t st) {
   switch (MB) {
-    case 2: return longk64_launch_mb<2, HASG, DT>(a, st);
-    case 4: return longk64_launch_mb<4, HASG, DT>(a, st);
-    case 7: return longk64_launch_mb<7, HASG, DT>(a, st);
-    case 13: return longk64_launch_mb<13, HASG, DT>(a, st);
-    case 16: return longk64_launch_mb<16, HASG, DT>(a, st);
+    case 2: return longk64_launch_mb<2>(sc, strips, gm, dt, a, nblk, st);
+    case 4: return longk64_launch_mb<4>(sc, strips, gm, dt, a, nblk, st);
+    case 7: return longk64_launch_mb<7>(sc, strips, gm, dt, a, nblk, st);
+    case 13: return longk64_launch_mb<13>(sc, strips, gm, dt, a, nblk, st);
+    case 16: return longk64_launch_mb<16>(sc, strips, gm, dt, a, nblk, st);
     default: return GPSA_EUNSUPPORTED;
   }
 }
 
+static int lk_block_table(int nprob, int MB, const int* sym, const int* rs, const int* ns, const double* const* B,
+                          unsigned* wg) {
+  static_assert(LK_MAXWG % 8 == 0, "8 queues");
+  constexpr int QL = LK_MAXWG / 8;
+  unsigned queue[8][QL];
+  int len[8] = {0, 0, 0, 0, 0, 0, 0, 0};
+  for (int p = 0; p < nprob; ++p) {
+    bool led = false;
+    for (int q = 0; q < p; ++q) led = led || (B[q] == B[p] && ns[q] == ns[p]);
+    if (led) continue;
+    for (int sl = 0; sl < ns[p]; ++sl) {
+      int x = 0;
+      for (int k = 1; k < 8; ++k) x = len[k] < len[x] ? k : x;
+      for (int q = p; q < nprob; ++q) {
+        if (B[q] != B[p] || ns[q] != ns[p]) continue;
+        for (int s = 0; s < rs[q]; ++s) {
+          if (len[x] == QL) return 0;
+          const unsigned i0 = (unsigned)lk_cut(MB, rs[q], s, sym[q] != 0), i1 = (unsigned)lk_cut(MB, rs[q], s + 1, sym[q] != 0);
+          queue[x][len[x]++] = (unsigned)q | i0 << 6 | i1 << 11 | (unsigned)sl << 16;
+        }
+      }
+    }
+  }
+  int depth = 0;
+  for (int k = 0; k < 8; ++k) depth = len[k] > depth ? len[k] : depth;
+  for (int b = 0; b < 8 * depth; ++b) wg[b] = (b >> 3) < len[b & 7] ? queue[b & 7][b >> 3] : LK_NOWG;
+  return 8 * depth;
+}
+
+static int longk_run(int nprob, const int* sym, const double* const* G, const double* const* B, const void* const* d,
+                     int d_dtype, int M, long long K, long long ld, const double* alpha, const double* beta,
+                     double* const* out, const int* plan_rs, const int* plan_ns, bool legacy_gate, void* workspace,
+                     long long workspace_bytes, void* stream) {
+  if (nprob < 1 || nprob > LK_MAXP || !sym || !B || !out || !alpha || !beta || M < 1 || K < 2 || ld < K)
+    return GPSA_EINVAL;
+  if (d != nullptr && d_dtype != GPSA_F32 && d_dtype != GPSA_F64) return GPSA_EINVAL;
+  if (G == nullptr && d == nullptr) return GPSA_EINVAL;
+  if ((plan_rs == nullptr) != (plan_ns == nullptr)) return GPSA_EINVAL;
+  const int MB = longk_mb_for(M);
+  if (!lk_shape_ok(MB, K, nprob) || (ld & 1)) return GPSA_EUNSUPPORTED;
+  int rs[LK_MAXP], ns[LK_MAXP];
+  long long wgs = 0;
+  if (plan_rs) {
+    for (int p = 0; p < nprob; ++p) {
+      rs[p] = plan_rs[p];
+      ns[p] = plan_ns[p];
+    }
+  } else {
+    if (legacy_gate && (long long)longk_nsplit(K, nprob) * nprob < 48) return GPSA_EUNSUPPORTED;
+    if (lk_plan(nprob, sym, MB, K, num_cus(), rs, ns)) return GPSA_EUNSUPPORTED;
+  }
+  const long long need = lk_plan_bytes(nprob, sym, MB, K, rs, ns, &wgs);
+  if (plan_rs && (need == 0 || wgs > num_cus() || wgs > LK_MAXWG)) return GPSA_EINVAL;
+  if (!plan_rs && (need == 0 || (!legacy_gate && wgs < 48))) return GPSA_EUNSUPPORTED;
+  LongKArgs a;
+  LongKOut o;
+  memset(&a, 0, sizeof(a));
+  memset(&o, 0, sizeof(o));
+  int ng_ = 0, sc = 4, strips = 0;
+  long long base = 0;
+  for (int p = 0; p < nprob; ++p) {
+    const double* Gp = G ? G[p] : nullptr;
+    if (!B[p] || !out[p] || (d && !d[p]) || (!d && !Gp)) return GPSA_EINVAL;
+    if ((reinterpret_cast<uintptr_t>(B[p]) & 15) || (Gp && (reinterpret_cast<uintptr_t>(Gp) & 15)) ||
+        (d && d_dtype == GPSA_F64 && (reinterpret_cast<uintptr_t>(d[p]) & 15)))
+      return GPSA_EUNSUPPORTED;
+    a.B[p] = B[p];
+    a.G[p] = Gp;
+    a.d[p] = d ? d[p] : nullptr;
+    a.pbase[p] = o.pbase[p] = base;
+    a.meta[p] = (unsigned)ns[p] | (unsigned)((sym[p] ? 1 : 0) | (Gp ? 2 : 0)) << 16;
+    o.meta[p] = a.meta[p] | (unsigned)rs[p] << 24;
+    o.out[p] = out[p];
+    o.alpha[p] = alpha[p];
+    o.beta[p] = beta[p];
+    base += (long long)ns[p] * lk_tiles(MB, sym[p] != 0) * 256;
+    ng_ += Gp ? 1 : 0;
+    strips |= rs[p] > 1;
+    const int nt = lk_nt(MB, rs[p], sym[p] != 0);
+    while (sc > 1 && (sc > MB || lk_nt(MB, sc, false) < nt)) sc >>= 1;
+  }
+  if (workspace_bytes < need) return GPSA_EWORKSPACE;
+  if (!workspace) return GPSA_EINVAL;
+  const int nblk = lk_block_table(nprob, MB, sym, rs, ns, B, a.wg);
+  if (nblk == 0) return plan_rs ? GPSA_EINVAL : GPSA_EUNSUPPORTED;
+  a.part = reinterpret_cast<double*>(workspace);
+  a.M = M;
+  a.K = K;
+  a.ld = ld;
+  hipStream_t st = as_stream(stream);
+  const int gm = ng_ == 0 ? 0 : (ng_ == nprob ? 1 : 2);
+  const int dt = !d ? 0 : (d_dtype == GPSA_F32 ? 1 : 2);
+  int rc = longk64_launch(MB, sc, strips != 0, gm, dt, a, nblk, st);
+  if (rc) return rc;
+  dim3 rg((unsigned)cdiv((long long)M * M, 64), (unsigned)nprob);
+  longk64_reduce_kernel<<<rg, 256, 0, st>>>(a.part, M, MB, o);
+  GPSA_LAUNCH_CHECK();
+  return 0;
+}
+
 }
 
 extern "C" {
+
+int gpsa_longk_f64_plan(int nprob, const int* sym, int M, long long K, int cus, int* rs, int* ns,
+                        long long* workspace_bytes) {
+  using namespace gpsa;
+  if (!sym || !rs || !ns || cus < 1) return GPSA_EINVAL;
+  const int MB = longk_mb_for(M);
+  if (!lk_shape_ok(MB, K, nprob)) return GPSA_EUNSUPPORTED;
+  if (lk_plan(nprob, sym, MB, K, cus, rs, ns)) return GPSA_EUNSUPPORTED;
+  long long wgs = 0;
+  const long long bytes = lk_plan_bytes(nprob, sym, MB, K, rs, ns, &wgs);
+  if (bytes == 0 || wgs < 48) return GPSA_EUNSUPPORTED;
+  if (workspace_bytes) *workspace_bytes = bytes;
+  return 0;
+}
+
+long long gpsa_longk_f64_plan_workspace(int nprob, const int* sym, int M, long long K, const int* rs, const int* ns) {
+  using namespace gpsa;
+  const int MB = longk_mb_for(M);
+  if (!sym || !rs || !ns || !lk_shape_ok(MB, K, nprob)) return 0;
+  return lk_plan_bytes(nprob, sym, MB, K, rs, ns, nullptr);
+}
+
+int gpsa_longk_f64_strip(int M, int sym, int rs, int s, int* row0, int* row1) {
+  using namespace gpsa;
+  const int MB = longk_mb_for(M);
+  if (MB == 0 || (rs != 1 && rs != 2 && rs != 4) || rs > MB || s < 0 || s >= rs) return GPSA_EINVAL;
+  if (row0) *row0 = lk_cut(MB, rs, s, sym != 0);
+  if (row1) *row1 = lk_cut(MB, rs, s + 1, sym != 0);
+  return lk_strip_tiles(MB, rs, s, sym != 0);
+}
+
+int gpsa_longk_f64_slice(long long K, int ns, int t, long long* g0, long long* g1) {
+  const long long ng = (K + 15) / 16;
+  if (K < 1 || ns < 1 || ns > ng || t < 0 || t >= ns || !g0 || !g1) return GPSA_EINVAL;
+  *g0 = t * ng / ns;
+  *g1 = (t + 1) * ng / ns;
+  return 0;
+}
+
+long long gpsa_longk_f64_mixed_workspace(int nprob, const int* sym, int M, long long K) {
+  using namespace gpsa;
+  int rs[LK_MAXP], ns[LK_MAXP];
+  long long bytes = 0;
+  if (gpsa_longk_f64_plan(nprob, sym, M, K, num_cus(), rs, ns, &bytes)) return 0;
+  return bytes;
+}
+
+int gpsa_longk_f64_mixed(int nprob, const int* sym, const double* const* G, const double* const* B,
+                         const void* const* d, int d_dtype, int M, long long K, long long ld, const double* alpha,
+                         const double* beta, double* const* out, const int* plan_rs, const int* plan_ns,
+                         void* workspace, long long workspace_bytes, void* stream) {
+  return gpsa::longk_run(nprob, sym, G, B, d, d_dtype, M, K, ld, alpha, beta, out, plan_rs, plan_ns, false, workspace,
+                         workspace_bytes, stream);
+}
 
 long long gpsa_longk_f64_workspace(int M, long long K, int nprob) {
   using namespace gpsa;
   const int MB = longk_mb_for(M);
-  if (MB == 0 || nprob < 1 || nprob > LK_MAXP || K < 512 || (K & 1)) return 0;
-  const int ns = longk_nsplit(K, nprob);
-  if ((long long)ns * nprob < 48) return 0;
-  return (long long)nprob * ns * MB * 16 * MB * 16 * 8;
+  if (!lk_shape_ok(MB, K, nprob)) return 0;
+  if ((long long)longk_nsplit(K, nprob) * nprob < 48) return 0;
+  int sym[LK_MAXP], rs[LK_MAXP], ns[LK_MAXP];
+  for (int p = 0; p < nprob; ++p) sym[p] = 0;
+  if (lk_plan(nprob, sym, MB, K, num_cus(), rs, ns)) return 0;
+  return lk_plan_bytes(nprob, sym, MB, K, rs, ns, nullptr);
 }
 
 int gpsa_longk_f64(int nprob, const double* const* G, const double* const* B, const void* const* d, int d_dtype,
                    int M, long long K, long long ld, int sym, const double* alpha, const double* beta,
                    double* const* out, void* workspace, long long workspace_bytes, void* stream) {
   using namespace gpsa;
-  if (nprob < 1 || nprob > LK_MAXP || !B || !out || !alpha || !beta || M < 1 || K < 2 || ld < K) return GPSA_EINVAL;
-  if (d != nullptr && d_dtype != GPSA_F32 && d_dtype != GPSA_F64) return GPSA_EINVAL;
-  if (G == nullptr && d == nullptr) return GPSA_EINVAL;
-  const long long need = gpsa_longk_f64_workspace(M, K, nprob);
-  if (need == 0 || (ld & 1)) return GPSA_EUNSUPPORTED;
-  if (workspace_bytes < need) return GPSA_EWORKSPACE;
-  const int MB = longk_mb_for(M);
-  LongKArgs a;
-  LongKOut o;
-  memset(&a, 0, sizeof(a));
-  memset(&o, 0, sizeof(o));
-  for (int p = 0; p < nprob; ++p) {
-    a.B[p] = B[p];
-    a.G[p] = G ? G[p] : nullptr;
-    a.d[p] = d ? d[p] : nullptr;
-    if (!B[p] || !out[p] || (G && !G[p]) || (d && !d[p])) return GPSA_EINVAL;
-    if ((reinterpret_cast<uintptr_t>(B[p]) & 15) || (G && (reinterpret_cast<uintptr_t>(G[p]) & 15)) ||
-        (d && d_dtype == GPSA_F64 && (reinterpret_cast<uintptr_t>(d[p]) & 15)))
-      return GPSA_EUNSUPPORTED;
-    o.out[p] = out[p];
-    o.alpha[p] = alpha[p];
-    o.beta[p] = beta[p];
-  }
-  a.part = reinterpret_cast<double*>(workspace);
-  a.M = M;
-  a.nprob = nprob;
-  a.nsplit = longk_nsplit(K, nprob);
-  a.sym = sym ? 1 : 0;
-  a.K = K;
-  a.ld = ld;
-  a.gper = cdiv(cdiv(K, 16), a.nsplit);
-  hipStream_t st = as_stream(stream);
-  int rc;
-  if (G && d && d_dtype == GPSA_F32) rc = longk64_launch<true, 1>(MB, a, st);
-  else if (G && d) rc = longk64_launch<true, 2>(MB, a, st);
-  else if (G) rc = longk64_launch<true, 0>(MB, a, st);
-  else if (d_dtype == GPSA_F32) rc = longk64_launch<false, 1>(MB, a, st);
-  else rc = longk64_launch<false, 2>(MB, a, st);
-  if (rc) return rc;
-  dim3 rg((unsigned)cdiv((long long)M * M, 64), (unsigned)nprob);
-  longk64_reduce_kernel<<<rg, 256, 0, st>>>(a.part, M, MB * 16, a.nsplit, a.sym, o);
-  GPSA_LAUNCH_CHECK();
-  return 0;
-}
-
-}
+  if (nprob < 1 || nprob > LK_MAXP) return GPSA_EINVAL;
+  int syms[LK_MAXP];
+  for (int p = 0; p < nprob; ++p) syms[p] = sym ? 1 : 0;
+  if (G)
+    for (int p = 0; p < nprob; ++p)
+      if (!G[p]) return GPSA_EINVAL;
+  return longk_run(nprob, syms, G, B, d, d_dtype, M, K, ld, alpha, beta, out, nullptr, nullptr, true, workspace,
+                   workspace_bytes, stream);
+}
+
+}
diff --git a/spatial_alignment_amd/csrc/step.hip b/spatial_alignment_amd/csrc/step.hip
--- a/spatial_alignment_amd/csrc/step.hip
+++ b/spatial_alignment_amd/csrc/step.hip
@@ -918,6 +918,34 @@
   if (!c.dry) rc = gpsa_longk_f64(nprob, G, Bm, d, d_dtype, M, K, ld, sym, alpha, beta, out, ws, wsb, c.stv());
   c.sc.release(mk);
   return rc;
+}
+
+static int longk_mixed(Ctx& c, int nprob, const int* sym, const double* const* G, const double* const* Bm,
+                       const void* const* d, int d_dtype, int M, long long K, long long ld, const double* alpha,
+                       const double* beta, double* const* out) {
+  const long long wsb = gpsa_longk_f64_mixed_workspace(nprob, sym, M, K);
+  if (wsb == 0 || (ld & 1)) return GPSA_EUNSUPPORTED;
+  const long long mk = c.sc.mark();
+  void* ws = c.sc.get<char>(wsb);
+  int rc = 0;
+  if (!c.dry)
+    rc = gpsa_longk_f64_mixed(nprob, sym, G, Bm, d, d_dtype, M, K, ld, alpha, beta, out, nullptr, nullptr, ws, wsb,
+                              c.stv());
+  c.sc.release(mk);
+  return rc;
+}
+
+static inline int warp_longk_views(int D) { return 48 / (D + 1); }
+static bool warp_longk_covered(int Mx, long long Cs, int D, int cnt) {
+  const int vc = warp_longk_views(D);
+  if (vc < 1 || (Cs & 1)) return false;
+  int sym[48];
+  for (int v0 = 0; v0 < cnt; v0 += vc) {
+    const int nv = cnt - v0 < vc ? cnt - v0 : vc;
+    for (int i = 0; i < nv * (D + 1); ++i) sym[i] = (i % (D + 1)) < D ? 1 : 0;
+    if (gpsa_longk_f64_mixed_workspace(nv * (D + 1), sym, Mx, Cs) == 0) return false;
+  }
+  return true;
 }
 
 static int mm_stage_fwd(Ctx& c) {
@@ -1632,39 +1660,34 @@
                    0.0, B.dresid + (long long)r.v0 * Mx * D, D, (long long)Mx * D, r.cnt, splitk_for(Cs, Mx, D)));
     GPSA_CK(project_views(c, c.inv(GW, P.pos_Kw(r.b0)), abar + oMC, Mx, Cs, gamma + oMC, nullptr, r.cnt, r.b0, true));
     bool done = false;
-    if (r.cnt * D <= 48 && gpsa_longk_f64_workspace(Mx, Cs, r.cnt * D) > 0 && gpsa_longk_f64_workspace(Mx, Cs, r.cnt) > 0) {
-      const double *Gs[48], *Bs[48];
-      const void* ds[48];
-      double al[48], be[48];
-      double* os[48];
-      int n = 0;
-      for (int i = 0; i < r.cnt; ++i)
-        for (int jj = 0; jj < D; ++jj, ++n) {
-          Gs[n] = nullptr;
-          Bs[n] = alpha + oMC + (long long)i * Mx * Cs;
-          ds[n] = g + oDC + ((long long)i * D + jj) * Cs;
-          al[n] = 1.0;
-          be[n] = acc ? 1.0 : 0.0;
-          os[n] = B.dstack[0] + ((long long)P.pos_OmG((r.v0 + i) * D + jj)) * mm;
+    if (warp_longk_covered(Mx, Cs, D, r.cnt)) {
+      const int vc = warp_longk_views(D);
+      for (int w0 = 0; w0 < r.cnt; w0 += vc) {
+        const int nv = r.cnt - w0 < vc ? r.cnt - w0 : vc;
+        const double *Gs[48], *Bs[48];
+        const void* ds[48];
+        double al[48], be[48];
+        double* os[48];
+        int sy[48];
+        int n = 0;
+        for (int i = w0; i < w0 + nv; ++i) {
+          for (int jj = 0; jj <= D; ++jj, ++n) {
+            const bool om = jj < D;
+            sy[n] = om ? 1 : 0;
+            Gs[n] = om ? nullptr : gamma + oMC + (long long)i * Mx * Cs;
+            Bs[n] = alpha + oMC + (long long)i * Mx * Cs;
+            ds[n] = om ? g + oDC + ((long long)i * D + jj) * Cs : qbar + (long long)(r.b0 + i) * Cs;
+            al[n] = om ? 1.0 : -1.0;
+            be[n] = acc ? 1.0 : 0.0;
+            os[n] = B.dstack[0] + (long long)(om ? P.pos_OmG((r.v0 + i) * D + jj) : P.pos_Kw(r.b0 + i)) * mm;
+          }
         }
-      int rc = longk(c, n, nullptr, Bs, ds, GPSA_F64, Mx, Cs, Cs, 1, al, be, os);
-      if (rc == 0) {
-        for (int i = 0; i < r.cnt; ++i) {
-          Gs[i] = gamma + oMC + (long long)i * Mx * Cs;
-          Bs[i] = alpha + oMC + (long long)i * Mx * Cs;
-          ds[i] = qbar + (long long)(r.b0 + i) * Cs;
-          al[i] = -1.0;
-          be[i] = acc ? 1.0 : 0.0;
-          os[i] = B.dstack[0] + (long long)P.pos_Kw(r.b0 + i) * mm;
-        }
-        rc = longk(c, r.cnt, Gs, Bs, ds, GPSA_F64, Mx, Cs, Cs, 0, al, be, os);
+        const int rc = longk_mixed(c, n, sy, Gs, Bs, ds, GPSA_F64, Mx, Cs, Cs, al, be, os);
         if (rc != 0) return rc == GPSA_EUNSUPPORTED ? GPSA_EINVAL : rc;
-        GPSA_RUN(gpsa_col_axpy_batched_f64(gamma + oMC, alpha + oMC, qbar + (long long)r.b0 * Cs, 2.0, Mx, Cs,
-                                           gamma + oMC, r.cnt, c.stv()));
-        done = true;
-      } else if (rc != GPSA_EUNSUPPORTED) {
-        return rc;
-      }
+      }
+      GPSA_RUN(gpsa_col_axpy_batched_f64(gamma + oMC, alpha + oMC, qbar + (long long)r.b0 * Cs, 2.0, Mx, Cs,
+                                         gamma + oMC, r.cnt, c.stv()));
+      done = true;
     }
     if (!done || dry) {
       if (acc && !dry) return GPSA_EINVAL;
@@ -1703,9 +1726,7 @@
 
 static bool warp_runs_longk(const Plan& P) {
   for (const Run& r : P.runs)
-    if (!(r.cnt * P.D <= 48 && gpsa_longk_f64_workspace(P.Mx, P.Cs, r.cnt * P.D) > 0 &&
-          gpsa_longk_f64_workspace(P.Mx, P.Cs, r.cnt) > 0))
-      return false;
+    if (!warp_longk_covered(P.Mx, P.Cs, P.D, r.cnt)) return false;
   return true;
 }
 
```
